# Zachary-Luk/3D-Denoising-Diffusion-Model

Hardware: AMD Instinct MI355X
Metric: denoised 64³ volumes/sec @250 DDPM steps, 1/2/4/8 MI355X; PSNR vs ref (higher is better)
Workload: dtype f32 (conv products: 3x f16-split MFMA, f32 accumulate)

## Files before the change

3d-denoising-diffusion-model_amd/csrc/api.hip:

```cpp
#include <hip/hip_runtime.h>
#include <stdarg.h>
#include <stdio.h>
#include <string.h>
#include "conv3d_params.h"
#include "ddpm3d.h"
#include "ops.h"

static thread_local char g_err[512] = "";

static int fail(int code, const char* fmt, ...) {
    va_list ap;
    va_start(ap, fmt);
    vsnprintf(g_err, sizeof(g_err), fmt, ap);
    va_end(ap);
    return code;
}
static int launched(hipError_t e, const char* what) {
    if (e == hipSuccess) return DDPM3D_OK;
    return fail(DDPM3D_ELAUNCH, "%s: %s", what, hipGetErrorString(e));
}
static bool aligned16(const void* p) { return (reinterpret_cast<uintptr_t>(p) & 15) == 0; }

extern "C" {

// ... 51 lines not shown
    if (N <= 0 || D <= 0 || H <= 0 || W <= 0 || Cin <= 0 || Cout <= 0 || !prec_ok(precision)) return 0;
    return ddpm3d_conv_cfg(N, D, H, W, Cin, Cout, ksize, precision).workspace_bytes;
}

enum { ROUTE_GENERAL = 0, ROUTE_SKINNY = 1, ROUTE_PW = 2 };
static int conv_prepare(const ddpm3d_conv_desc* d, ConvK& k, ConvCfg& c, int& route, bool for_launch) {
    if (!d) return fail(DDPM3D_EINVAL, "conv3d: null descriptor");
    if (d->N <= 0 || d->D <= 0 || d->H <= 0 || d->W <= 0 || d->Cout <= 0 || d->Cin <= 0)
        return fail(DDPM3D_EINVAL, "conv3d: non-positive shape N=%d D=%d H=%d W=%d Cin=%d Cout=%d", d->N, d->D,
                    d->H, d->W, d->Cin, d->Cout);
    if (d->ksize != 1 && d->ksize != 3) return fail(DDPM3D_EINVAL, "conv3d: ksize %d (1 or 3)", d->ksize);
    if (!prec_ok(d->precision)) return fail(DDPM3D_ENOSUP, "conv3d: precision mode %d not implemented", d->precision);
    if (d->C0 + d->C1 != d->Cin) return fail(DDPM3D_EINVAL, "conv3d: C0+C1 != Cin");
    if (for_launch && (!d->src0 || !d->w_packed || !d->bias || !d->out)) return fail(DDPM3D_EINVAL, "conv3d: null buffer");
    if (d->in_mode == DDPM3D_IN_PLANAR2) {
        if (d->Cin != 2 || d->C0 != 1 || d->C1 != 1 || (for_launch && !d->src1) || d->aff_a)
            return fail(DDPM3D_EINVAL, "conv3d: planar2 input needs C0=C1=1, two planes, no affine");
    } else {
        if (d->in_mode < 0 || d->in_mode > DDPM3D_IN_STRIDE2) return fail(DDPM3D_EINVAL, "conv3d: in_mode %d", d->in_mode);
        if (d->in_mode == DDPM3D_IN_STRIDE2 && d->ksize != 3)
            return fail(DDPM3D_EINVAL, "conv3d: the strided input mode is the 3x3x3 Downsample conv's");
        if (d->Cin % DDPM3D_CONV_CK) return fail(DDPM3D_EINVAL, "conv3d: Cin=%d not a multiple of %d", d->Cin, DDPM3D_CONV_CK);
        if (d->C1 > 0 && (d->C0 % DDPM3D_CONV_CK || (for_launch && !d->src1)))
            return fail(DDPM3D_EINVAL, "conv3d: concat needs C0 %% %d == 0 and src1", DDPM3D_CONV_CK);
        if (!aligned16(d->src0) || (d->src1 && !aligned16(d->src1)))
            return fail(DDPM3D_EINVAL, "conv3d: sources must be 16-byte aligned");
        if (d->in_mode == DDPM3D_IN_UP && ((d->H | d->W) & 1))
            return fail(DDPM3D_EINVAL, "conv3d: upsampled input needs even H, W (got %d, %d)", d->H, d->W);
    }
    if ((d->aff_a == nullptr) != (d->aff_b == nullptr)) return fail(DDPM3D_EINVAL, "conv3d: aff_a/aff_b must come together");
    if (d->aff_a && (!aligned16(d->aff_a) || !aligned16(d->aff_b)))
        return fail(DDPM3D_EINVAL, "conv3d: affine tables must be 16-byte aligned");
    if (!aligned16(d->w_packed)) return fail(DDPM3D_EINVAL, "conv3d: w_packed must be 16-byte aligned");
    if (d->res_mode < 0 || d->res_mode > 3 || (d->res_mode != DDPM3D_RES_NONE && !d->res))
        return fail(DDPM3D_EINVAL, "conv3d: residual mode %d without / with bad buffer", d->res_mode);
    if (d->res_mode == DDPM3D_RES_UP && ((d->H | d->W) & 1))
        return fail(DDPM3D_EINVAL, "conv3d: upsampled residual needs even H, W");
    if (d->bias_stride_n < 0) return fail(DDPM3D_EINVAL, "conv3d: negative bias_stride_n");
    if (d->out_layout != DDPM3D_OUT_NDHWC && d->out_layout != DDPM3D_OUT_NCDHW)
        return fail(DDPM3D_EINVAL, "conv3d: out_layout %d", d->out_layout);

    c = ddpm3d_conv_cfg(d->N, d->D, d->H, d->W, d->Cin, d->Cout, d->ksize, d->precision);
    if (d->kernel_hint & DDPM3D_HINT_SPLITK_MASK) {
        const int s_forced = (d->kernel_hint & DDPM3D_HINT_SPLITK_MASK) >> DDPM3D_HINT_SPLITK_SHIFT;
        const int nch = ddpm3d_cin_pad(d->Cin) / DDPM3D_CONV_CK;
        if (s_forced > nch || (s_forced != c.S && c.WN != 4))
            return fail(DDPM3D_EINVAL, "conv3d: a forced split factor needs Cout > 64 and S <= Cin / 16");
        ddpm3d_conv_cfg_split(c, s_forced, d->N, d->D, d->H, d->W, d->Cout);
    }
    if (prec_wz(d->precision) &&
        !(wz_layer_ok(d->Cout, d->Cin, d->ksize) && c.WN == 4 && c.MT == 4 &&
          (d->in_mode == DDPM3D_IN_SAME || d->in_mode == DDPM3D_IN_UP)))
        return fail(DDPM3D_ENOSUP, "conv3d: the Winograd-D form needs ksize 3, Cout %% 128 == 0 "
                                   "and input mode SAME or UP; use the F16X3 packing for this call");
    if (for_launch && c.S > 1 && (!d->workspace || d->workspace_bytes < c.workspace_bytes || !aligned16(d->workspace)))
        return fail(DDPM3D_EINVAL, "conv3d: this shape is split %d-way over Cin and needs %zu bytes of "
                                   "16-byte aligned workspace (got %zu)", c.S, c.workspace_bytes,
                    d->workspace ? d->workspace_bytes : (size_t)0);
    memset(&k, 0, sizeof(k));
    k.src0 = d->src0; k.src1 = d->src1; k.affA = d->aff_a; k.affB = d->aff_b;
    k.w = (const float*)d->w_packed; k.bias = d->bias; k.res = d->res; k.out = d->out; k.stats = d->stats;
    k.N = d->N; k.D = d->D; k.H = d->H; k.W = d->W; k.Cin = d->Cin; k.Cout = d->Cout;
    k.C0 = d->C0; k.C1 = d->C1;
    k.CinPad = ddpm3d_cin_pad(d->Cin); k.CoutPad = ddpm3d_cout_pad(d->Cout);
    k.in_mode = d->in_mode; k.act = d->act; k.bias_stride_n = d->bias_stride_n;
    k.res_mode = d->res_mode; k.out_layout = d->out_layout;
    k.tilesZ = c.tilesZ; k.tilesY = c.tilesY; k.tilesX = c.tilesX;
    k.stats_rows = c.stats_rows;
    k.reduce_vox = c.reduce_vox;
    k.hint = d->kernel_hint;
    bool phase = false;
    if (d->kernel_hint & DDPM3D_HINT_UP_PHASE) {
        if (d->precision != DDPM3D_PREC_F16X3_WZ || d->in_mode != DDPM3D_IN_UP)
            return fail(DDPM3D_EINVAL, "conv3d: DDPM3D_HINT_UP_PHASE needs precision F16X3_WZ and in_mode UP");
        UpPhaseGeom g;
        phase = ddpm3d_up_phase_geom(d->D, d->H, d->W, c, g) && d->res_mode != DDPM3D_RES_POOL;
        if (!phase) k.hint &= ~DDPM3D_HINT_UP_PHASE;
    }
    const size_t w_front = phase ? ddpm3d_packed_bytes(d->Cout, d->Cin, d->ksize, d->precision) : (size_t)0;
    k.w = (const float*)((const char*)d->w_packed + w_front);
    k.io = d->io_dtype;
    if (d->io_dtype & ~(DDPM3D_IO_SRC0_BF16 | DDPM3D_IO_SRC1_BF16 | DDPM3D_IO_OUT_BF16 | DDPM3D_IO_RES_BF16 |
                        DDPM3D_IO_HALF_IS_F16))
        return fail(DDPM3D_EINVAL, "conv3d: unknown io_dtype bits %#x", d->io_dtype);
    if ((d->io_dtype & DDPM3D_IO_OUT_BF16) && d->out_layout != DDPM3D_OUT_NDHWC)
        return fail(DDPM3D_EINVAL, "conv3d: a 16-bit output needs the NDHWC layout");
    if ((d->io_dtype & (DDPM3D_IO_SRC0_BF16 | DDPM3D_IO_SRC1_BF16)) && d->in_mode == DDPM3D_IN_PLANAR2)
        return fail(DDPM3D_EINVAL, "conv3d: the planar input volumes are fp32");
    if (prec_scaled(d->precision)) {
        if (!d->in_bound || d->in_bound_count <= 0 || d->in_bound_count > 64 || d->in_bound_stride <= 0)
            return fail(DDPM3D_EINVAL, "conv3d: the split-f16 precisions need in_bound (1..64 entries per sample): "
                                       "the activation scale is derived from it, nothing is clamped");
        k.in_bound = d->in_bound;
        k.in_bound_count = d->in_bound_count;
        k.in_bound_stride = d->in_bound_stride;
    }
    k.ksplit = c.S;
    k.chunks_per_split = (k.CinPad / DDPM3D_CONV_CK + c.S - 1) / c.S;
    if (d->ksize == 1 && c.S > 1) k.chunks_per_split = (k.chunks_per_split + 1) & ~1;
    k.partial = (float*)d->workspace;
    {
        const bool dbl = d->in_mode == DDPM3D_IN_POOL || d->in_mode == DDPM3D_IN_STRIDE2;
        const long long Hs = dbl ? 2LL * d->H : (d->in_mode == DDPM3D_IN_UP ? d->H / 2 : d->H);
        const long long Ws = dbl ? 2LL * d->W : (d->in_mode == DDPM3D_IN_UP ? d->W / 2 : d->W);
        const long long vox = (long long)d->N * d->D * Hs * Ws;
        const long long b0 = vox * d->C0 * ((d->io_dtype & DDPM3D_IO_SRC0_BF16) ? 2 : 4);
        const long long b1 = vox * d->C1 * ((d->io_dtype & DDPM3D_IO_SRC1_BF16) ? 2 : 4);
        const size_t wb = phase ? ddpm3d_up_phase_body_bytes(d->Cout, d->Cin)
                                : ddpm3d_packed_bytes(d->Cout, d->Cin, d->ksize, d->precision);
        if (b0 >= 0xFFFFFFF0LL || b1 >= 0xFFFFFFF0LL || wb >= 0xFFFFFFF0ULL)
            return fail(DDPM3D_E2BIG, "conv3d: a source tensor or the weights exceed 4 GiB; split the batch");
        if ((long long)d->D * d->H * d->W * d->Cout * 4 >= 0xFFFFFFF0LL)
            return fail(DDPM3D_E2BIG, "conv3d: one output sample exceeds 4 GiB; tile the volume");
        k.src0_bytes = (unsigned)b0; k.src1_bytes = (unsigned)b1; k.w_bytes = (unsigned)wb;
        k.wstat = (d->kernel_hint & DDPM3D_HINT_WSTAT_ON)    ? 1
                  : (d->kernel_hint & DDPM3D_HINT_WSTAT_OFF) ? 0
                                                             : ((long long)wb > b0 + b1 ? 1 : 0);
    }
    if (phase)
        k.wscale = (const float*)((const char*)k.w + ddpm3d_up_phase_body_bytes(d->Cout, d->Cin));
    else if (c.PREC != DDPM3D_PREC_F32)
        k.wscale = (const float*)((const char*)d->w_packed +
                                  ddpm3d_packed_bytes(d->Cout, d->Cin, d->ksize, d->precision) -
                                  (size_t)ddpm3d_cout_pad(d->Cout) * 4);
    if (d->stats && d->stats_rows != k.stats_rows)
        return fail(DDPM3D_EINVAL, "conv3d: stats_rows=%d, this shape writes %d", d->stats_rows, k.stats_rows);
    if (d->stats && !aligned16(d->stats)) return fail(DDPM3D_EINVAL, "conv3d: stats must be 16-byte aligned");
    if (d->stats && d->out_layout != DDPM3D_OUT_NDHWC)
        return fail(DDPM3D_EINVAL, "conv3d: statistics only with NDHWC output");
    const long long blocks = (long long)k.N * k.tilesZ * k.tilesY * k.tilesX;
    if (blocks > 0x7fffffffLL) return fail(DDPM3D_EINVAL, "conv3d: grid too large");
    if (d->ksize == 3 && d->Cout <= 2 && d->in_mode == DDPM3D_IN_SAME && d->C1 == 0 && !d->stats &&
        d->res_mode == DDPM3D_RES_NONE &&
        ddpm3d_skinny_ok(k.CinPad, d->precision, !(d->io_dtype & DDPM3D_IO_SRC0_BF16) ? 0
                                                  : ((d->io_dtype & DDPM3D_IO_HALF_IS_F16) ? 2 : 1)))
        route = ROUTE_SKINNY;
    else
        route = ddpm3d_pw_ok(k, c, d->ksize) ? ROUTE_PW : ROUTE_GENERAL;
    return DDPM3D_OK;
}

int ddpm3d_conv3d(const ddpm3d_conv_desc* d, void* stream) {
    ConvK k;
    ConvCfg c;
    int route = ROUTE_GENERAL;
    const int ok = conv_prepare(d, k, c, route, true);
    if (ok != DDPM3D_OK) return ok;
    if (route == ROUTE_SKINNY)
        return launched(ddpm3d_launch_conv_skinny(k, d->precision, (hipStream_t)stream), "conv3d (skinny)");
    const int rc = route == ROUTE_PW ? launched(ddpm3d_launch_conv_pw(k, c, (hipStream_t)stream), "conv3d (1x1)")
                                     : launched(ddpm3d_launch_conv(k, c, (hipStream_t)stream), "conv3d");
    if (rc != DDPM3D_OK || c.S == 1) return rc;
    return launched(ddpm3d_launch_splitk_reduce(k, (hipStream_t)stream), "conv3d split-K reduce");
}

int ddpm3d_conv_plan(const ddpm3d_conv_desc* d, int* stats_rows, size_t* workspace_bytes, int* split) {
    ConvK k;
    ConvCfg c;
    int route = ROUTE_GENERAL;
    const int ok = conv_prepare(d, k, c, route, false);
    if (ok != DDPM3D_OK) return ok;
    if (stats_rows) *stats_rows = c.stats_rows;
    if (workspace_bytes) *workspace_bytes = c.workspace_bytes;
    if (split) *split = c.S;
    return DDPM3D_OK;
}

int ddpm3d_conv_kernel_family(const ddpm3d_conv_desc* d, char* name, int name_len) {
    if (!name || name_len <= 0) return fail(DDPM3D_EINVAL, "conv_kernel_family: no buffer");
    ConvK k;
    ConvCfg c;
    int route = ROUTE_GENERAL;
    const int ok = conv_prepare(d, k, c, route, false);
    if (ok != DDPM3D_OK) return ok;
    const int tile = 1 << c.TXL;
    int n;
    if (route == ROUTE_SKINNY) n = snprintf(name, (size_t)name_len, "conv3d_p%d_k3_skinny", d->precision);
    else if (route == ROUTE_PW) n = snprintf(name, (size_t)name_len, "conv1x1_p%d_t%d", d->precision, tile);
    else n = snprintf(name, (size_t)name_len, "conv3d_p%d_k%d_wn%d_t%d", d->precision, d->ksize, c.WN, tile);
    if (n < 0 || n >= name_len) return fail(DDPM3D_EINVAL, "conv_kernel_family: buffer of %d bytes is too short", name_len);
    return DDPM3D_OK;
}

int ddpm3d_gn_finalize(const double* stats0, int C0, int rows0, const double* stats1, int C1, int rows1,
                       int N, int groups, double count, float eps, const float* gamma, const float* beta,
                       const float* film, int film_stride, int film_off, float* aff_a, float* aff_b,
                       float* bound, void* stream) {
    const int C = C0 + C1;
    if (!stats0 || N <= 0 || groups <= 0 || C0 <= 0 || C1 < 0 || rows0 <= 0 || count <= 0)
        return fail(DDPM3D_EINVAL, "gn_finalize: bad arguments");
    if (!aligned16(stats0) || (stats1 && !aligned16(stats1)))
        return fail(DDPM3D_EINVAL, "gn_finalize: statistics must be 16-byte aligned");
    if (gamma ? (!beta || !aff_a || !aff_b) : !bound)
        return fail(DDPM3D_EINVAL, "gn_finalize: gamma needs beta, aff_a, aff_b; without gamma only `bound` is written");
    if (C % groups) return fail(DDPM3D_EINVAL, "gn_finalize: C=%d not divisible by %d groups", C, groups);
    const int cg = C / groups;
    if (C1 > 0 && (!stats1 || rows1 <= 0 || C0 % cg))
        return fail(DDPM3D_EINVAL, "gn_finalize: a group straddles the concat boundary (C0=%d, group=%d)", C0, cg);
    return launched(ddpm3d_launch_gn_finalize(stats0, C0, rows0, stats1, C1, rows1, N, groups, count, eps,
                                              gamma, beta, film, film_stride, film_off, aff_a, aff_b, bound,
                                              (hipStream_t)stream),
                    "gn_finalize");
}

int ddpm3d_absmax(const float* x0, const float* x1, int N, size_t per_sample, float* bound, void* stream) {
    if (!x0 || !bound || N <= 0 || per_sample == 0) return fail(DDPM3D_EINVAL, "absmax: bad arguments");
    return launched(ddpm3d_launch_absmax(x0, x1, N, per_sample, bound, (hipStream_t)stream), "absmax");
}

int ddpm3d_gn_stats_rows(int voxels) { return voxels > 0 ? ddpm3d_gn_stats_rows_impl(voxels) : 0; }

int ddpm3d_gn_stats(const float* x, int N, int voxels, int C, double* stats, void* stream) {
    if (!x || !stats || N <= 0 || voxels <= 0 || C <= 0 || (C & 3) || !aligned16(x) || !aligned16(stats))
        return fail(DDPM3D_EINVAL, "gn_stats: bad arguments (C must be a multiple of 4, x 16-byte aligned)");
    return launched(ddpm3d_launch_gn_stats(x, N, voxels, C, stats, (hipStream_t)stream), "gn_stats");
}

int ddpm3d_timestep_embedding(const float* t, int rows, int dim, const float* freqs, float* out, void* stream) {
    if (!t || !out || !freqs || rows <= 0 || dim <= 1) return fail(DDPM3D_EINVAL, "timestep_embedding: bad arguments");
    return launched(ddpm3d_launch_timestep_embedding(t, rows, dim, freqs, out, (hipStream_t)stream),
                    "timestep_embedding");
}

int ddpm3d_linear(const float* in, int rows, int K, const float* w, const float* bias, int O, int silu_in,
                  float* out, int out_stride, void* stream) {
    if (!in || !w || !bias || !out || rows <= 0 || K <= 0 || O <= 0 || out_stride < O)
        return fail(DDPM3D_EINVAL, "linear: bad arguments");
    return launched(ddpm3d_launch_linear(in, rows, K, w, bias, O, silu_in, out, out_stride, (hipStream_t)stream),
                    "linear");
}

int ddpm3d_pool_act(const void* src, const float* aff_a, const float* aff_b, int act, int fast_act, int N, int D,
                    int H, int W, int C, void* out, int io_dtype, void* stream) {
    if (!src || !out || N <= 0 || D <= 0 || H <= 0 || W <= 0 || C <= 0 || (C & 3))
        return fail(DDPM3D_EINVAL, "pool_act: bad arguments (C must be a multiple of 4)");
    if ((aff_a == nullptr) != (aff_b == nullptr)) return fail(DDPM3D_EINVAL, "pool_act: aff_a/aff_b must come together");
    if (act && !aff_a) return fail(DDPM3D_EINVAL, "pool_act: an activation needs the affine tables (pass A = 1, B = 0)");
    if (io_dtype & ~(DDPM3D_IO_SRC0_BF16 | DDPM3D_IO_OUT_BF16 | DDPM3D_IO_HALF_IS_F16))
        return fail(DDPM3D_EINVAL, "pool_act: io_dtype bits %#x", io_dtype);
    if (!aligned16(src) || !aligned16(out) || (aff_a && (!aligned16(aff_a) || !aligned16(aff_b))))
        return fail(DDPM3D_EINVAL, "pool_act: buffers must be 16-byte aligned");
    if ((long long)N * D * H * W * (C / 4) > 0x7fffffffLL * 256)
        return fail(DDPM3D_E2BIG, "pool_act: grid too large; split the batch");
    return launched(ddpm3d_launch_pool_act((const float*)src, aff_a, aff_b, act, fast_act, N, D, H, W, C, (float*)out,
                                           (io_dtype & DDPM3D_IO_SRC0_BF16) != 0, (io_dtype & DDPM3D_IO_OUT_BF16) != 0,
                                           (io_dtype & DDPM3D_IO_HALF_IS_F16) != 0, (hipStream_t)stream),
                    "pool_act");
}

int ddpm3d_add_embedding(float* emb, const float* table, const int64_t* idx, int rows, int dim, int num_classes,
                         void* stream) {
    if (!emb || !table || !idx || rows <= 0 || dim <= 0 || num_classes <= 0)
        return fail(DDPM3D_EINVAL, "add_embedding: bad arguments");
    (void)num_classes;
    return launched(ddpm3d_launch_add_embedding(emb, table, idx, rows, dim, num_classes, (hipStream_t)stream), "add_embedding");
}

int ddpm3d_ncdhw_to_ndhwc(const float* in, int N, int C, int voxels, float* out, void* stream) {
    if (!in || !out || N <= 0 || C <= 0 || voxels <= 0) return fail(DDPM3D_EINVAL, "ncdhw_to_ndhwc: bad arguments");
    return launched(ddpm3d_launch_transpose(in, N, C, voxels, out, (hipStream_t)stream), "ncdhw_to_ndhwc");
}
int ddpm3d_ndhwc_to_ncdhw(const float* in, int N, int C, int voxels, float* out, void* stream) {
    if (!in || !out || N <= 0 || C <= 0 || voxels <= 0) return fail(DDPM3D_EINVAL, "ndhwc_to_ncdhw: bad arguments");
    return launched(ddpm3d_launch_transpose(in, N, voxels, C, out, (hipStream_t)stream), "ndhwc_to_ncdhw");
}

int ddpm3d_ncdhw_to_ndhwc_pad(const float* in, int N, int C, int voxels, int Cpad, float* out, void* stream) {
    if (!in || !out || N <= 0 || C <= 0 || voxels <= 0 || Cpad < C)
        return fail(DDPM3D_EINVAL, "ncdhw_to_ndhwc_pad: bad arguments");
    return launched(ddpm3d_launch_to_ndhwc_pad(in, N, C, voxels, Cpad, out, (hipStream_t)stream), "ncdhw_to_ndhwc_pad");
}

int ddpm3d_subsample_hw2(const float* in, int N, int D, int H, int W, int C, float* out, void* stream) {
    if (!in || !out || N <= 0 || D <= 0 || H <= 0 || W <= 0 || C <= 0 || (H & 1) || (W & 1) || (C & 3) ||
        !aligned16(in) || !aligned16(out))
        return fail(DDPM3D_EINVAL, "subsample_hw2: needs even H, W, C %% 4 == 0 and 16-byte aligned tensors");
    return launched(ddpm3d_launch_subsample_hw2(in, N, D, H, W, C, out, (hipStream_t)stream), "subsample_hw2");
}

int ddpm3d_attention_p(const float* qkv, int N, int T, int heads, int head_channels, int precision,
                       const float* qkv_bound, int bound_count, int bound_stride, float* out, void* stream) {
    if (!qkv || !out || N <= 0 || T <= 0 || heads <= 0) return fail(DDPM3D_EINVAL, "attention: bad arguments");
    if (head_channels != 32 && head_channels != 64 && head_channels != 128)
        return fail(DDPM3D_ENOSUP, "attention: %d channels per head (32, 64 or 128 are built)", head_channels);
    if (precision != DDPM3D_PREC_F32 && precision != DDPM3D_PREC_F16X3)
        return fail(DDPM3D_ENOSUP, "attention: precision %d (F32 and F16X3 are built)", precision);
    if (!aligned16(qkv) || !aligned16(out)) return fail(DDPM3D_EINVAL, "attention: buffers must be 16-byte aligned");
    if (precision != DDPM3D_PREC_F32 && (!qkv_bound || bound_count <= 0 || bound_count > 64 || bound_stride <= 0))
        return fail(DDPM3D_EINVAL, "attention: the split-f16 arithmetic needs qkv_bound (1..64 entries per sample)");
    return launched(ddpm3d_launch_attention(qkv, N, T, heads, head_channels, precision, qkv_bound, bound_count,
                                            bound_stride, out, (hipStream_t)stream),
                    "attention");
}

int ddpm3d_attention(const float* qkv, int N, int T, int heads, int head_channels, float* out, void* stream) {
    return ddpm3d_attention_p(qkv, N, T, heads, head_channels, DDPM3D_PREC_F32, nullptr, 0, 0, out, stream);
}

static int step_args_ok(const float* mo, const float* x, const float* noise, const float* coef,
                        const int64_t* t, int N, int voxels, float* sample) {
    return mo && x && noise && coef && t && sample && N > 0 && voxels > 0;
}

int ddpm3d_p_sample_step(const float* model_out, const float* x, const float* noise, const float* coef,
                         const int64_t* t_idx, int N, int voxels, int flags, float* sample,
                         float* pred_xstart, void* stream) {
// ... 383 lines not shown
```

3d-denoising-diffusion-model_amd/csrc/conv3d.hip:

```cpp
#include <hip/hip_runtime.h>
#include "conv3d_load.h"
#include "conv3d_epilogue.h"

template <int PREC, int PIPEM, int KS, int WN, int MT, int TXL, int TYL>
__global__ __launch_bounds__(256, (PIPEM == 2 ? 1 : (TXL == 2 ? 2 : 3))) void conv3d_kernel(const ConvK p) {
    constexpr int CK = DDPM3D_CONV_CK;
    constexpr int PIPE = PIPEM == 1 ? 1 : 0;
    constexpr int SXY = PIPEM == 2 ? 2 : 1;
    constexpr int WM = 4 / WN;
    constexpr int TX = 1 << TXL, TY = 1 << TYL;
    constexpr int TZ = WM * MT * 32 / (TX * TY);
    constexpr int PAD = KS / 2;
    constexpr int HX = SXY * (TX - 1) + KS, HY = SXY * (TY - 1) + KS, HZ = TZ + 2 * PAD;
    constexpr int HV = HX * HY * HZ;
    constexpr int VS = 5;
    constexpr int RY = LdsGeom<TX, HX, HY>::RY;
    constexpr int RZ = LdsGeom<TX, HX, HY>::RZ;
    constexpr int QPV = CK / 4;
    constexpr int NT = KS * KS * KS;
    constexpr int NL = (HV * QPV + 255) / 256;

    extern __shared__ __attribute__((aligned(16))) unsigned char lds[];

    const int tid = threadIdx.x;
// ... 71 lines not shown
    for (int chunk = chunk_begin; chunk < chunk_end; ++chunk) {
        __syncthreads();
        {
            auto store_item = [&](int hz, int hy, int hx, const f32x4 v) {
                unsigned char* vrow = lds + (hz * RZ + hy * RY + hx * VS) * 16;
                if constexpr (PREC == 0) {
                    *reinterpret_cast<f32x4*>(vrow + q * 16) = v;
                } else if constexpr (PREC == 5) {
                    *reinterpret_cast<u32x2*>(vrow + q * 8) = u32x2{bf16_pack(v[0], v[1]), bf16_pack(v[2], v[3])};
                } else {
                    h4 hi, lo;
#pragma unroll
                    for (int c = 0; c < 4; ++c) {
                        const float s = v[c] * asc.s;
                        hi[c] = (_Float16)s;
                        lo[c] = (_Float16)(s - (float)hi[c]);
                    }
                    *reinterpret_cast<h4*>(vrow + q * 8) = hi;
                    if constexpr (PREC == 1) *reinterpret_cast<h4*>(vrow + 32 + q * 8) = lo;
                }
            };
            if constexpr (PIPE) {
#pragma unroll
                for (int i = 0; i < NL; ++i) {
                    const int idx = tid + i * 256;
                    if (idx < HV * QPV) {
                        const int hv = idx / QPV;
                        const int hz = hv / (HY * HX);
                        const int rem = hv - hz * (HY * HX);
                        const int hy = rem / HX;
                        const int hx = rem - hy * HX;
                        const bool inb = halo_inb(p, z0 - PAD + hz, y0 - PAD + hy, x0 - PAD + hx);
                        store_item(hz, hy, hx, halo_finish<PREC != 0>(hs, quad_bits_expand(raw[i], hs.b16, hs.f16), inb, act_mask));
                    }
                }
            } else {
#pragma unroll 1
                for (int idx = tid; idx < HV * QPV; idx += 256) {
                    const int hv = idx / QPV;
                    const int hz = hv / (HY * HX);
                    const int rem = hv - hz * (HY * HX);
                    const int hy = rem / HX;
                    const int hx = rem - hy * HX;
                    store_item(hz, hy, hx, halo_fetch<PREC != 0>(p, hs, n, z0 - PAD + hz, SXY * y0 - PAD + hy,
                                                                 SXY * x0 - PAD + hx, q, chunk == 0));
                }
            }
        }
        __syncthreads();
        const bool more = chunk + 1 < chunk_end;
        if (more) hs = halo_src<CK>(p, n, chunk + 1, q);
        if (!wave_active) {
            if (PIPE && more) issue_raw(hs);
            continue;
        }

        const unsigned wchunk = (unsigned)chunk * wchunk_stride;
        constexpr bool LO = PREC != 2 && PREC != 5;
        constexpr int R = 3;
        u32x4 bq[R][2];
#pragma unroll
        for (int s = 0; s < R - 1 && s < NT; ++s) {
            bq[s][0] = buffer_load16(wrsrc, wlane, wchunk + s * wtap_stride);
            if (LO) bq[s][1] = buffer_load16(wrsrc, wlane, wchunk + s * wtap_stride + wpart);
        }
        constexpr bool AHEAD = PREC != 0 && (TXL == 2 || KS == 1);
        h8 af[2][MT][2];
        if constexpr (AHEAD) {
#pragma unroll
            for (int t = 0; t < MT; ++t) {
                af[0][t][0] = *reinterpret_cast<const h8*>(lds + arow[t]);
                if (LO) af[0][t][1] = *reinterpret_cast<const h8*>(lds + arow[t] + 32);
            }
        }
#pragma unroll
        for (int tap = 0; tap < NT; ++tap) {
            if constexpr (AHEAD) {
                __builtin_amdgcn_sched_barrier(0);
                if (tap + 1 < NT) {
                    const int t1 = tap + 1;
                    const int off1 = ((t1 / (KS * KS)) * RZ + ((t1 / KS) % KS) * RY + (t1 % KS) * VS) * 16;
#pragma unroll
                    for (int t = 0; t < MT; ++t) {
                        af[t1 & 1][t][0] = *reinterpret_cast<const h8*>(lds + arow[t] + off1);
                        if (LO) af[t1 & 1][t][1] = *reinterpret_cast<const h8*>(lds + arow[t] + off1 + 32);
                    }
                }
            }
            if (tap + R - 1 < NT) {
                bq[(tap + R - 1) % R][0] = buffer_load16(wrsrc, wlane, wchunk + (tap + R - 1) * wtap_stride);
                if (LO) bq[(tap + R - 1) % R][1] = buffer_load16(wrsrc, wlane, wchunk + (tap + R - 1) * wtap_stride + wpart);
            }
            if constexpr (AHEAD) __builtin_amdgcn_sched_barrier(0);
            if (PIPE && tap == (NT >= R ? NT - R : 0) && more) issue_raw(hs);
            const int dz = tap / (KS * KS), dy = (tap / KS) % KS, dx = tap % KS;
            const int tapoff = (dz * RZ + dy * RY + dx * VS) * 16;
            const u32x4 b0 = bq[tap % R][0], b1 = LO ? bq[tap % R][1] : b0;
            if constexpr (PREC == 0) {
#pragma unroll
                for (int kk = 0; kk < 2; ++kk) {
                    f32x4 a[MT];
#pragma unroll
                    for (int t = 0; t < MT; ++t)
                        a[t] = *reinterpret_cast<const f32x4*>(lds + arow[t] + tapoff + kk * 32);
                    const f32x4 b = __builtin_bit_cast(f32x4, kk == 0 ? b0 : b1);
#pragma unroll
                    for (int s = 0; s < 4; ++s)
#pragma unroll
                        for (int t = 0; t < MT; ++t)
                            acc[t] = __builtin_amdgcn_mfma_f32_32x32x2f32(a[t][s], b[s], acc[t], 0, 0, 0);
                }
            } else if constexpr (PREC == 2 || PREC == 5) {
                const h8 bhi = __builtin_bit_cast(h8, b0);
#pragma unroll
                for (int t = 0; t < MT; ++t) {
                    const h8 ahi = AHEAD ? af[tap & 1][t][0] : *reinterpret_cast<const h8*>(lds + arow[t] + tapoff);
                    acc[t] = mfma16<PREC == 5>(ahi, bhi, acc[t]);
                }
            } else {
                const h8 bhi = __builtin_bit_cast(h8, b0);
                const h8 blo = __builtin_bit_cast(h8, b1);
#pragma unroll
                for (int t = 0; t < MT; ++t) {
                    const h8 ahi = AHEAD ? af[tap & 1][t][0] : *reinterpret_cast<const h8*>(lds + arow[t] + tapoff);
                    const h8 alo = AHEAD ? af[tap & 1][t][1] : *reinterpret_cast<const h8*>(lds + arow[t] + tapoff + 32);
                    acc[t] = __builtin_amdgcn_mfma_f32_32x32x16_f16(alo, bhi, acc[t], 0, 0, 0);
                    acc[t] = __builtin_amdgcn_mfma_f32_32x32x16_f16(ahi, blo, acc[t], 0, 0, 0);
                    acc[t] = __builtin_amdgcn_mfma_f32_32x32x16_f16(ahi, bhi, acc[t], 0, 0, 0);
                }
            }
        }
    }

    if (!wave_active) return;

    const int tile_in_n = (tz_i * p.tilesY + ty_i) * p.tilesX + tx_i;
    conv_epilogue<PREC, WM, MT, TXL, TYL, PREC == 2 || PREC == 5>(p, acc, n, z0, y0, x0, tile_in_n, wm, cout, half, wg.split,
                                                                 asc.inv);
}

#ifndef DDPM3D_PREC_ONLY
#error "compile with -DDDPM3D_PREC_ONLY=0, 1, 2, 3 or 5"
#endif
#if DDPM3D_PREC_ONLY == 0

__global__ __launch_bounds__(256) void conv_splitk_reduce_kernel(const ConvK p) {
    const size_t DHW = (size_t)p.D * p.H * p.W;
    const int rows = p.stats_rows;
    const int n = blockIdx.x / rows, r = blockIdx.x % rows;
    const size_t v0 = (size_t)r * p.reduce_vox;
    const size_t v1 = min(v0 + (size_t)p.reduce_vox, DHW);
    const size_t slab_stride = (size_t)p.N * DHW * p.Cout;
    for (int cout = threadIdx.x; cout < p.Cout; cout += 256) {
        const float bias = p.bias[(size_t)n * p.bias_stride_n + cout];
        GnAcc gs;
        gs.init(0.0f);
        float cnt = 0.0f;
        for (size_t v = v0; v < v1; ++v) {
            const size_t e = ((size_t)n * DHW + v) * p.Cout + cout;
            float val = p.partial[e];
            for (int s = 1; s < p.ksplit; ++s) val += p.partial[e + s * slab_stride];
            val += bias;
            if (p.res_mode != DDPM3D_RES_NONE) {
                const int x = (int)(v % p.W), y = (int)((v / p.W) % p.H), z = (int)(v / ((size_t)p.W * p.H));
                val += ddpm3d_residual(p, n, z, y, x, cout);
            }
            if (p.out_layout == DDPM3D_OUT_NDHWC)
                ddpm3d_act_store(p.out, e, val, (p.io & DDPM3D_IO_OUT_BF16) != 0, (p.io & DDPM3D_IO_HALF_IS_F16) != 0);
            else
                p.out[((size_t)n * p.Cout + cout) * DHW + v] = val;
            if (cnt == 0.0f) gs.init(val);
            gs.add(val);
            cnt += 1.0f;
        }
        if (p.stats != nullptr)
            *reinterpret_cast<double2*>(p.stats + (((size_t)n * p.Cout + cout) * rows + r) * 2) =
                make_double2(gs.sum1(cnt), gs.sum2(cnt));
    }
}

template <int RV>
__global__ __launch_bounds__(256) void conv_splitk_reduce_v4_kernel(const ConvK p) {
    const size_t DHW = (size_t)p.D * p.H * p.W;
    const int rows = p.stats_rows;
    const int n = blockIdx.x / rows, r = blockIdx.x % rows;
    const size_t v0 = (size_t)r * RV;
    const size_t slab_stride = (size_t)p.N * DHW * p.Cout;
    const int quads = p.Cout / 4;
    const int cq = threadIdx.x & 63, vl = threadIdx.x >> 6;
    __shared__ double red[2][4][64 * 4];
    {
        const int q = blockIdx.y * 64 + cq;
        const bool qok = q < quads;
        GnAcc gs[4];
        float cnt = 0.0f;
#pragma unroll
        for (int c = 0; c < 4; ++c) gs[c].init(0.0f);
        if (qok) {
            const f32x4 bias = *reinterpret_cast<const f32x4*>(p.bias + (size_t)n * p.bias_stride_n + q * 4);
#pragma unroll
            for (int i = 0; i < RV / 4; ++i) {
                const size_t v = v0 + vl + 4 * i;
                if (v < DHW) {
                    const size_t e = ((size_t)n * DHW + v) * p.Cout + q * 4;
                    f32x4 val = *reinterpret_cast<const f32x4*>(p.partial + e);
                    int s = 1;
                    for (; s + 3 < p.ksplit; s += 4) {
                        const f32x4 a = *reinterpret_cast<const f32x4*>(p.partial + e + (size_t)s * slab_stride);
                        const f32x4 b = *reinterpret_cast<const f32x4*>(p.partial + e + (size_t)(s + 1) * slab_stride);
                        const f32x4 c = *reinterpret_cast<const f32x4*>(p.partial + e + (size_t)(s + 2) * slab_stride);
                        const f32x4 d = *reinterpret_cast<const f32x4*>(p.partial + e + (size_t)(s + 3) * slab_stride);
                        val += a; val += b; val += c; val += d;
                    }
                    for (; s < p.ksplit; ++s)
                        val += *reinterpret_cast<const f32x4*>(p.partial + e + (size_t)s * slab_stride);
                    val += bias;
                    if (p.res_mode != DDPM3D_RES_NONE) {
                        const int x = (int)(v % p.W), y = (int)((v / p.W) % p.H), z = (int)(v / ((size_t)p.W * p.H));
#pragma unroll
                        for (int c = 0; c < 4; ++c) val[c] += ddpm3d_residual(p, n, z, y, x, q * 4 + c);
                    }
                    if (p.io & DDPM3D_IO_OUT_BF16) {
                        const bool f16 = (p.io & DDPM3D_IO_HALF_IS_F16) != 0;
                        u32x2 pk = u32x2{half_pack(val[0], val[1], f16), half_pack(val[2], val[3], f16)};
                        *reinterpret_cast<u32x2*>(reinterpret_cast<unsigned short*>(p.out) + e) = pk;
                        asm volatile("s_nop 7" : "+v"(pk) : : "memory");
                    }
                    else
                        *reinterpret_cast<f32x4*>(p.out + e) = val;
#pragma unroll
                    for (int c = 0; c < 4; ++c) {
                        if (cnt == 0.0f) gs[c].init(val[c]);
                        gs[c].add(val[c]);
                    }
                    cnt += 1.0f;
                }
            }
        }
        if (p.stats != nullptr) {
#pragma unroll
            for (int c = 0; c < 4; ++c) {
                red[0][vl][cq * 4 + c] = gs[c].sum1(cnt);
                red[1][vl][cq * 4 + c] = gs[c].sum2(cnt);
            }
            __syncthreads();
            if (vl == 0 && qok) {
#pragma unroll
                for (int c = 0; c < 4; ++c) {
                    const double a = (red[0][0][cq * 4 + c] + red[0][1][cq * 4 + c]) +
                                     (red[0][2][cq * 4 + c] + red[0][3][cq * 4 + c]);
                    const double b = (red[1][0][cq * 4 + c] + red[1][1][cq * 4 + c]) +
                                     (red[1][2][cq * 4 + c] + red[1][3][cq * 4 + c]);
                    *reinterpret_cast<double2*>(p.stats + (((size_t)n * p.Cout + q * 4 + c) * rows + r) * 2) =
                        make_double2(a, b);
                }
            }
            __syncthreads();
        }
    }
}

hipError_t ddpm3d_launch_splitk_reduce(const ConvK& k, hipStream_t st) {
    if (k.Cout % 4 == 0 && k.out_layout == DDPM3D_OUT_NDHWC) {
        const dim3 grid(k.N * k.stats_rows, (k.Cout / 4 + 63) / 64);
        switch (k.reduce_vox) {
            case 4: hipLaunchKernelGGL(conv_splitk_reduce_v4_kernel<4>, grid, dim3(256), 0, st, k); break;
            case 8: hipLaunchKernelGGL(conv_splitk_reduce_v4_kernel<8>, grid, dim3(256), 0, st, k); break;
            case 16: hipLaunchKernelGGL(conv_splitk_reduce_v4_kernel<16>, grid, dim3(256), 0, st, k); break;
            default: return hipErrorInvalidValue;
        }
    } else
        hipLaunchKernelGGL(conv_splitk_reduce_kernel, dim3(k.N * k.stats_rows), dim3(256), 0, st, k);
    return hipGetLastError();
}

hipError_t ddpm3d_launch_conv_p0(const ConvK& k, const ConvCfg& c, hipStream_t st);
hipError_t ddpm3d_launch_conv_p1(const ConvK& k, const ConvCfg& c, hipStream_t st);
hipError_t ddpm3d_launch_conv_p2(const ConvK& k, const ConvCfg& c, hipStream_t st);
hipError_t ddpm3d_launch_conv_p5(const ConvK& k, const ConvCfg& c, hipStream_t st);
hipError_t ddpm3d_launch_conv_wz(const ConvK& k, const ConvCfg& c, hipStream_t st);

hipError_t ddpm3d_launch_conv(const ConvK& k, const ConvCfg& c, hipStream_t st) {
    switch (c.PREC) {
        case 0: return ddpm3d_launch_conv_p0(k, c, st);
        case 1: return ddpm3d_launch_conv_p1(k, c, st);
        case 2: return ddpm3d_launch_conv_p2(k, c, st);
        case 3:
        case 4:
        case 6: return ddpm3d_launch_conv_wz(k, c, st);
        case 5: return ddpm3d_launch_conv_p5(k, c, st);
    }
    return hipErrorInvalidValue;
}
#endif

#if DDPM3D_PREC_ONLY == 3
#include "conv3d_wz.h"
hipError_t ddpm3d_launch_conv_wz(const ConvK& k, const ConvCfg& c, hipStream_t st) {
    const int gy = k.CoutPad / 128;
    const int gx = k.N * k.tilesZ * k.tilesY * k.tilesX;
#ifdef DDPM3D_WZ_STAMPS
    constexpr size_t stamp_lds = 4 * WZ_NSTAMP * 8;
#else
    constexpr size_t stamp_lds = 0;
#endif
    constexpr size_t lds = (size_t)WzGeom::BUF + stamp_lds;
    if (k.hint & DDPM3D_HINT_UP_PHASE) {
        UpPhaseGeom g;
        if (c.PREC != DDPM3D_PREC_F16X3_WZ || !ddpm3d_up_phase_geom(k.D, k.H, k.W, c, g)) return hipErrorInvalidValue;
        ConvK k2 = k;
        k2.tilesX = g.tilesX; k2.tilesY = g.tilesY; k2.tilesZ = g.tilesZ;
        const dim3 grid(4 * k.N * g.tilesZ * g.tilesY * g.tilesX, gy, k.ksplit);
        constexpr size_t plds4 = (size_t)WzGeomT<4>::BUF + stamp_lds, plds84 = (size_t)WzGeomT<8, 4>::BUF + stamp_lds;
        if (g.TX == 4)
            hipLaunchKernelGGL((conv3d_wz_kernel<WZ_F16X3_UP, 4, 4, 4>), grid, dim3(256), plds4, st, k2);
        else if (g.TY == 4)
            hipLaunchKernelGGL((conv3d_wz_kernel<WZ_F16X3_UP, 4, 8, 4>), grid, dim3(256), plds84, st, k2);
        else
            hipLaunchKernelGGL((conv3d_wz_kernel<WZ_F16X3_UP, 4, 8, 8>), grid, dim3(256), lds, st, k2);
        return hipGetLastError();
    }
    if (c.TXL == 2) {
        constexpr size_t lds4 = (size_t)WzGeomT<4>::BUF + stamp_lds;
        if (c.PREC == DDPM3D_PREC_F16_WZ)
            hipLaunchKernelGGL((conv3d_wz_kernel<WZ_F16, 0, 4>), dim3(gx, gy, k.ksplit), dim3(256), lds4, st, k);
        else if (c.PREC == DDPM3D_PREC_BF16_WZ)
            hipLaunchKernelGGL((conv3d_wz_kernel<WZ_BF16, 0, 4>), dim3(gx, gy, k.ksplit), dim3(256), lds4, st, k);
        else
            hipLaunchKernelGGL((conv3d_wz_kernel<WZ_F16X3, 4, 4>), dim3(gx, gy, k.ksplit), dim3(256), lds4, st, k);
        return hipGetLastError();
    }
#ifndef DDPM3D_WZ_T84
#define DDPM3D_WZ_T84 1
#endif
    if (DDPM3D_WZ_T84 && k.H % 8 == 0 && k.D % 4 == 0 && !(k.hint & DDPM3D_HINT_WZ_ORDER_MASK)) {
        ConvK k2 = k;
        k2.tilesY = 2 * k.tilesY;
        k2.tilesZ = k.tilesZ / 2;
        constexpr size_t lds84 = (size_t)WzGeomT<8, 4>::BUF + stamp_lds;
        if (c.PREC == DDPM3D_PREC_F16_WZ)
            hipLaunchKernelGGL((conv3d_wz_kernel<WZ_F16, 0, 8, 4>), dim3(gx, gy, k.ksplit), dim3(256), lds84, st, k2);
        else if (c.PREC == DDPM3D_PREC_BF16_WZ)
            hipLaunchKernelGGL((conv3d_wz_kernel<WZ_BF16, 0, 8, 4>), dim3(gx, gy, k.ksplit), dim3(256), lds84, st, k2);
        else
            hipLaunchKernelGGL((conv3d_wz_kernel<WZ_F16X3, 4, 8, 4>), dim3(gx, gy, k.ksplit), dim3(256), lds84, st, k2);
        return hipGetLastError();
    }
    if (c.PREC == DDPM3D_PREC_F16_WZ)
        hipLaunchKernelGGL(conv3d_wz_kernel<WZ_F16>, dim3(gx, gy, k.ksplit), dim3(256), lds, st, k);
    else if (c.PREC == DDPM3D_PREC_BF16_WZ)
        hipLaunchKernelGGL(conv3d_wz_kernel<WZ_BF16>, dim3(gx, gy, k.ksplit), dim3(256), lds, st, k);
    else {
        int order = (k.hint & DDPM3D_HINT_WZ_ORDER_MASK) >> DDPM3D_HINT_WZ_ORDER_SHIFT;
        if (order == 0) order = 5;
        switch (order - 1) {
            case 0: hipLaunchKernelGGL((conv3d_wz_kernel<WZ_F16X3, 0>), dim3(gx, gy, k.ksplit), dim3(256), lds, st, k); break;
            case 1: hipLaunchKernelGGL((conv3d_wz_kernel<WZ_F16X3, 1>), dim3(gx, gy, k.ksplit), dim3(256), lds, st, k); break;
            case 2: hipLaunchKernelGGL((conv3d_wz_kernel<WZ_F16X3, 2>), dim3(gx, gy, k.ksplit), dim3(256), lds, st, k); break;
            case 4: hipLaunchKernelGGL((conv3d_wz_kernel<WZ_F16X3, 4>), dim3(gx, gy, k.ksplit), dim3(256), lds, st, k); break;
            default: return hipErrorInvalidValue;
        }
    }
    return hipGetLastError();
}
#else

template <int PREC, int PIPE, int KS, int WN, int MT, int TXL, int TYL>
static hipError_t launch_cfg(const ConvK& k, int grid_x, int grid_y, hipStream_t st) {
    constexpr int TX = 1 << TXL, TY = 1 << TYL, TZ = (4 / WN) * MT * 32 / (TX * TY);
    constexpr int PAD = KS / 2, SXY = PIPE == 2 ? 2 : 1;
    constexpr int HX = SXY * (TX - 1) + KS, HY = SXY * (TY - 1) + KS, HZ = TZ + 2 * PAD;
    constexpr size_t lds_bytes = (size_t)HZ * LdsGeom<TX, HX, HY>::RZ * 16;
    if constexpr (lds_bytes > 65536) {
        static DynLdsOnce once = {};
        const hipError_t attr = ddpm3d_allow_dynamic_lds(
            once, reinterpret_cast<const void*>(&conv3d_kernel<PREC, PIPE, KS, WN, MT, TXL, TYL>), (int)lds_bytes);
        if (attr != hipSuccess) return attr;
    }
    hipLaunchKernelGGL((conv3d_kernel<PREC, PIPE, KS, WN, MT, TXL, TYL>), dim3(grid_x, grid_y, k.ksplit), dim3(256),
                       lds_bytes, st, k);
    return hipGetLastError();
}

#define DDPM3D_CAT2(a, b) a##b
#define DDPM3D_CAT(a, b) DDPM3D_CAT2(a, b)
hipError_t DDPM3D_CAT(ddpm3d_launch_conv_p, DDPM3D_PREC_ONLY)(const ConvK& k, const ConvCfg& c, hipStream_t st) {
    const int gx = k.N * k.tilesZ * k.tilesY * k.tilesX;
    const int gy = (k.CoutPad + 32 * c.WN - 1) / (32 * c.WN);
    const int pipe = k.in_mode == DDPM3D_IN_STRIDE2 ? 2 : ((k.in_mode == DDPM3D_IN_SAME || k.in_mode == DDPM3D_IN_UP) ? 1 : 0);
#define CASE(P_, PI_, KS_, WN_, MT_, TXL_, TYL_)                                                      \
    if (pipe == PI_ && c.KS == KS_ && c.WN == WN_ && c.MT == MT_ && c.TXL == TXL_ && c.TYL == TYL_)   \
        return launch_cfg<P_, PI_, KS_, WN_, MT_, TXL_, TYL_>(k, gx, gy, st);
#define CASES(P_, PI_)                                                                          \
    CASE(P_, PI_, 3, 4, 4, 3, 3) CASE(P_, PI_, 3, 2, 2, 3, 3) CASE(P_, PI_, 3, 1, 1, 3, 3)      \
    CASE(P_, PI_, 3, 4, 4, 2, 2) CASE(P_, PI_, 3, 2, 2, 2, 2) CASE(P_, PI_, 3, 1, 1, 2, 2)      \
    CASE(P_, PI_, 1, 4, 4, 3, 3) CASE(P_, PI_, 1, 2, 2, 3, 3) CASE(P_, PI_, 1, 1, 1, 3, 3)      \
    CASE(P_, PI_, 1, 4, 4, 2, 2) CASE(P_, PI_, 1, 2, 2, 2, 2) CASE(P_, PI_, 1, 1, 1, 2, 2)
    CASES(DDPM3D_PREC_ONLY, 1) CASES(DDPM3D_PREC_ONLY, 0)
    CASE(DDPM3D_PREC_ONLY, 2, 3, 4, 4, 3, 3) CASE(DDPM3D_PREC_ONLY, 2, 3, 2, 2, 3, 3) CASE(DDPM3D_PREC_ONLY, 2, 3, 1, 1, 3, 3)
    CASE(DDPM3D_PREC_ONLY, 2, 3, 4, 4, 2, 2) CASE(DDPM3D_PREC_ONLY, 2, 3, 2, 2, 2, 2) CASE(DDPM3D_PREC_ONLY, 2, 3, 1, 1, 2, 2)
#undef CASES
#undef CASE
    return hipErrorInvalidValue;
}
#endif
```

3d-denoising-diffusion-model_amd/csrc/conv3d_params.h:

```cpp
#pragma once
#include <hip/hip_runtime.h>
#include <stddef.h>
#include <stdlib.h>
#include "ddpm3d.h"

#define DDPM3D_CONV_CK 16
#define DDPM3D_REDUCE_VOX 16
#define DDPM3D_X3_W_TARGET 8.0f

struct ConvK {
    const float* src0;
    const float* src1;
    const float* affA;
    const float* affB;
    const float* w;
    const float* bias;
    const float* res;
    float* out;
    double* stats;
    float* partial;
    const float* wscale;
    const float* in_bound;
    int in_bound_count, in_bound_stride;
    unsigned w_bytes, src0_bytes, src1_bytes;
    int N, D, H, W, Cin, Cout, C0, C1, CinPad, CoutPad;
    int in_mode, act, bias_stride_n, res_mode, out_layout, stats_rows;
    int tilesX, tilesY, tilesZ;
    int ksplit, chunks_per_split;
    int wstat;
    int reduce_vox;
    int hint;
    int io;
};

struct ConvCfg {
    int PREC;
    int KS;
    int WN;
    int MT;
    int TXL, TYL;
    int S;
    int tilesX, tilesY, tilesZ;
    int stats_rows;
    int reduce_vox;
    size_t workspace_bytes;
};

static inline int ddpm3d_round_up(int v, int m) { return (v + m - 1) / m * m; }
static inline int ddpm3d_cout_pad(int Cout) { return ddpm3d_round_up(Cout, 32); }
static inline int ddpm3d_cin_pad(int Cin) { return ddpm3d_round_up(Cin, DDPM3D_CONV_CK); }

static inline void ddpm3d_conv_cfg_split(ConvCfg& c, int S, int N, int D, int H, int W, int Cout) {
    const long long vox = (long long)D * H * W;
    c.S = S;
    if (S > 1) {
        c.stats_rows = (int)((vox + c.reduce_vox - 1) / c.reduce_vox);
        c.workspace_bytes = (size_t)S * N * vox * Cout * sizeof(float);
    } else {
        c.stats_rows = c.tilesZ * c.tilesY * c.tilesX * (4 / c.WN);
        c.workspace_bytes = 0;
    }
}

static inline ConvCfg ddpm3d_conv_cfg(int N, int D, int H, int W, int Cin, int Cout, int ksize, int prec) {
    ConvCfg c;
    c.PREC = prec;
    const bool one_mfma = prec == DDPM3D_PREC_F16 || prec == DDPM3D_PREC_F16_WZ || prec == DDPM3D_PREC_BF16 ||
                          prec == DDPM3D_PREC_BF16_WZ;
    c.KS = ksize;
    c.WN = Cout > 64 ? 4 : (Cout > 32 ? 2 : 1);
#ifdef DDPM3D_FORCE_T4_3X3
    if (H >= 8 && W >= 8 && ksize != 3) { c.TXL = 3; c.TYL = 3; } else { c.TXL = 2; c.TYL = 2; }
#else
    if (H >= 8 && W >= 8) { c.TXL = 3; c.TYL = 3; } else { c.TXL = 2; c.TYL = 2; }
#endif
    c.MT = c.WN;
    const int TX = 1 << c.TXL, TY = 1 << c.TYL, TZ = (4 / c.WN) * c.MT * 32 / (TX * TY);
    c.tilesX = (W + TX - 1) / TX;
    c.tilesY = (H + TY - 1) / TY;
    c.tilesZ = (D + TZ - 1) / TZ;
    const long long mtiles = (long long)N * c.tilesZ * c.tilesY * c.tilesX;
    const long long blocks = mtiles * ((ddpm3d_cout_pad(Cout) + 32 * c.WN - 1) / (32 * c.WN));
    const int nch = ddpm3d_cin_pad(Cin) / DDPM3D_CONV_CK;
    int best = 1;
    if (ksize == 1 && c.WN == 4) {
        double best_cost = 1e300;
        for (int s = 1; s <= 32 && s <= nch; ++s) {
            const int cps = (nch + s - 1) / s;
            if (s > 1 && cps < 4) break;
            const long long per_cu = (blocks * s + 255) / 256;
            const double cost = (double)per_cu * (0.25 * cps + 6.0) + (s > 1 ? 6.0 : 0.0);
            if (cost < best_cost * 0.9) { best_cost = cost; best = s; }
        }
    }
    if (ksize == 3 && c.WN == 4 && !one_mfma) {
        static const double eff[4] = {1.0, 0.62, 0.78, 0.82};
        double best_cost = 1e300;
        for (int s = 1; s <= 16 && s <= nch; ++s) {
            const int cps = (nch + s - 1) / s;
            if (s > 1 && cps < 2) break;
            const long long per_cu = (blocks * s + 255) / 256;
            const double e = eff[per_cu > 3 ? 3 : (int)per_cu];
            const double cost = (double)per_cu * (cps + (s > 1 ? 0.75 : 0.5)) / e;
            if (cost < best_cost * 0.99) { best_cost = cost; best = s; }
        }
    }
    if (ksize == 3 && c.WN == 4 && one_mfma) {
        static const double eff[4] = {1.0, 0.5, 1.0, 0.9};
        static const int cand[] = {1, 2, 3, 4, 5, 6, 8, 10, 12, 16};
        const double out_mb = (double)N * D * H * W * Cout * 4.0 / 1e6;
        double best_cost = 1e300;
        for (int i = 0; i < 10 && cand[i] <= nch; ++i) {
            const int s = cand[i];
            const int cps = (nch + s - 1) / s;
            if (s > 1 && cps < 2) break;
            const long long per_cu = (blocks * s + 255) / 256;
            const double e = eff[per_cu > 3 ? 3 : (int)per_cu];
            const double cost = (double)per_cu * (cps + (s > 1 ? 3.0 : 0.25)) / e + (s > 1 ? 0.2 * s * out_mb : 0.0);
            if (cost < best_cost * 0.99) { best_cost = cost; best = s; }
        }
    }
    const long long vox = (long long)D * H * W;
    c.reduce_vox = DDPM3D_REDUCE_VOX;
    while (c.reduce_vox > 4 &&
           (long long)N * ((vox + c.reduce_vox - 1) / c.reduce_vox) * ((Cout / 4 + 63) / 64) < 1024)
        c.reduce_vox /= 2;
    ddpm3d_conv_cfg_split(c, best, N, D, H, W, Cout);
    return c;
}

static inline size_t ddpm3d_packed_bytes(int Cout, int Cin, int ksize, int prec) {
    const size_t taps = (prec == DDPM3D_PREC_F16X3_WZ || prec == DDPM3D_PREC_F16_WZ || prec == DDPM3D_PREC_BF16_WZ)
                            ? 36 : (size_t)ksize * ksize * ksize;
    const size_t body = taps * ddpm3d_cin_pad(Cin) * ddpm3d_cout_pad(Cout) * 4;
    return prec != 0 ? body + (size_t)ddpm3d_cout_pad(Cout) * 4 : body;
}

static inline size_t ddpm3d_up_phase_body_bytes(int Cout, int Cin) {
    return (size_t)64 * ddpm3d_cin_pad(Cin) * ddpm3d_cout_pad(Cout) * 4;
}
static inline size_t ddpm3d_up_phase_bytes(int Cout, int Cin) {
    return ddpm3d_packed_bytes(Cout, Cin, 3, DDPM3D_PREC_F16X3_WZ) + ddpm3d_up_phase_body_bytes(Cout, Cin) +
           (size_t)ddpm3d_cout_pad(Cout) * 4;
}
struct UpPhaseGeom { int TX, TY, tilesX, tilesY, tilesZ; };
static inline bool ddpm3d_up_phase_geom(int D, int H, int W, const ConvCfg& c, UpPhaseGeom& g) {
    if (((H | W) & 1) || c.KS != 3 || c.WN != 4 || c.MT != 4) return false;
    const int Hl = H / 2, Wl = W / 2;
    if (Hl >= 8 && Wl >= 8) { g.TX = 8; g.TY = (Hl % 8 == 0 && D % 4 == 0) ? 4 : 8; }
    else { g.TX = 4; g.TY = 4; }
    const int TZ = 128 / (g.TX * g.TY);
    g.tilesX = (Wl + g.TX - 1) / g.TX;
    g.tilesY = (Hl + g.TY - 1) / g.TY;
    g.tilesZ = (D + TZ - 1) / TZ;
    return 4LL * g.tilesX * g.tilesY * g.tilesZ == (long long)c.tilesX * c.tilesY * c.tilesZ;
}

struct DynLdsOnce { unsigned long long mask[4]; };
static inline hipError_t ddpm3d_allow_dynamic_lds(DynLdsOnce& done, const void* kernel, int bytes) {
    int dev = 0;
    hipError_t e = hipGetDevice(&dev);
    if (e != hipSuccess) return e;
    dev &= 255;
    unsigned long long& w = done.mask[dev >> 6];
    const unsigned long long bit = 1ull << (dev & 63);
    if (__atomic_load_n(&w, __ATOMIC_ACQUIRE) & bit) return hipSuccess;
    e = hipFuncSetAttribute(kernel, hipFuncAttributeMaxDynamicSharedMemorySize, bytes);
    if (e == hipSuccess) __atomic_fetch_or(&w, bit, __ATOMIC_RELEASE);
    return e;
}

hipError_t ddpm3d_launch_conv(const ConvK& k, const ConvCfg& c, hipStream_t st);
hipError_t ddpm3d_launch_splitk_reduce(const ConvK& k, hipStream_t st);
hipError_t ddpm3d_launch_conv_skinny(const ConvK& k, int prec, hipStream_t st);
hipError_t ddpm3d_launch_conv_pw(const ConvK& k, const ConvCfg& c, hipStream_t st);
static inline bool ddpm3d_pw_ok(const ConvK& k, const ConvCfg& c, int ksize) {
    const bool s0 = (k.io & DDPM3D_IO_SRC0_BF16) != 0, s1 = (k.io & DDPM3D_IO_SRC1_BF16) != 0;
    return ksize == 1 && (c.PREC == 1 || c.PREC == 2 || c.PREC == 5) && c.WN == 4 && c.MT == 4 &&
           k.in_mode == DDPM3D_IN_SAME && k.affA == nullptr && k.act == 0 && k.stats == nullptr &&
           k.Cout % 128 == 0 && k.Cin % 32 == 0 && k.C0 % 32 == 0 && (k.C1 == 0 || s0 == s1) &&
           (k.ksplit == 1 || k.chunks_per_split % 2 == 0);
}
bool ddpm3d_skinny_ok(int CinPad, int prec, int src16);

struct GnAcc {
#ifdef DDPM3D_STATS_F64
    double a1, a2;
    __device__ __forceinline__ void init(float) { a1 = 0.0; a2 = 0.0; }
    __device__ __forceinline__ void add(float v) { const double d = (double)v; a1 += d; a2 = __builtin_fma(d, d, a2); }
    __device__ __forceinline__ double sum1(float) const { return a1; }
    __device__ __forceinline__ double sum2(float) const { return a2; }
#else
    float p, s1, s2;
    __device__ __forceinline__ void init(float pivot) { p = pivot; s1 = 0.0f; s2 = 0.0f; }
    __device__ __forceinline__ void add(float v) { const float d = v - p; s1 += d; s2 = __builtin_fmaf(d, d, s2); }
    __device__ __forceinline__ double sum1(float n) const { return (double)n * (double)p + (double)s1; }
    __device__ __forceinline__ double sum2(float n) const {
        const double dp = (double)p;
        return (double)s2 + 2.0 * dp * (double)s1 + (double)n * dp * dp;
    }
#endif
};

__device__ __forceinline__ float ddpm3d_half_to_float(unsigned short h, bool f16) {
    if (f16) return (float)__builtin_bit_cast(_Float16, h);
    return __builtin_bit_cast(float, (unsigned)h << 16);
}
__device__ __forceinline__ float ddpm3d_act_load(const float* base, size_t e, bool b16, bool f16) {
    if (b16) return ddpm3d_half_to_float(reinterpret_cast<const unsigned short*>(base)[e], f16);
    return base[e];
}
__device__ __forceinline__ unsigned short ddpm3d_to_bf16(float v) {
    return __builtin_bit_cast(unsigned short, (__bf16)v);
}
__device__ __forceinline__ unsigned short ddpm3d_to_half(float v, bool f16) {
    if (f16) return __builtin_bit_cast(unsigned short, (_Float16)v);
    return ddpm3d_to_bf16(v);
}
__device__ __forceinline__ void ddpm3d_act_store(float* base, size_t e, float v, bool b16, bool f16) {
    if (b16) reinterpret_cast<unsigned short*>(base)[e] = ddpm3d_to_half(v, f16);
    else base[e] = v;
}

__device__ __forceinline__ float ddpm3d_residual(const ConvK& p, int n, int z, int y, int x, int cout) {
    const bool b16 = (p.io & DDPM3D_IO_RES_BF16) != 0, f16 = (p.io & DDPM3D_IO_HALF_IS_F16) != 0;
    if (p.res_mode == DDPM3D_RES_SAME) {
        const size_t vox = (((size_t)n * p.D + z) * p.H + y) * p.W + x;
        return ddpm3d_act_load(p.res, vox * p.Cout + cout, b16, f16);
    }
    if (p.res_mode == DDPM3D_RES_UP) {
        const int Hr = p.H / 2, Wr = p.W / 2;
        const size_t rv = (((size_t)n * p.D + z) * Hr + (y >> 1)) * Wr + (x >> 1);
        return ddpm3d_act_load(p.res, rv * p.Cout + cout, b16, f16);
    }
    if (p.res_mode == DDPM3D_RES_POOL) {
        const int Hr = p.H * 2, Wr = p.W * 2;
        const size_t rv = (((size_t)n * p.D + z) * Hr + 2 * y) * Wr + 2 * x;
        const size_t e = rv * p.Cout + cout;
        const float r = ((ddpm3d_act_load(p.res, e, b16, f16) + ddpm3d_act_load(p.res, e + p.Cout, b16, f16)) +
                         ddpm3d_act_load(p.res, e + (size_t)Wr * p.Cout, b16, f16)) +
                        ddpm3d_act_load(p.res, e + (size_t)Wr * p.Cout + p.Cout, b16, f16);
        return r * 0.25f;
    }
    return 0.0f;
}
```

3d-denoising-diffusion-model_amd/csrc/conv3d_stage.h:

```cpp
#pragma once
#include "conv3d_epilogue.h"

enum { WZ_F16X3 = 0, WZ_F16 = 1, WZ_BF16 = 2,
       WZ_F16X3_UP = 3 };

__device__ __forceinline__ void split_pair(float s0, float s1, unsigned& hi, unsigned& lo) {
    float l0, l1;
    asm("v_cvt_pk_f16_f32 %0, %3, %4\n\t"
        "v_fma_mix_f32 %1, %0, -1.0, %3 op_sel:[0,0,0] op_sel_hi:[1,0,0]\n\t"
        "v_fma_mix_f32 %2, %0, -1.0, %4 op_sel:[1,0,0] op_sel_hi:[1,0,0]"
        : "=&v"(hi), "=&v"(l0), "=&v"(l1)
        : "v"(s0), "v"(s1));
    asm("v_cvt_pk_f16_f32 %0, %1, %2" : "=v"(lo) : "v"(l0), "v"(l1));
}

template <int TX_, int TY_ = TX_>
struct WzGeomT {
    static constexpr int CK = DDPM3D_CONV_CK;
    static constexpr int TX = TX_, TY = TY_, HX = TX_ + 2, HY = TY_ + 2, NP = 4, VS = 5;
    static constexpr int RP = TX_ * TY_;
    static constexpr int NZP = 64 / RP;
    static constexpr int NPL = 2 * NZP + 2;
    static constexpr int RY = LdsGeom<TX_, HX, HY>::RY;
    static constexpr int RZ = LdsGeom<TX_, HX, HY>::RZ;
    static constexpr int PAIR = NP * RZ * 16;
    static constexpr int BUF = NZP * PAIR;
    static constexpr int HC = HX * HY * (CK / 4);
    static constexpr int NL = (HC + 255) / 256;
    static_assert(RP * NZP == 64 && PAIR % 256 == 0, "128-voxel tiles; pair images keep the bank residues");
};
typedef WzGeomT<8, 8> WzGeom;

template <class G>
struct StageLaneT {
    unsigned vo0[G::NL], vo1[G::NL];
    unsigned es0, es1;
    bool f16;
    int lds[G::NL];
    bool ok[G::NL];
    unsigned plane0, plane1;
    int zb;
    float scale;
    float km, ka;
    int q;
};
typedef StageLaneT<WzGeom> StageLane;

template <class G = WzGeom, bool LOWRES = false>
__device__ __forceinline__ StageLaneT<G> stage_lane(const ConvK& p, int lt, int n, int y0, int x0, int zb, float scale) {
    StageLaneT<G> s;
    s.scale = scale;
    const int up_mode = p.in_mode == DDPM3D_IN_UP ? 1 : 0;
    const int Hs = p.H >> up_mode, Ws = p.W >> up_mode;
    const int up = LOWRES ? 0 : up_mode;
    const int Hb = LOWRES ? Hs : p.H, Wb = LOWRES ? Ws : p.W;
    s.q = lt & 3;
    s.zb = zb;
    s.es0 = (p.io & DDPM3D_IO_SRC0_BF16) ? 2u : 4u;
    s.es1 = (p.io & DDPM3D_IO_SRC1_BF16) ? 2u : 4u;
    s.f16 = (p.io & DDPM3D_IO_HALF_IS_F16) != 0;
    s.plane0 = (unsigned)(Hs * Ws) * (unsigned)p.C0 * s.es0;
    s.plane1 = (unsigned)(Hs * Ws) * (unsigned)p.C1 * s.es1;
    s.km = p.act ? -1.44269504088896341f / scale : 0.0f;
    s.ka = p.act ? 0.0f : -126.0f;
#pragma unroll
    for (int i = 0; i < G::NL; ++i) {
        const int idx = lt + i * 256;
        const int hyx = idx >> 2;
        const int hy = hyx / G::HX, hx = hyx - hy * G::HX;
        const int y = y0 - 1 + hy, x = x0 - 1 + hx;
        s.ok[i] = idx < G::HC && (unsigned)y < (unsigned)Hb && (unsigned)x < (unsigned)Wb;
        const unsigned vox = (unsigned)(((n * p.D + zb) * Hs + (y >> up)) * Ws + (x >> up));
        s.vo0[i] = s.ok[i] ? (vox * (unsigned)p.C0 + s.q * 4u) * s.es0 : DDPM3D_OOB_OFFSET;
        s.vo1[i] = s.ok[i] ? (vox * (unsigned)p.C1 + s.q * 4u) * s.es1 : DDPM3D_OOB_OFFSET;
        s.lds[i] = (hy * G::RY + hx * G::VS) * 16 + s.q * 8;
    }
    return s;
}

template <class G>
__device__ __forceinline__ void stage_lane_scale(const ConvK& p, StageLaneT<G>& s, float scale) {
    s.scale = scale;
    s.km = p.act ? -1.44269504088896341f / scale : 0.0f;
}

template <class G>
__device__ __forceinline__ void stage_zero_border(const StageLaneT<G>& s, unsigned char* lds_images, int nimages, int lt) {
#pragma unroll
    for (int i = 0; i < G::NL; ++i) {
        if (lt + i * 256 < G::HC && !s.ok[i]) {
            for (int b = 0; b < nimages * G::NZP; ++b)
#pragma unroll
                for (int j = 0; j < G::NP; ++j) {
                    unsigned char* v = lds_images + b * G::PAIR + j * G::RZ * 16 + s.lds[i];
                    *reinterpret_cast<u32x2*>(v) = u32x2{0u, 0u};
                    *reinterpret_cast<u32x2*>(v + 32) = u32x2{0u, 0u};
                }
        }
    }
}

template <class G>
struct StageRawT {
    u32x4 v[G::NL][G::NPL];
    f32x4 ga, gb;
    unsigned zmask;
    bool b16;
};
typedef StageRawT<WzGeom> StageRaw;

template <class G>
__device__ __forceinline__ void stage_issue(const ConvK& p, const StageLaneT<G>& s, StageRawT<G>& r, int n, int z0, int chunk) {
    const int c0 = chunk * G::CK;
    const bool from0 = c0 < p.C0;
    const __amdgpu_buffer_rsrc_t rs = from0 ? make_rsrc(p.src0, p.src0_bytes) : make_rsrc(p.src1, p.src1_bytes);
    const unsigned plane = from0 ? s.plane0 : s.plane1;
    const unsigned cb4 = (unsigned)(from0 ? c0 : c0 - p.C0) * (from0 ? s.es0 : s.es1);
    r.b16 = (from0 ? s.es0 : s.es1) == 2u;
    r.zmask = 0;
#pragma unroll
    for (int k = 0; k < G::NPL; ++k) {
        const int z = z0 - 1 + k;
        if ((unsigned)z < (unsigned)p.D) {
            r.zmask |= 1u << k;
            const unsigned soff = cb4 + (unsigned)(z - s.zb) * plane;
#pragma unroll
            for (int i = 0; i < G::NL; ++i)
                r.v[i][k] = buffer_load_quad(rs, from0 ? s.vo0[i] : s.vo1[i], soff, r.b16);
        }
    }
    if (p.affA != nullptr) {
        r.ga = *reinterpret_cast<const f32x4*>(p.affA + (size_t)n * p.Cin + c0 + s.q * 4);
        r.gb = *reinterpret_cast<const f32x4*>(p.affB + (size_t)n * p.Cin + c0 + s.q * 4);
    } else {
        r.ga = f32x4{1.f, 1.f, 1.f, 1.f};
        r.gb = f32x4{0.f, 0.f, 0.f, 0.f};
    }
}

template <int MODE, class G>
__device__ __forceinline__ void stage_write(const StageLaneT<G>& s, const StageRawT<G>& r, unsigned char* buf) {
    float sa[4], sb[4];
#pragma unroll
    for (int c = 0; c < 4; ++c) {
        sa[c] = r.ga[c] * s.scale;
        sb[c] = r.gb[c] * s.scale;
    }
#pragma unroll
    for (int i = 0; i < G::NL; ++i) {
        auto plane = [&](const int k, float (&d)[4]) {
            if (r.zmask & (1u << k)) {
                const f32x4 x = quad_bits_expand(r.v[i][k], r.b16, s.f16);
#pragma unroll
                for (int c = 0; c < 4; ++c) {
                    const float ys = __builtin_fmaf(x[c], sa[c], sb[c]);
#ifdef DDPM3D_WZ_NOSILU
                    d[c] = ys;
// ... 45 lines not shown
```

3d-denoising-diffusion-model_amd/csrc/conv3d_wz.h:

```cpp
#pragma once
#include "conv3d_stage.h"

#ifdef DDPM3D_WZ_STAMPS
#define WZ_NSTAMP 48
#define WZ_STAMP(i) do { if (lane == 0) wz_stamps[(i)] = __builtin_amdgcn_s_memtime(); } while (0)
#else
#define WZ_STAMP(i) do { } while (0)
#endif

template <int MODE_, int IL = 0, int TX = 8, int TY = TX>
__global__ __launch_bounds__(256, 2) void conv3d_wz_kernel(const ConvK p) {
    constexpr bool PHASE = MODE_ == WZ_F16X3_UP;
    constexpr int MODE = PHASE ? (int)WZ_F16X3 : MODE_;
    typedef WzGeomT<TX, TY> G;
    constexpr bool X3 = MODE == WZ_F16X3;
    constexpr int CK = DDPM3D_CONV_CK, NT = PHASE ? 16 : 36;
    constexpr int TPJ = NT / 4;
    constexpr int TXL = TX == 8 ? 3 : 2, TYL = TY == 8 ? 3 : 2;
    constexpr int VS = G::VS, RY = G::RY, RZ = G::RZ;

    extern __shared__ __attribute__((aligned(16))) unsigned char lds[];

    const int tid = threadIdx.x;
    const int lane = tid & 63;
    const int wn = __builtin_amdgcn_readfirstlane(tid >> 6);
    const int half = lane >> 5;
#ifdef DDPM3D_WZ_STAMPS
    unsigned long long* wz_stamps = reinterpret_cast<unsigned long long*>(lds + G::BUF) + wn * WZ_NSTAMP;
    WZ_STAMP(0);
#endif

    const WgId wg = wg_id(p);
    int tile = wg.tile;
    const int tx_i = tile % p.tilesX; tile /= p.tilesX;
    const int ty_i = tile % p.tilesY; tile /= p.tilesY;
    const int tz_i = tile % p.tilesZ; tile /= p.tilesZ;
    const int ph = PHASE ? (tile & 3) : 0;
    const int py = ph >> 1, px = ph & 1;
    const int n = PHASE ? tile >> 2 : tile;
    const int x0 = tx_i * TX, y0 = ty_i * TY, z0 = tz_i * 2 * G::NZP;

    int arow[2];
#pragma unroll
    for (int t = 0; t < 2; ++t) {
        const int m = t * 32 + (lane & 31);
        const int pos = m % G::RP;
        arow[t] = (m / G::RP) * G::PAIR + ((pos >> TXL) * RY + (pos & (TX - 1)) * VS + half) * 16;
        if constexpr (PHASE) arow[t] += (py * RY + px * VS) * 16;
    }

    const int cout = wg.cy * 128 + wn * 32 + (lane & 31);
    const float pre_ws = cout < p.Cout ? p.wscale[cout] : 1.0f;
    const float pre_bias = cout < p.Cout ? p.bias[(size_t)n * p.bias_stride_n + cout] : 0.0f;
    const __amdgpu_buffer_rsrc_t wrsrc = make_rsrc(p.w, p.w_bytes);
    const unsigned wlane = ((unsigned)cout * 2 + half) * 16;
    const unsigned wpart = (unsigned)p.CoutPad * 32;
    const unsigned wchunk_stride = 2 * wpart;
    const unsigned wtap_stride = (unsigned)(p.CinPad / CK) * wchunk_stride;

    f32x16 acc[4][2];
#pragma unroll
    for (int j = 0; j < 4; ++j)
#pragma unroll
        for (int t = 0; t < 2; ++t)
#pragma unroll
            for (int i = 0; i < 16; ++i) acc[j][t][i] = 0.0f;

    const int nchunks = p.CinPad / CK;
    const int chunk_begin = wg.split * p.chunks_per_split;
    const int chunk_end = min(nchunks, chunk_begin + p.chunks_per_split);

    ActScale asc = {1.0f, 1.0f};
    float bound_raw = 0.0f;
    if constexpr (MODE != WZ_BF16) bound_raw = act_scale_load(p, n);
    StageLaneT<G> sl = stage_lane<G, PHASE>(p, tid, n, y0, x0, max(z0 - 1, 0), 1.0f);
    stage_zero_border(sl, lds, 1, tid);
    StageRawT<G> raw;
    if (chunk_begin < chunk_end) stage_issue(p, sl, raw, n, z0, chunk_begin);
    if constexpr (MODE != WZ_BF16) {
        asc = act_scale_finish(bound_raw, 2.0f);
        stage_lane_scale(p, sl, asc.s);
    }
    WZ_STAMP(1);

    constexpr int L = X3 ? 1 : 0;
#ifndef DDPM3D_WZ_RING_X3
#define DDPM3D_WZ_RING_X3 4
#endif
#ifndef DDPM3D_WZ_RING_X1
#define DDPM3D_WZ_RING_X1 8
#endif
    constexpr int R = X3 ? DDPM3D_WZ_RING_X3 : DDPM3D_WZ_RING_X1;
    constexpr int STAGE_TAP = X3 ? NT - 3 : NT - 8;
    for (int chunk = chunk_begin; chunk < chunk_end; ++chunk) {
        const bool more = chunk + 1 < chunk_end;
        const unsigned char* bufc = lds;
        WZ_STAMP(2 + (chunk - chunk_begin) * 5);
        __syncthreads();
        WZ_STAMP(3 + (chunk - chunk_begin) * 5);
        stage_write<MODE, G>(sl, raw, lds);
        WZ_STAMP(4 + (chunk - chunk_begin) * 5);
        __syncthreads();
        WZ_STAMP(5 + (chunk - chunk_begin) * 5);

        if constexpr (IL == 3 || IL == 4 || IL == 6) __builtin_amdgcn_s_setprio(1);
        unsigned woff = (unsigned)chunk * wchunk_stride + (PHASE ? (unsigned)ph * 16u * wtap_stride : 0u);
        auto bump = [&]() {
            woff += wtap_stride;
            asm volatile("" : "+s"(woff));
        };
        u32x4 bq[R][X3 ? 2 : 1];
#pragma unroll
        for (int s = 0; s < R - 1; ++s) {
            bq[s][0] = buffer_load16(wrsrc, wlane, woff);
            if (X3) bq[s][L] = buffer_load16(wrsrc, wlane, woff + wpart);
            bump();
        }
#ifndef DDPM3D_WZ_A_AHEAD
#define DDPM3D_WZ_A_AHEAD 1
#endif
        constexpr int AH = DDPM3D_WZ_A_AHEAD, AS = AH + 1;
        h8 af[AS][2][X3 ? 2 : 1];
        auto aread = [&](const int t1) {
            const int off1 = PHASE ? ((t1 / 4) * RZ + ((t1 / 2) % 2) * RY + (t1 % 2) * VS) * 16
                                   : ((t1 / 9) * RZ + ((t1 / 3) % 3) * RY + (t1 % 3) * VS) * 16;
#pragma unroll
            for (int t = 0; t < 2; ++t) {
                af[t1 % AS][t][0] = *reinterpret_cast<const h8*>(bufc + arow[t] + off1);
                if (X3) af[t1 % AS][t][L] = *reinterpret_cast<const h8*>(bufc + arow[t] + off1 + 32);
            }
        };
#pragma unroll
        for (int t1 = 0; t1 < AH; ++t1) aread(t1);
#pragma unroll
        for (int tap = 0; tap < NT; ++tap) {
            __builtin_amdgcn_sched_barrier(0);
            if (tap + AH < NT) aread(tap + AH);
            if (tap + R - 1 < NT) {
                bq[(tap + R - 1) % R][0] = buffer_load16(wrsrc, wlane, woff);
                if (X3) bq[(tap + R - 1) % R][L] = buffer_load16(wrsrc, wlane, woff + wpart);
                bump();
            }
            if constexpr (!IL) __builtin_amdgcn_sched_barrier(0);
            if (tap == STAGE_TAP && more) stage_issue(p, sl, raw, n, z0, chunk + 1);
            const int j = tap / TPJ;
            const h8 bhi = __builtin_bit_cast(h8, bq[tap % R][0]);
            if (X3) {
                const h8 blo = __builtin_bit_cast(h8, bq[tap % R][L]);
#pragma unroll
                for (int t = 0; t < 2; ++t)
                    acc[j][t] = mfma16<false>(af[tap % AS][t][L], bhi, acc[j][t]);
#pragma unroll
                for (int t = 0; t < 2; ++t)
                    acc[j][t] = mfma16<false>(af[tap % AS][t][0], blo, acc[j][t]);
            }
#pragma unroll
            for (int t = 0; t < 2; ++t)
                acc[j][t] = mfma16<MODE == WZ_BF16>(af[tap % AS][t][0], bhi, acc[j][t]);
            if constexpr (IL == 1 || IL == 3) {
#pragma unroll
                for (int i = 0; i < (X3 ? 4 : 2); ++i) {
                    __builtin_amdgcn_sched_group_barrier(0x008, 1, 0);
                    __builtin_amdgcn_sched_group_barrier(0x100, 1, 0);
                }
#pragma unroll
                for (int i = 0; i < (X3 ? 2 : 1); ++i) {
                    __builtin_amdgcn_sched_group_barrier(0x008, 1, 0);
                    __builtin_amdgcn_sched_group_barrier(0x020, 1, 0);
                }
            } else if constexpr (IL == 5 || IL == 6) {
#pragma unroll
                for (int i = 0; i < (X3 ? 2 : 1); ++i) {
                    __builtin_amdgcn_sched_group_barrier(0x008, 1, 0);
                    __builtin_amdgcn_sched_group_barrier(0x100, 2, 0);
                }
#pragma unroll
                for (int i = 0; i < (X3 ? 2 : 1); ++i) {
                    __builtin_amdgcn_sched_group_barrier(0x008, 1, 0);
                    __builtin_amdgcn_sched_group_barrier(0x020, 1, 0);
                }
            } else if constexpr (IL == 2 || IL == 4) {
#pragma unroll
                for (int i = 0; i < (X3 ? 2 : 1); ++i) {
                    __builtin_amdgcn_sched_group_barrier(0x008, 1, 0);
                    __builtin_amdgcn_sched_group_barrier(0x020, 1, 0);
                }
#pragma unroll
                for (int i = 0; i < (X3 ? 4 : 2); ++i) {
                    __builtin_amdgcn_sched_group_barrier(0x008, 1, 0);
                    __builtin_amdgcn_sched_group_barrier(0x100, 1, 0);
                }
            }
        }
        if constexpr (IL == 3 || IL == 4 || IL == 6) __builtin_amdgcn_s_setprio(0);
        WZ_STAMP(6 + (chunk - chunk_begin) * 5);
    }
    WZ_STAMP(42);

    f32x16 outv[4];
#pragma unroll
    for (int t = 0; t < 2; ++t) {
        outv[t] = acc[0][t] + acc[1][t] + acc[2][t];
        outv[2 + t] = acc[1][t] - acc[2][t] - acc[3][t];
    }
    const int tile_in_n = ((ph * p.tilesZ + tz_i) * p.tilesY + ty_i) * p.tilesX + tx_i;
    #ifndef DDPM3D_WZ_WIDE_X3
#define DDPM3D_WZ_WIDE_X3 0
#endif
#ifndef DDPM3D_WZ_LEAN
#define DDPM3D_WZ_LEAN 1
#endif
    constexpr bool LEAN = DDPM3D_WZ_LEAN && MODE != WZ_F16X3;
    const float ws1[1] = {pre_ws}, bs1[1] = {pre_bias};
    if (p.ksplit > 1) {
        if (LEAN && conv_epilogue_lean<1, 1, 4, 1, TXL, TYL, G::NZP != 1, true>(p, outv, n, z0, y0, x0, tile_in_n, 0, cout, half,
                                                                                         wg.split, asc.inv, ws1, bs1)) {
        } else
        conv_epilogue<1, 1, 4, TXL, TYL, true, G::NZP != 1, true, PHASE>(p, outv, n, z0, y0, x0, tile_in_n, 0, cout, half, wg.split,
                                                                 asc.inv, true, pre_ws, pre_bias, py, px);
    } else if (LEAN &&
               conv_epilogue_lean<1, 1, 4, 1, TXL, TYL, G::NZP != 1, false>(p, outv, n, z0, y0, x0, tile_in_n, 0, cout, half, wg.split,
                                                                           asc.inv, ws1, bs1)) {
    } else
    conv_epilogue<1, 1, 4, TXL, TYL, MODE != WZ_F16X3 || DDPM3D_WZ_WIDE_X3, G::NZP != 1, false, PHASE>(p, outv, n, z0, y0, x0, tile_in_n, 0, cout, half, wg.split,
                                                                 asc.inv, true, pre_ws, pre_bias, py, px);
#ifdef DDPM3D_WZ_STAMPS
    WZ_STAMP(43);
    if (lane == 0) {
        wz_stamps[44] = __builtin_amdgcn_s_getreg((31 << 11) | 4);
        wz_stamps[45] = __builtin_amdgcn_s_getreg((31 << 11) | 20);
        wz_stamps[46] = __builtin_amdgcn_s_memrealtime();
    }
    if (p.partial != nullptr && lane < WZ_NSTAMP) {
        const size_t wgl = blockIdx.x + (size_t)gridDim.x * (blockIdx.y + (size_t)gridDim.y * blockIdx.z);
        float* dump = p.partial + (p.ksplit > 1 ? (size_t)p.ksplit * p.N * p.D * p.H * p.W * p.Cout : (size_t)0);
        reinterpret_cast<unsigned long long*>(dump)[(wgl * 4 + wn) * WZ_NSTAMP + lane] = wz_stamps[lane];
    }
#endif
}
```

3d-denoising-diffusion-model_amd/csrc/unet_plan.hip:

```cpp
#include <hip/hip_runtime.h>
#include <stdarg.h>
#include <stdio.h>
#include <string.h>
#include <map>
#include <new>
#include <vector>
#include "ddpm3d.h"

namespace {

struct Act {
    size_t off = 0;
    int C = 0, D = 0, H = 0, W = 0;
    int esize = 4;
    size_t stats_off = 0;
    int rows = 0;
    size_t bytes(int N) const { return (size_t)N * D * H * W * C * esize; }
    long long voxels() const { return (long long)D * H * W; }
};

enum StepKind { S_CONV, S_FINALIZE, S_ABSMAX, S_PAD, S_POOL, S_ATTN };

struct Step {
    int kind;
    ddpm3d_conv_desc conv;
    size_t st0, st1; int C0, rows0, C1, rows1; double count; const float *gamma, *beta; int film, film_off;
    size_t A, B, bound; bool has_ab;
    size_t per_sample; int two; size_t dst; int C, Cpad, vox;
    size_t src, pA, pB; int act, D, H, W, io;
    size_t qkv, qb; int T, heads, ch, prec; bool has_qb;
};

struct Planner {
    const ddpm3d_unet_desc& m;
    int N, D, H, W;
    char* base;
    size_t top = 0;
    std::map<std::pair<size_t, int>, std::vector<size_t>> pool;
    std::vector<Step> steps;
    std::vector<int> film_steps, bias_steps;
    std::vector<int> bias_offs;
    std::vector<int> ws_steps;
    size_t ws_bytes = 0, ws_off = 0;
    int first_step = -1, last_step = -1, absmax_step = -1, pad_step = -1;
    size_t in_absmax = 0;
    int half_esize;
    bool scaled, f16;
    char err[256] = "";
    int code = DDPM3D_EINVAL;

    Planner(const ddpm3d_unet_desc& d, int n, int dd, int hh, int ww, char* b)
        : m(d), N(n), D(dd), H(hh), W(ww), base(b) {
        half_esize = (m.arithmetic == DDPM3D_PREC_F16 || m.arithmetic == DDPM3D_PREC_BF16) ? 2 : 4;
        f16 = m.arithmetic == DDPM3D_PREC_F16;
        scaled = m.arithmetic == DDPM3D_PREC_F16X3 || m.arithmetic == DDPM3D_PREC_F16;
    }
    bool fail(const char* fmt, ...) {
        va_list ap;
        va_start(ap, fmt);
        vsnprintf(err, sizeof(err), fmt, ap);
        va_end(ap);
        return false;
    }
    size_t alloc(size_t bytes) {
        const size_t o = (top + 255) & ~(size_t)255;
        top = o + bytes;
        return o;
    }
    void* at(size_t off) const { return base + off; }

    Act new_act(int C, int d, int h, int w, bool fp32 = false) {
        Act a;
        a.C = C; a.D = d; a.H = h; a.W = w;
        a.esize = fp32 ? 4 : half_esize;
        const size_t b = a.bytes(N);
        auto& fr = pool[{b, a.esize}];
        if (!fr.empty()) { a.off = fr.back(); fr.pop_back(); }
        else a.off = alloc(b);
        return a;
    }
    void release(const Act& a) { pool[{a.bytes(N), a.esize}].push_back(a.off); }

    bool finalize(const Act* s0, const Act* s1, const float* gamma, const float* beta, int film_off, bool force_bound,
                  size_t* A, size_t* B, size_t* bound, bool* has) {
        *has = false;
        if (!gamma && !(scaled || force_bound)) return true;
        if (s1 && s1->voxels() != s0->voxels()) return fail("concat of tensors with different spatial size");
        const int Cn = s0->C + (s1 ? s1->C : 0);
        Step st;
        memset(&st, 0, sizeof(st));
        st.kind = S_FINALIZE;
        st.st0 = s0->stats_off; st.C0 = s0->C; st.rows0 = s0->rows;
        st.st1 = s1 ? s1->stats_off : 0; st.C1 = s1 ? s1->C : 0; st.rows1 = s1 ? s1->rows : 0;
        st.count = (double)s0->voxels();
        st.gamma = gamma; st.beta = beta;
        st.has_ab = gamma != nullptr;
        if (gamma) { st.A = alloc((size_t)N * Cn * 4); st.B = alloc((size_t)N * Cn * 4); }
        st.bound = alloc((size_t)N * 32 * 2 * 4);
        st.film = film_off >= 0;
        st.film_off = film_off >= 0 ? film_off : 0;
        if (st.film) film_steps.push_back((int)steps.size());
        steps.push_back(st);
        *A = st.A; *B = st.B; *bound = st.bound; *has = true;
        return true;
    }

    struct ConvArgs {
        const Act* src0 = nullptr; const Act* src1 = nullptr;
        Act* out = nullptr;
        size_t A = 0, B = 0; bool aff = false;
        int act = DDPM3D_ACT_NONE, in_mode = DDPM3D_IN_SAME;
        const Act* res = nullptr; int res_mode = DDPM3D_RES_NONE;
        bool planar = false, want_stats = true, bias_per_n = false;
        bool ncdhw_out = false;
        size_t bound = 0; int bound_first = 0, bound_count = 0, bound_stride = 0; bool has_bound = false;
        int film_off = 0;
    };
    bool conv_step(const ddpm3d_conv_weights& pc, ConvArgs a, int* step_index = nullptr) {
        ddpm3d_conv_desc d;
        memset(&d, 0, sizeof(d));
        const bool wz = pc.w_packed_wz && !a.planar && (a.in_mode == DDPM3D_IN_SAME || a.in_mode == DDPM3D_IN_UP);
        d.precision = wz ? (pc.precision_wz & ~DDPM3D_WZ_UP_PHASE_IMAGE) : pc.precision;
        d.w_packed = wz ? pc.w_packed_wz : pc.w_packed;
        if (wz && (pc.precision_wz & DDPM3D_WZ_UP_PHASE_IMAGE) && a.in_mode == DDPM3D_IN_UP)
            d.kernel_hint = DDPM3D_HINT_UP_PHASE;
        d.bias = pc.bias;
        d.Cout = pc.Cout; d.ksize = pc.ksize;
        const Act* geo = a.out ? a.out : a.src0;
        d.N = N; d.D = geo->D; d.H = geo->H; d.W = geo->W;
        d.out_layout = a.ncdhw_out ? DDPM3D_OUT_NCDHW : DDPM3D_OUT_NDHWC;
        if (a.planar) {
            d.in_mode = DDPM3D_IN_PLANAR2; d.Cin = 2; d.C0 = 1; d.C1 = 1;
        } else {
            d.in_mode = a.in_mode;
            d.src0 = (const float*)at(a.src0->off); d.C0 = a.src0->C;
            if (a.src1) { d.src1 = (const float*)at(a.src1->off); d.C1 = a.src1->C; }
            d.Cin = d.C0 + d.C1;
            if (d.Cin != pc.Cin) return fail("conv %dx%d fed %d channels", pc.Cout, pc.Cin, d.Cin);
            if (a.src0->esize == 2) d.io_dtype |= DDPM3D_IO_SRC0_BF16;
            if (a.src1 && a.src1->esize == 2) d.io_dtype |= DDPM3D_IO_SRC1_BF16;
        }
        if (a.out) {
            d.out = (float*)at(a.out->off);
            if (a.out->esize == 2) d.io_dtype |= DDPM3D_IO_OUT_BF16;
        }
        if (a.aff) { d.aff_a = (const float*)at(a.A); d.aff_b = (const float*)at(a.B); }
        d.act = a.act;
        if (a.res) {
            if (a.res->C != pc.Cout) return fail("residual has %d channels, the conv writes %d", a.res->C, pc.Cout);
            d.res = (const float*)at(a.res->off);
            if (a.res->esize == 2) d.io_dtype |= DDPM3D_IO_RES_BF16;
        }
        d.res_mode = a.res_mode;
        if (d.io_dtype && f16) d.io_dtype |= DDPM3D_IO_HALF_IS_F16;
        if (scaled) {
            if (!a.has_bound) return fail("conv step without an input bound");
            d.in_bound = (const float*)at(a.bound) + a.bound_first;
            d.in_bound_count = a.bound_count; d.in_bound_stride = a.bound_stride;
        }
        int rows = 0, split = 1;
        size_t need = 0;
        const int rc = ddpm3d_conv_plan(&d, &rows, &need, &split);
        if (rc != DDPM3D_OK) { code = rc; return fail("%s", ddpm3d_last_error()); }
        if (a.out && a.want_stats) {
            a.out->rows = rows;
            a.out->stats_off = alloc((size_t)N * rows * pc.Cout * 2 * sizeof(double));
            d.stats = (double*)at(a.out->stats_off);
            d.stats_rows = rows;
        }
        if (need) { ws_steps.push_back((int)steps.size()); if (need > ws_bytes) ws_bytes = need; }
        Step st;
        memset(&st, 0, sizeof(st));
        st.kind = S_CONV;
        st.conv = d;
        if (a.bias_per_n) { bias_steps.push_back((int)steps.size()); bias_offs.push_back(a.film_off); }
        if (step_index) *step_index = (int)steps.size();
        steps.push_back(st);
        return true;
    }

    bool resblock(const ddpm3d_layer& e, const Act* s0, const Act* s1, Act* y_out) {
        int d = s0->D, h = s0->H, w = s0->W, im = DDPM3D_IN_SAME, rm = DDPM3D_RES_SAME;
        if (e.updown == DDPM3D_UPDOWN_DOWN) {
            if ((s0->H | s0->W) & 1) return fail("Downsample needs even H, W (got %dx%d)", s0->H, s0->W);
            h /= 2; w /= 2; im = DDPM3D_IN_POOL; rm = DDPM3D_RES_POOL;
        } else if (e.updown == DDPM3D_UPDOWN_UP) {
            h *= 2; w *= 2; im = DDPM3D_IN_UP; rm = DDPM3D_RES_UP;
        }
        size_t A1, B1, bnd1; bool has1;
        if (!finalize(s0, s1, e.norm1_gamma, e.norm1_beta, -1, false, &A1, &B1, &bnd1, &has1)) return false;
        Act h1 = new_act(e.conv1.Cout, d, h, w);
        ConvArgs c1;
        c1.src0 = s0; c1.src1 = s1; c1.out = &h1; c1.A = A1; c1.B = B1; c1.aff = true; c1.act = DDPM3D_ACT_SILU;
        c1.in_mode = im; c1.bound = bnd1; c1.bound_first = 0; c1.bound_count = 32; c1.bound_stride = 2; c1.has_bound = has1;
        Act pooled;
        bool use_pooled = false;
        if (e.updown == DDPM3D_UPDOWN_DOWN && e.conv1.w_packed_wz && !s1) {
            pooled = new_act(s0->C, d, h, w, true);
            Step st;
            memset(&st, 0, sizeof(st));
            st.kind = S_POOL;
            st.src = s0->off; st.pA = A1; st.pB = B1; st.act = DDPM3D_ACT_SILU;
            st.D = d; st.H = h; st.W = w; st.C = s0->C; st.dst = pooled.off;
            st.io = (s0->esize == 2 ? DDPM3D_IO_SRC0_BF16 : 0) | ((s0->esize == 2 && f16) ? DDPM3D_IO_HALF_IS_F16 : 0);
            steps.push_back(st);
            c1.src0 = &pooled; c1.aff = false; c1.act = DDPM3D_ACT_NONE; c1.in_mode = DDPM3D_IN_SAME;
            use_pooled = true;
        }
        size_t A2, B2, bnd2; bool has2;
        if (m.film) {
            if (!conv_step(e.conv1, c1)) return false;
            if (!finalize(&h1, nullptr, e.norm2_gamma, e.norm2_beta, e.film_off, false, &A2, &B2, &bnd2, &has2)) return false;
        } else {
            c1.bias_per_n = true; c1.film_off = e.film_off;
            if (!conv_step(e.conv1, c1)) return false;
            if (!finalize(&h1, nullptr, e.norm2_gamma, e.norm2_beta, -1, false, &A2, &B2, &bnd2, &has2)) return false;
        }
        if (use_pooled) release(pooled);
        Act y = new_act(e.conv2.Cout, d, h, w);
        ConvArgs c2;
        c2.src0 = &h1; c2.out = &y; c2.A = A2; c2.B = B2; c2.aff = true; c2.act = DDPM3D_ACT_SILU;
        c2.bound = bnd2; c2.bound_count = 32; c2.bound_stride = 2; c2.has_bound = has2;
        if (e.skip.w_packed) {
            if (e.updown != DDPM3D_UPDOWN_NONE) return fail("up/down ResBlock with a channel change is not in the reference");
            ConvArgs cs;
            cs.src0 = s0; cs.src1 = s1; cs.out = &y; cs.want_stats = false;
            cs.bound = bnd1; cs.bound_first = 1; cs.bound_count = 32; cs.bound_stride = 2; cs.has_bound = has1;
            if (!conv_step(e.skip, cs)) return false;
            c2.res = &y; c2.res_mode = DDPM3D_RES_SAME;
        } else {
            if (s1) return fail("ResBlock with an Identity skip over a concatenated input (%d + %d -> %d channels)",
                                s0->C, s1->C, e.conv2.Cout);
            c2.res = s0; c2.res_mode = rm;
        }
        if (!conv_step(e.conv2, c2)) return false;
        release(h1);
        *y_out = y;
        return true;
    }

    bool attention(const ddpm3d_layer& e, const Act* x, Act* y_out) {
        const int Cn = x->C;
        if (e.heads <= 0 || Cn % e.heads) return fail("attention: %d channels not divisible by %d heads", Cn, e.heads);
        const int ch = Cn / e.heads;
        if (ch != 32 && ch != 64 && ch != 128) return fail("attention with %d channels per head (32, 64 or 128 are built)", ch);
        size_t A, B, bnd; bool has;
        if (!finalize(x, nullptr, e.norm1_gamma, e.norm1_beta, -1, false, &A, &B, &bnd, &has)) return false;
        Act qkv = new_act(3 * Cn, x->D, x->H, x->W, true);
        ConvArgs cq;
        cq.src0 = x; cq.out = &qkv; cq.A = A; cq.B = B; cq.aff = true; cq.act = DDPM3D_ACT_NONE;
        cq.bound = bnd; cq.bound_count = 32; cq.bound_stride = 2; cq.has_bound = has;
        if (!conv_step(e.conv1, cq)) return false;
        size_t qA, qB, qb; bool hasq;
        if (!finalize(&qkv, nullptr, nullptr, nullptr, -1, m.arithmetic != DDPM3D_PREC_F32, &qA, &qB, &qb, &hasq)) return false;
        Act a = new_act(Cn, x->D, x->H, x->W, true);
        Step st;
        memset(&st, 0, sizeof(st));
        st.kind = S_ATTN;
        st.qkv = qkv.off; st.T = (int)x->voxels(); st.heads = e.heads; st.ch = ch;
        st.prec = m.arithmetic == DDPM3D_PREC_F32 ? DDPM3D_PREC_F32 : DDPM3D_PREC_F16X3;
        st.qb = qb; st.has_qb = hasq; st.dst = a.off;
        steps.push_back(st);
        release(qkv);
        Act y = new_act(Cn, x->D, x->H, x->W);
        ConvArgs cp;
        cp.src0 = &a; cp.out = &y; cp.res = x; cp.res_mode = DDPM3D_RES_SAME;
        cp.bound = qb; cp.bound_first = 1; cp.bound_count = 32; cp.bound_stride = 2; cp.has_bound = hasq;
        if (!conv_step(e.conv2, cp)) return false;
        release(a);
        *y_out = y;
        return true;
    }

    bool layer(const ddpm3d_layer& e, const Act* s0, const Act* s1, Act* out) {
        const bool n1 = e.norm1_gamma && e.norm1_beta, n2 = e.norm2_gamma && e.norm2_beta;
        const bool c1 = e.conv1.w_packed && e.conv1.bias, c2 = e.conv2.w_packed && e.conv2.bias;
        if (e.kind == DDPM3D_LAYER_RES && !(n1 && n2 && c1 && c2 && (!e.skip.w_packed || e.skip.bias)))
            return fail("ResBlock description without its norms / convs");
        if (e.kind == DDPM3D_LAYER_ATTN && !(n1 && c1 && c2)) return fail("AttentionBlock description without norm / qkv / proj_out");
        if ((e.kind == DDPM3D_LAYER_UPCONV || e.kind == DDPM3D_LAYER_DOWNCONV) && !c1) return fail("resampling conv without weights");
        if (e.kind == DDPM3D_LAYER_RES) return resblock(e, s0, s1, out);
        if (e.kind == DDPM3D_LAYER_ATTN) return attention(e, s0, out);
        if (e.kind == DDPM3D_LAYER_UPCONV || e.kind == DDPM3D_LAYER_DOWNCONV) {
            const bool up = e.kind == DDPM3D_LAYER_UPCONV;
            if (!up && ((s0->H | s0->W) & 1)) return fail("Downsample needs even H, W (got %dx%d)", s0->H, s0->W);
            Act y = new_act(e.conv1.Cout, s0->D, up ? s0->H * 2 : s0->H / 2, up ? s0->W * 2 : s0->W / 2);
            size_t A, B, bnd; bool has;
            if (!finalize(s0, nullptr, nullptr, nullptr, -1, false, &A, &B, &bnd, &has)) return false;
            ConvArgs c;
            c.src0 = s0; c.out = &y; c.in_mode = up ? DDPM3D_IN_UP : DDPM3D_IN_STRIDE2;
            c.bound = bnd; c.bound_first = 1; c.bound_count = 32; c.bound_stride = 2; c.has_bound = has;
            if (!conv_step(e.conv1, c)) return false;
            *out = y;
            return true;
        }
        return fail("unknown layer kind %d", e.kind);
    }

    bool build() {
        Act h = new_act(m.first.Cout, D, H, W);
        Act xin;
        if (m.planar) {
            in_absmax = alloc((size_t)N * 2 * 4);
            Step st;
            memset(&st, 0, sizeof(st));
            st.kind = S_ABSMAX; st.per_sample = (size_t)D * H * W; st.two = 1; st.dst = in_absmax;
            if (scaled) { absmax_step = (int)steps.size(); steps.push_back(st); }
            ConvArgs c;
            c.out = &h; c.planar = true; c.bound = in_absmax; c.bound_count = 2; c.bound_stride = 1; c.has_bound = true;
            if (!conv_step(m.first, c, &first_step)) return false;
        } else {
            xin = new_act(m.cin_pad, D, H, W, true);
            in_absmax = alloc((size_t)N * 4);
            Step st;
            memset(&st, 0, sizeof(st));
            st.kind = S_ABSMAX; st.per_sample = (size_t)m.in_channels * D * H * W; st.two = 0; st.dst = in_absmax;
            if (scaled) { absmax_step = (int)steps.size(); steps.push_back(st); }
            Step sp;
            memset(&sp, 0, sizeof(sp));
            sp.kind = S_PAD; sp.C = m.in_channels; sp.Cpad = m.cin_pad; sp.vox = D * H * W; sp.dst = xin.off;
            pad_step = (int)steps.size();
            steps.push_back(sp);
            ConvArgs c;
            c.src0 = &xin; c.out = &h; c.bound = in_absmax; c.bound_count = 1; c.bound_stride = 1; c.has_bound = true;
            if (!conv_step(m.first, c, &first_step)) return false;
        }
        std::vector<Act> hs;
        hs.push_back(h);
        int li = 0;
        for (int b = 0; b < m.n_input_blocks; ++b) {
            for (int i = 0; i < m.input_block_layers[b]; ++i) {
                Act prev = h;
                if (!layer(m.layers[li++], &prev, nullptr, &h)) return false;
                if (i > 0) release(prev);
            }
            hs.push_back(h);
        }
        for (int i = 0; i < m.n_middle_layers; ++i) {
            Act prev = h;
            if (!layer(m.layers[li++], &prev, nullptr, &h)) return false;
            if (prev.off != hs.back().off) release(prev);
        }
        for (int b = 0; b < m.n_output_blocks; ++b) {
            Act skip = hs.back();
            hs.pop_back();
            Act s0 = h, s1 = skip;
            bool two = true;
            for (int i = 0; i < m.output_block_layers[b]; ++i) {
                if (!layer(m.layers[li++], &s0, two ? &s1 : nullptr, &h)) return false;
                release(s0);
                if (two) release(s1);
                s0 = h;
                two = false;
            }
        }
        if (li != m.n_layers) return fail("the block sizes cover %d of %d layers", li, m.n_layers);
        size_t A, B, bnd; bool has;
        if (!finalize(&h, nullptr, m.out_gamma, m.out_beta, -1, false, &A, &B, &bnd, &has)) return false;
        ConvArgs c;
        c.src0 = &h; c.A = A; c.B = B; c.aff = true; c.act = DDPM3D_ACT_SILU; c.ncdhw_out = true; c.want_stats = false;
        c.bound = bnd; c.bound_count = 32; c.bound_stride = 2; c.has_bound = has;
        if (!conv_step(m.out, c, &last_step)) return false;
        release(h);
        if (ws_bytes) ws_off = alloc(ws_bytes);
        for (int i : ws_steps) { steps[i].conv.workspace = at(ws_off); steps[i].conv.workspace_bytes = ws_bytes; }
        return true;
    }
};

thread_local char g_unet_err[256] = "";

}

struct ddpm3d_unet_plan {
    std::vector<Step> steps;
    std::vector<int> film_steps, bias_steps, bias_offs;
    int first_step, last_step, absmax_step, pad_step;
    int N, planar, out_channels;
    char* base;
};

extern "C" {

const char* ddpm3d_unet_last_error(void) { return g_unet_err; }

static bool desc_ok(const ddpm3d_unet_desc* m, int N, int D, int H, int W) {
    return m && N > 0 && D > 0 && H > 0 && W > 0 && m->layers && m->n_layers > 0 && m->first.w_packed && m->out.w_packed &&
           m->out_gamma && m->out_beta && (m->n_input_blocks == 0 || m->input_block_layers) &&
           (m->n_output_blocks == 0 || m->output_block_layers) &&
           (m->arithmetic == DDPM3D_PREC_F32 || m->arithmetic == DDPM3D_PREC_F16X3 || m->arithmetic == DDPM3D_PREC_F16 ||
            m->arithmetic == DDPM3D_PREC_BF16);
}

size_t ddpm3d_unet_plan_bytes(const ddpm3d_unet_desc* m, int N, int D, int H, int W) {
    if (!desc_ok(m, N, D, H, W)) { snprintf(g_unet_err, sizeof(g_unet_err), "unet_plan_bytes: bad description"); return 0; }
    Planner p(*m, N, D, H, W, reinterpret_cast<char*>(4096));
    if (!p.build()) { snprintf(g_unet_err, sizeof(g_unet_err), "%s", p.err); return 0; }
    return (p.top + 255) & ~(size_t)255;
}

int ddpm3d_unet_plan_create(const ddpm3d_unet_desc* m, int N, int D, int H, int W, void* arena, size_t arena_bytes,
                            ddpm3d_unet_plan** plan) {
    if (!desc_ok(m, N, D, H, W) || !arena || !plan || (reinterpret_cast<uintptr_t>(arena) & 255)) {
        snprintf(g_unet_err, sizeof(g_unet_err), "unet_plan_create: bad description, or an arena that is not 256-byte aligned");
        return DDPM3D_EINVAL;
    }
    Planner p(*m, N, D, H, W, static_cast<char*>(arena));
    if (!p.build()) { snprintf(g_unet_err, sizeof(g_unet_err), "%s", p.err); return p.code; }
    if (p.top > arena_bytes) {
        snprintf(g_unet_err, sizeof(g_unet_err), "unet_plan_create: the plan needs %zu bytes, the arena has %zu", p.top, arena_bytes);
        return DDPM3D_EINVAL;
    }
    ddpm3d_unet_plan* pl = new (std::nothrow) ddpm3d_unet_plan();
    if (!pl) return DDPM3D_EINVAL;
    pl->steps.swap(p.steps);
    pl->film_steps.swap(p.film_steps);
    pl->bias_steps.swap(p.bias_steps);
    pl->bias_offs.swap(p.bias_offs);
    pl->first_step = p.first_step; pl->last_step = p.last_step; pl->absmax_step = p.absmax_step; pl->pad_step = p.pad_step;
    pl->N = N; pl->planar = m->planar; pl->out_channels = m->out.Cout;
    pl->base = static_cast<char*>(arena);
    *plan = pl;
    return DDPM3D_OK;
}

void ddpm3d_unet_plan_destroy(ddpm3d_unet_plan* plan) { delete plan; }

int ddpm3d_unet_forward(ddpm3d_unet_plan* pl, const float* x, const float* low_res, const float* film_rows,
                        int film_stride, float* out, void* stream) {
    if (!pl || !x || !film_rows || !out || (pl->planar && !low_res)) {
        snprintf(g_unet_err, sizeof(g_unet_err), "unet_forward: null argument");
        return DDPM3D_EINVAL;
    }
    char* b = pl->base;
    if (pl->planar) {
        pl->steps[pl->first_step].conv.src0 = x;
        pl->steps[pl->first_step].conv.src1 = low_res;
    }
    for (size_t i = 0; i < pl->bias_steps.size(); ++i) {
        ddpm3d_conv_desc& d = pl->steps[pl->bias_steps[i]].conv;
        d.bias = film_rows + pl->bias_offs[i];
        d.bias_stride_n = film_stride;
    }
    pl->steps[pl->last_step].conv.out = out;
    for (const Step& s : pl->steps) {
        int rc = DDPM3D_OK;
        switch (s.kind) {
            case S_CONV: rc = ddpm3d_conv3d(&s.conv, stream); break;
            case S_FINALIZE:
                rc = ddpm3d_gn_finalize((const double*)(b + s.st0), s.C0, s.rows0, s.C1 ? (const double*)(b + s.st1) : nullptr,
                                        s.C1, s.rows1, pl->N, 32, s.count, 1e-5f, s.gamma, s.beta,
                                        s.film ? film_rows : nullptr, s.film ? film_stride : 0, s.film_off,
                                        s.has_ab ? (float*)(b + s.A) : nullptr, s.has_ab ? (float*)(b + s.B) : nullptr,
                                        (float*)(b + s.bound), stream);
                break;
            case S_ABSMAX:
                rc = ddpm3d_absmax(x, s.two ? low_res : nullptr, pl->N, s.per_sample, (float*)(b + s.dst), stream);
                break;
            case S_PAD: rc = ddpm3d_ncdhw_to_ndhwc_pad(x, pl->N, s.C, s.vox, s.Cpad, (float*)(b + s.dst), stream); break;
            case S_POOL:
                rc = ddpm3d_pool_act(b + s.src, (const float*)(b + s.pA), (const float*)(b + s.pB), s.act, 1, pl->N, s.D, s.H,
                                     s.W, s.C, b + s.dst, s.io, stream);
                break;
            case S_ATTN:
                rc = ddpm3d_attention_p((const float*)(b + s.qkv), pl->N, s.T, s.heads, s.ch, s.prec,
                                        s.has_qb ? (const float*)(b + s.qb) + 1 : nullptr, 32, 2, (float*)(b + s.dst), stream);
                break;
        }
        if (rc != DDPM3D_OK) {
            snprintf(g_unet_err, sizeof(g_unet_err), "unet_forward: %s", ddpm3d_last_error());
            return rc;
        }
    }
    return DDPM3D_OK;
}

}
```

3d-denoising-diffusion-model_amd/guided_diffusion/_hip.py:

```python

import ctypes as C
import os

import torch

_HERE = os.path.dirname(os.path.abspath(__file__))
LIB_PATH = os.environ.get("DDPM3D_LIB") or os.path.normpath(os.path.join(_HERE, "..", "csrc", "libddpm3d.so"))

IN_SAME, IN_POOL, IN_UP, IN_PLANAR2, IN_STRIDE2 = 0, 1, 2, 3, 4
RES_NONE, RES_SAME, RES_POOL, RES_UP = 0, 1, 2, 3
ACT_NONE, ACT_SILU = 0, 1
OUT_NDHWC, OUT_NCDHW = 0, 1
F_LEARN_SIGMA, F_PREDICT_XSTART, F_CLIP = 1, 2, 4
NCOEF = 8
NQCOEF = 4
NSCOEF = 8
S_CX, S_W0, S_W1, S_W2, S_CZ = 0, 1, 2, 3, 4
PREC_F32, PREC_F16X3, PREC_F16, PREC_F16X3_WZ, PREC_F16_WZ, PREC_BF16, PREC_BF16_WZ = 0, 1, 2, 3, 4, 5, 6
PRECISIONS = {"f32": PREC_F32, "f16x3": PREC_F16X3, "f16": PREC_F16, "bf16": PREC_BF16}
WINOGRAD_OF = {PREC_F16X3: PREC_F16X3_WZ, PREC_F16: PREC_F16_WZ, PREC_BF16: PREC_BF16_WZ}
IO_SRC0_BF16, IO_SRC1_BF16, IO_OUT_BF16, IO_RES_BF16 = 1, 2, 4, 8
IO_HALF_IS_F16 = 16
ABI_VERSION = 13
MAX_DRAWS = 64
HINT_WSTAT_OFF, HINT_WSTAT_ON = 0x100, 0x200
HINT_SPLITK_SHIFT = 16
HINT_WZ_ORDER_SHIFT = 12
HINT_UP_PHASE = 0x400
WZ_UP_PHASE_IMAGE = 0x100

_fp = C.c_void_p


class ConvDesc(C.Structure):
    _fields_ = [
        ("N", C.c_int32), ("D", C.c_int32), ("H", C.c_int32), ("W", C.c_int32),
        ("Cin", C.c_int32), ("Cout", C.c_int32), ("ksize", C.c_int32), ("in_mode", C.c_int32),
        ("src0", _fp), ("src1", _fp), ("C0", C.c_int32), ("C1", C.c_int32),
        ("aff_a", _fp), ("aff_b", _fp), ("act", C.c_int32), ("precision", C.c_int32),
        ("w_packed", _fp), ("bias", _fp), ("bias_stride_n", C.c_int32), ("res_mode", C.c_int32),
        ("res", _fp), ("out", _fp), ("out_layout", C.c_int32), ("stats_rows", C.c_int32),
        ("stats", _fp), ("workspace", _fp), ("workspace_bytes", C.c_size_t),
        ("kernel_hint", C.c_int32), ("in_bound_count", C.c_int32), ("in_bound", _fp),
        ("in_bound_stride", C.c_int32), ("io_dtype", C.c_int32),
    ]


class ConvWeights(C.Structure):
    _fields_ = [("w_packed", _fp), ("w_packed_wz", _fp), ("bias", _fp), ("Cout", C.c_int32), ("Cin", C.c_int32),
                ("ksize", C.c_int32), ("precision", C.c_int32), ("precision_wz", C.c_int32)]


class Layer(C.Structure):
    _fields_ = [("kind", C.c_int32), ("updown", C.c_int32), ("heads", C.c_int32), ("film_off", C.c_int32),
                ("norm1_gamma", _fp), ("norm1_beta", _fp), ("norm2_gamma", _fp), ("norm2_beta", _fp),
                ("conv1", ConvWeights), ("conv2", ConvWeights), ("skip", ConvWeights)]


class UnetDesc(C.Structure):
    _fields_ = [("n_layers", C.c_int32), ("layers", C.POINTER(Layer)),
                ("n_input_blocks", C.c_int32), ("input_block_layers", C.POINTER(C.c_int32)),
                ("n_middle_layers", C.c_int32),
                ("n_output_blocks", C.c_int32), ("output_block_layers", C.POINTER(C.c_int32)),
                ("first", ConvWeights), ("out_gamma", _fp), ("out_beta", _fp), ("out", ConvWeights),
                ("film", C.c_int32), ("planar", C.c_int32), ("in_channels", C.c_int32), ("cin_pad", C.c_int32),
                ("arithmetic", C.c_int32)]


(EM_N, EM_SUM_E, EM_SUM_ABS_E, EM_SUM_SQ_E, EM_SUM_Y, EM_SUM_SQ_Y, EM_MIN_Y, EM_MAX_Y, EM_COVER_1, EM_COVER_2,
 EM_REC) = range(11)

(ROI_N, ROI_SUM_X, ROI_SUM_SQ_X, ROI_MIN_X, ROI_MAX_X, ROI_SUM_E, ROI_SUM_ABS_E, ROI_SUM_SQ_E, ROI_REC) = range(9)
ROI_MAX_REGIONS, ROI_CHUNK = 4096, 4096

JOINT_MAX_STARTS = 8


class JointStarts(C.Structure):
    _fields_ = [("nx", C.c_int32), ("ny", C.c_int32), ("nz", C.c_int32), ("xs", C.c_int32 * JOINT_MAX_STARTS),
                ("ys", C.c_int32 * JOINT_MAX_STARTS), ("zs", C.c_int32 * JOINT_MAX_STARTS)]


class Tiling(C.Structure):
    _fields_ = [("n", C.c_int32 * 3), ("starts", C.POINTER(C.c_int32) * 3), ("d_starts", C.c_void_p),
                ("d_cover", C.c_void_p), ("d_tables", C.c_void_p)]


class RoiIndex(C.Structure):
    _fields_ = [("regions", C.c_int32), ("entries", C.c_int64), ("offsets", C.POINTER(C.c_int64)),
                ("d_offsets", C.c_void_p), ("d_chunks", C.c_void_p), ("d_index", C.c_void_p)]


LAYER_RES, LAYER_ATTN, LAYER_DOWNCONV, LAYER_UPCONV = 1, 2, 3, 4
UPDOWN = {None: 0, "down": 1, "up": 2}

EXPORTS = {
    "ddpm3d_abi_version": (C.c_int, []),
    "ddpm3d_last_error": (C.c_char_p, []),
    "ddpm3d_packed_weight_bytes": (C.c_size_t, [C.c_int, C.c_int, C.c_int, C.c_int]),
    "ddpm3d_pack_conv_weight": (C.c_int, [_fp, C.c_int, C.c_int, C.c_int, C.c_int, _fp, _fp]),
    "ddpm3d_packed_up_phase_bytes": (C.c_size_t, [C.c_int, C.c_int]),
    "ddpm3d_pack_up_phase_weight": (C.c_int, [_fp, C.c_int, C.c_int, _fp, _fp]),
    "ddpm3d_conv_stats_rows": (C.c_int, [C.c_int] * 8),
    "ddpm3d_conv_workspace_bytes": (C.c_size_t, [C.c_int] * 8),
    "ddpm3d_conv3d": (C.c_int, [C.POINTER(ConvDesc), _fp]),
    "ddpm3d_conv_kernel_family": (C.c_int, [C.POINTER(ConvDesc), C.c_char_p, C.c_int]),
    "ddpm3d_conv_plan": (C.c_int, [C.POINTER(ConvDesc), C.POINTER(C.c_int), C.POINTER(C.c_size_t), C.POINTER(C.c_int)]),
    "ddpm3d_unet_plan_bytes": (C.c_size_t, [C.POINTER(UnetDesc), C.c_int, C.c_int, C.c_int, C.c_int]),
    "ddpm3d_unet_plan_create": (C.c_int, [C.POINTER(UnetDesc), C.c_int, C.c_int, C.c_int, C.c_int, _fp, C.c_size_t,
                                          C.POINTER(_fp)]),
    "ddpm3d_unet_forward": (C.c_int, [_fp, _fp, _fp, _fp, C.c_int, _fp, _fp]),
    "ddpm3d_unet_plan_destroy": (None, [_fp]),
    "ddpm3d_unet_last_error": (C.c_char_p, []),
    "ddpm3d_gn_finalize": (C.c_int, [_fp, C.c_int, C.c_int, _fp, C.c_int, C.c_int, C.c_int, C.c_int,
                                     C.c_double, C.c_float, _fp, _fp, _fp, C.c_int, C.c_int, _fp, _fp, _fp, _fp]),
    "ddpm3d_absmax": (C.c_int, [_fp, _fp, C.c_int, C.c_size_t, _fp, _fp]),
    "ddpm3d_gn_stats_rows": (C.c_int, [C.c_int]),
    "ddpm3d_gn_stats": (C.c_int, [_fp, C.c_int, C.c_int, C.c_int, _fp, _fp]),
    "ddpm3d_timestep_embedding": (C.c_int, [_fp, C.c_int, C.c_int, _fp, _fp, _fp]),
    "ddpm3d_linear": (C.c_int, [_fp, C.c_int, C.c_int, _fp, _fp, C.c_int, C.c_int, _fp, C.c_int, _fp]),
    "ddpm3d_attention": (C.c_int, [_fp, C.c_int, C.c_int, C.c_int, C.c_int, _fp, _fp]),
    "ddpm3d_attention_p": (C.c_int, [_fp, C.c_int, C.c_int, C.c_int, C.c_int, C.c_int, _fp, C.c_int, C.c_int,
                                     _fp, _fp]),
    "ddpm3d_ncdhw_to_ndhwc": (C.c_int, [_fp, C.c_int, C.c_int, C.c_int, _fp, _fp]),
    "ddpm3d_ndhwc_to_ncdhw": (C.c_int, [_fp, C.c_int, C.c_int, C.c_int, _fp, _fp]),
    "ddpm3d_ncdhw_to_ndhwc_pad": (C.c_int, [_fp, C.c_int, C.c_int, C.c_int, C.c_int, _fp, _fp]),
    "ddpm3d_subsample_hw2": (C.c_int, [_fp, C.c_int, C.c_int, C.c_int, C.c_int, C.c_int, _fp, _fp]),
    "ddpm3d_p_sample_step": (C.c_int, [_fp, _fp, _fp, _fp, _fp, C.c_int, C.c_int, C.c_int, _fp, _fp, _fp]),
    "ddpm3d_ddim_step": (C.c_int, [_fp, _fp, _fp, _fp, _fp, C.c_int, C.c_int, C.c_int, C.c_float,
                                   _fp, _fp, _fp]),
    "ddpm3d_add_embedding": (C.c_int, [_fp, _fp, _fp, C.c_int, C.c_int, C.c_int, _fp]),
    "ddpm3d_pool_act": (C.c_int, [_fp, _fp, _fp, C.c_int, C.c_int, C.c_int, C.c_int, C.c_int, C.c_int, C.c_int, _fp,
                                  C.c_int, _fp]),
    "ddpm3d_q_sample": (C.c_int, [_fp, _fp, _fp, _fp, C.c_int, C.c_int, C.c_int, _fp, _fp]),
    "ddpm3d_vb_terms_workspace_bytes": (C.c_size_t, [C.c_int, C.c_int]),
    "ddpm3d_vb_terms": (C.c_int, [_fp, _fp, _fp, _fp, _fp, _fp, _fp, C.c_int, C.c_int, C.c_int, C.c_int, _fp,
                                  C.c_size_t, _fp, _fp, _fp, C.c_int, _fp, _fp]),
    "ddpm3d_prior_bpd": (C.c_int, [_fp, _fp, C.c_int, C.c_int, C.c_int, _fp, C.c_size_t, _fp, _fp]),
    "ddpm3d_p_mean_variance": (C.c_int, [_fp, _fp, _fp, _fp, C.c_int, C.c_int, C.c_int, C.c_int, _fp, _fp, _fp,
                                         _fp, _fp]),
    "ddpm3d_ddim_reverse_step": (C.c_int, [_fp, _fp, _fp, _fp, C.c_int, C.c_int, C.c_int, C.c_int, _fp, _fp, _fp]),
    "ddpm3d_dpm_solver_step": (C.c_int, [_fp, _fp, _fp, _fp, _fp, _fp, _fp, _fp, C.c_int, C.c_int, C.c_int,
                                         C.c_int, C.c_int, _fp, _fp, _fp]),
    "ddpm3d_draw_stitch": (C.c_int, [_fp, C.c_int, C.c_int, _fp, C.c_int, C.c_int, C.c_int, C.c_int, C.c_int, C.c_int,
                                     _fp, _fp, _fp]),
    "ddpm3d_draw_moments": (C.c_int, [_fp, _fp, C.c_int, C.c_int64, _fp, _fp, _fp]),
    "ddpm3d_joint_gather": (C.c_int, [_fp, C.c_int, C.c_int, C.c_int, C.c_int, C.c_int, C.POINTER(JointStarts),
                                      C.c_int, C.c_int, _fp, _fp]),
    "ddpm3d_joint_blend": (C.c_int, [_fp, C.c_int, C.c_int, C.c_int, C.c_int, C.c_int, C.POINTER(JointStarts), _fp,
                                     _fp, _fp]),
    "ddpm3d_tiles_gather": (C.c_int, [_fp, C.c_int, C.c_int, C.c_int, C.c_int, C.c_int, C.POINTER(Tiling), C.c_int,
                                      C.c_int, _fp, _fp]),
    "ddpm3d_tiles_blend": (C.c_int, [_fp, C.c_int, C.c_int, C.c_int, C.c_int, C.c_int, C.POINTER(Tiling), _fp, _fp]),
    "ddpm3d_error_moments_workspace_bytes": (C.c_size_t, [C.c_int, C.c_int64]),
    "ddpm3d_error_moments": (C.c_int, [_fp, _fp, _fp, _fp, C.c_int, C.c_int64, _fp, C.c_size_t, _fp, _fp]),
    "ddpm3d_ssim3d_workspace_bytes": (C.c_size_t, [C.c_int] * 4),
    "ddpm3d_ssim3d": (C.c_int, [_fp, _fp, _fp, C.c_int, C.c_int, C.c_int, C.c_int, C.c_double, C.c_double, _fp,
                                C.c_size_t, _fp, _fp, _fp]),
    "ddpm3d_roi_moments_workspace_bytes": (C.c_size_t, [C.c_int, C.POINTER(RoiIndex)]),
    "ddpm3d_roi_moments": (C.c_int, [_fp, _fp, C.c_int, C.c_int64, C.POINTER(RoiIndex), _fp, C.c_size_t, _fp, _fp]),
    "ddpm3d_mfma_probe_flops_per_iter": (C.c_double, [C.c_int]),
    "ddpm3d_mfma_probe": (C.c_int, [C.c_int, C.c_int, C.c_int, _fp, _fp, _fp]),
}

_lib = None


def load():
    global _lib
    if _lib is not None:
        return _lib
    if not os.path.exists(LIB_PATH):
        raise RuntimeError(
            "ddpm3d HIP library not found at %s -- build it with "
            "`make -C 3d-denoising-diffusion-model_amd/csrc` (or __graft_entry__.build()); "
            "there is no CPU fallback." % LIB_PATH)
    lib = C.CDLL(LIB_PATH)
    for name, (res, args) in EXPORTS.items():
        fn = getattr(lib, name)
        fn.restype = res
        fn.argtypes = args
    if lib.ddpm3d_abi_version() != ABI_VERSION:
        raise RuntimeError("libddpm3d ABI %d, binding expects %d" % (lib.ddpm3d_abi_version(), ABI_VERSION))
    _lib = lib
    return lib


E_INVAL, E_LAUNCH, E_NOSUP, E_2BIG = -1, -2, -3, -4
PROBE_F16_32X32X16, PROBE_F16_16X16X32, PROBE_F32_32X32X2, PROBE_BF16_32X32X16, PROBE_BF16_16X16X32 = 0, 1, 2, 3, 4


class Ddpm3dError(RuntimeError):

    def __init__(self, code, msg):
        super().__init__("ddpm3d error %d: %s" % (code, msg))
        self.code = code


def check(rc):
    if rc != 0:
        raise Ddpm3dError(rc, load().ddpm3d_last_error().decode())


def conv_plan(desc):
    rows, ws, split = C.c_int(0), C.c_size_t(0), C.c_int(0)
    check(load().ddpm3d_conv_plan(C.byref(desc), C.byref(rows), C.byref(ws), C.byref(split)))
    return rows.value, ws.value, split.value


def stream():
    return torch.cuda.current_stream().cuda_stream


def ptr(t):
    return 0 if t is None else t.data_ptr()


def require_device(t, what):
    if not (isinstance(t, torch.Tensor) and t.is_cuda):
        raise RuntimeError("%s must live on the GPU: this package runs on HIP kernels only "
                           "(got %s)" % (what, getattr(t, "device", type(t))))
    if t.dtype != torch.float32 or not t.is_contiguous():
        raise RuntimeError("%s must be contiguous float32" % what)
```

3d-denoising-diffusion-model_amd/guided_diffusion/engine.py:

```python

import collections
import ctypes as C
import math
import os

import torch

from . import _hip as H


class Act:
    __slots__ = ("buf", "C", "D", "H", "W", "stats", "rows")

    def __init__(self, buf, Cn, D, Hh, W, stats, rows):
        self.buf, self.C, self.D, self.H, self.W, self.stats, self.rows = buf, Cn, D, Hh, W, stats, rows

    @property
    def half(self):
        return self.buf.dtype in (torch.bfloat16, torch.float16)

    @property
    def voxels(self):
        return self.D * self.H * self.W


class PackedConv:
    __slots__ = ("w", "b", "Cout", "Cin", "k", "precision", "wz", "up_phase")

    def __init__(self, weight, bias, precision, stream):
        lib = H.load()
        self.wz = None
        self.up_phase = False
        Cout, Cin, k = weight.shape[0], weight.shape[1], weight.shape[2]
        n = lib.ddpm3d_packed_weight_bytes(Cout, Cin, k, precision)
        if n == 0:
            raise RuntimeError("unsupported conv weight shape %s" % (tuple(weight.shape),))
        w32 = weight.detach().float().contiguous()
        self.w = torch.empty(n, dtype=torch.uint8, device=weight.device)
        H.check(lib.ddpm3d_pack_conv_weight(H.ptr(w32), Cout, Cin, k, precision, H.ptr(self.w), stream))
        self.b = bias.detach().float().contiguous()
        self.Cout, self.Cin, self.k, self.precision = Cout, Cin, k, precision

    def pack_up_phase(self, weight, stream):
        lib = H.load()
        n = lib.ddpm3d_packed_up_phase_bytes(self.Cout, self.Cin)
        if n == 0:
            raise RuntimeError("no phase image for a %dx%d conv" % (self.Cout, self.Cin))
        w32 = weight.detach().float().contiguous()
        self.w = torch.empty(n, dtype=torch.uint8, device=weight.device)
        H.check(lib.ddpm3d_pack_up_phase_weight(H.ptr(w32), self.Cout, self.Cin, H.ptr(self.w), stream))
        self.up_phase = True


class UNetEngine:

    def __init__(self, topo, params, model_channels, film, device, precision="f32", in_channels=2, planar=True,
                 winograd=True, step_graph=False):
        if precision not in H.PRECISIONS:
            raise ValueError("precision must be one of %s" % sorted(H.PRECISIONS))
        self.precision = precision
        self.step_graph = step_graph
        self.native_plan = False
        self.native_plans = collections.OrderedDict()
        self._native_desc = None
        self.lib = H.load()
        self.topo = topo
        self.device = device
        self.mc = model_channels
        self.film = film
        self.p = params
        self.plans = collections.OrderedDict()
        self.split_above = {}
        st = H.stream()
        self.conv = {}
        self.winograd = winograd
        if planar and in_channels != 2:
            raise ValueError("the planar first conv reads ONE image and ONE low_res channel (got in_channels=%d)"
                             % in_channels)
        self.planar = planar
        self.in_channels = in_channels
        self.cin_pad = (in_channels + 15) // 16 * 16
        first = topo.input[0][0].prefix
        qkv_perm = {}
        if getattr(topo, "new_attention_order", False):
            for e in topo.all_layers():
                if e.kind == "attn":
                    Cn, ch = e.cin, e.cin // e.heads
                    leg = torch.arange(3 * Cn)
                    h, part, i = leg // (3 * ch), (leg // ch) % 3, leg % ch
                    qkv_perm[e.prefix + ".qkv"] = (part * Cn + h * ch + i).to(device)
        params = dict(params)
        for base, perm in qkv_perm.items():
            params[base + ".weight"] = params[base + ".weight"][perm].contiguous()
            params[base + ".bias"] = params[base + ".bias"][perm].contiguous()
        self.p = params
        self.up_phase = (winograd and precision == "f16x3" and os.environ.get("DDPM3D_UP_PHASE", "1") != "0")
        up_conv1 = {e.prefix + ".in_layers.2" for e in topo.all_layers() if e.kind == "res" and e.updown == "up"}
        for name, t in params.items():
            if name.endswith(".weight") and t.dim() >= 3:
                base = name[:-len(".weight")]
                if t.dim() == 5:
                    w = t
                elif t.dim() == 4 and t.shape[2] == 3:
                    w = torch.zeros(t.shape[0], t.shape[1], 3, 3, 3, dtype=t.dtype, device=t.device)
                    w[:, :, 1] = t
                else:
                    w = t.reshape(t.shape[0], t.shape[1], 1, 1, 1)
                if base == first and not planar and w.shape[1] != self.cin_pad:
                    wp = torch.zeros(w.shape[0], self.cin_pad, *w.shape[2:], dtype=w.dtype, device=w.device)
                    wp[:, :w.shape[1]] = w
                    w = wp
                prec = H.PRECISIONS[precision]
                self.conv[base] = PackedConv(w, params[base + ".bias"], prec, st)
                if (prec in H.WINOGRAD_OF and self.winograd and w.shape[2] == 3 and w.shape[0] % 128 == 0
                        and w.shape[1] % 16 == 0):
                    self.conv[base].wz = PackedConv(w, params[base + ".bias"], H.WINOGRAD_OF[prec], st)
                    if self.up_phase and base in up_conv1:
                        self.conv[base].wz.pack_up_phase(w, st)
        ws, bs, self.film_off = [], [], {}
        off = 0
        for entry in topo.all_layers():
            if entry.kind != "res":
                continue
            w = params[entry.prefix + ".emb_layers.1.weight"]
            b = params[entry.prefix + ".emb_layers.1.bias"]
            if not film:
                b = b + params[entry.prefix + ".in_layers.2.bias"]
            self.film_off[entry.prefix] = off
            ws.append(w.float())
            bs.append(b.float())
            off += w.shape[0]
        self.film_total = off
        self.ted = 4 * model_channels
        half = model_channels // 2
        self.freqs = torch.exp(-math.log(10000) * torch.arange(start=0, end=half, dtype=torch.float32)
                               / half).to(device)
        self.emb_w = torch.cat(ws, 0).contiguous()
        self.emb_b = torch.cat(bs, 0).contiguous()
        torch.cuda.current_stream().synchronize()

    def film_rows(self, t_float, y=None):
        lib, st, p = self.lib, H.stream(), self.p
        R = t_float.numel()
        dev = self.device
        temb = torch.empty(R, self.mc, dtype=torch.float32, device=dev)
        e1 = torch.empty(R, self.ted, dtype=torch.float32, device=dev)
        e2 = torch.empty(R, self.ted, dtype=torch.float32, device=dev)
        rows = torch.empty(R, self.film_total, dtype=torch.float32, device=dev)
        H.check(lib.ddpm3d_timestep_embedding(H.ptr(t_float), R, self.mc, H.ptr(self.freqs), H.ptr(temb), st))
        H.check(lib.ddpm3d_linear(H.ptr(temb), R, self.mc, H.ptr(p["time_embed.0.weight"]),
                                  H.ptr(p["time_embed.0.bias"]), self.ted, 0, H.ptr(e1), self.ted, st))
        H.check(lib.ddpm3d_linear(H.ptr(e1), R, self.ted, H.ptr(p["time_embed.2.weight"]),
                                  H.ptr(p["time_embed.2.bias"]), self.ted, 1, H.ptr(e2), self.ted, st))
        if y is not None:
            table = p["label_emb.weight"]
            H.check(lib.ddpm3d_add_embedding(H.ptr(e2), H.ptr(table), H.ptr(y), R, self.ted, table.shape[0], st))
        H.check(lib.ddpm3d_linear(H.ptr(e2), R, self.ted, H.ptr(self.emb_w), H.ptr(self.emb_b),
                                  self.film_total, 1, H.ptr(rows), self.film_total, st))
        return rows

    MAX_PLANS = 4

    def plan(self, N, D, Hh, W):
        key = (N, D, Hh, W)
        pl = self.plans.get(key)
        if pl is None:
            while len(self.plans) >= self.MAX_PLANS:
                self.plans.popitem(last=False)
            pl = _Plan(self, N, D, Hh, W)
            self.plans[key] = pl
        else:
            self.plans.move_to_end(key)
        return pl

    def _conv_weights(self, pc):
        w = H.ConvWeights()
        if pc is not None:
            w.w_packed, w.bias = H.ptr(pc.w), H.ptr(pc.b)
            w.Cout, w.Cin, w.ksize, w.precision = pc.Cout, pc.Cin, pc.k, pc.precision
            if pc.wz is not None:
                w.w_packed_wz, w.precision_wz = H.ptr(pc.wz.w), pc.wz.precision
                if pc.wz.up_phase:
                    w.precision_wz |= H.WZ_UP_PHASE_IMAGE
        return w

    def native_desc(self):
        if self._native_desc is not None:
            return self._native_desc[0]
        topo, p = self.topo, self.p
        layers, keep = [], []

        def one(e):
            L = H.Layer()
            L.updown, L.heads = H.UPDOWN[e.updown], e.heads
            if e.kind == "res":
                L.kind = H.LAYER_RES
                L.film_off = self.film_off[e.prefix]
                L.norm1_gamma, L.norm1_beta = H.ptr(p[e.prefix + ".in_layers.0.weight"]), H.ptr(p[e.prefix + ".in_layers.0.bias"])
                L.norm2_gamma, L.norm2_beta = H.ptr(p[e.prefix + ".out_layers.0.weight"]), H.ptr(p[e.prefix + ".out_layers.0.bias"])
                L.conv1 = self._conv_weights(self.conv[e.prefix + ".in_layers.2"])
                L.conv2 = self._conv_weights(self.conv[e.prefix + ".out_layers.3"])
                L.skip = self._conv_weights(self.conv.get(e.prefix + ".skip_connection"))
            elif e.kind == "attn":
                L.kind = H.LAYER_ATTN
                L.norm1_gamma, L.norm1_beta = H.ptr(p[e.prefix + ".norm.weight"]), H.ptr(p[e.prefix + ".norm.bias"])
                L.conv1 = self._conv_weights(self.conv[e.prefix + ".qkv"])
                L.conv2 = self._conv_weights(self.conv[e.prefix + ".proj_out"])
            elif e.kind == "downconv":
                L.kind = H.LAYER_DOWNCONV
                L.conv1 = self._conv_weights(self.conv[e.prefix + ".op"])
            elif e.kind == "upconv":
                L.kind = H.LAYER_UPCONV
                L.conv1 = self._conv_weights(self.conv[e.prefix + ".conv"])
            else:
                raise ValueError(e.kind)
            return L

        in_sizes, out_sizes = [], []
        for blk in topo.input[1:]:
            in_sizes.append(len(blk))
            layers += [one(e) for e in blk]
        layers += [one(e) for e in topo.middle]
        for blk in topo.output:
            out_sizes.append(len(blk))
            layers += [one(e) for e in blk]
        arr = (H.Layer * len(layers))(*layers)
        ins = (C.c_int32 * max(1, len(in_sizes)))(*in_sizes)
        outs = (C.c_int32 * max(1, len(out_sizes)))(*out_sizes)
        d = H.UnetDesc()
        d.n_layers, d.layers = len(layers), arr
        d.n_input_blocks, d.input_block_layers = len(in_sizes), ins
        d.n_middle_layers = len(topo.middle)
        d.n_output_blocks, d.output_block_layers = len(out_sizes), outs
        d.first = self._conv_weights(self.conv[topo.input[0][0].prefix])
        d.out_gamma, d.out_beta = H.ptr(p["out.0.weight"]), H.ptr(p["out.0.bias"])
        d.out = self._conv_weights(self.conv["out.2"])
        d.film, d.planar = int(self.film), int(self.planar)
        d.in_channels, d.cin_pad = self.in_channels, self.cin_pad
        d.arithmetic = H.PRECISIONS[self.precision]
        self._native_desc = (d, arr, ins, outs)
        return d

    def native(self, N, D, Hh, W):
        key = (N, D, Hh, W)
        pl = self.native_plans.get(key)
        if pl is None:
            while len(self.native_plans) >= self.MAX_PLANS:
                self.native_plans.popitem(last=False)
            pl = _NativePlan(self, N, D, Hh, W)
            self.native_plans[key] = pl
        else:
            self.native_plans.move_to_end(key)
        return pl

    def forward(self, x, low_res, film_rows, film_stride, out=None):
        N, _, D, Hh, W = x.shape
        if N > self.split_above.get((D, Hh, W), 1 << 30):
            return self._forward_halves(x, low_res, film_rows, film_stride, out)
        try:
            if self.native_plan:
                return self.native(N, D, Hh, W).run(x, low_res, film_rows, film_stride, out)
            pl = self.plan(N, D, Hh, W)
            return pl.run(x, low_res, film_rows, film_stride, out)
        except H.Ddpm3dError as e:
            if N == 1 or e.code != H.E_2BIG:
                raise
        self.plans.pop((N, D, Hh, W), None)
        self.split_above[(D, Hh, W)] = min(self.split_above.get((D, Hh, W), 1 << 30), N - 1)
        return self._forward_halves(x, low_res, film_rows, film_stride, out)

    def _forward_halves(self, x, low_res, film_rows, film_stride, out):
        N = x.shape[0]
        res = out
        h = (N + 1) // 2
        for a, b in ((0, h), (h, N)):
            rows = film_rows if film_stride == 0 else film_rows.reshape(-1)[a * film_stride:]
            part = self.forward(x[a:b].contiguous(), None if low_res is None else low_res[a:b].contiguous(),
                                rows, film_stride, None if res is None else res[a:b])
            if res is None:
                res = torch.empty((N,) + tuple(part.shape[1:]), dtype=part.dtype, device=part.device)
                res[a:b] = part
        return res


class _PlanBase:
    timing = None

    def run(self, x, low_res, film_rows, film_stride, out=None):
        H.require_device(x, "x")
        if self.eng.planar:
            H.require_device(low_res, "low_res")
        if self.eng.step_graph and self.timing is None:
            return self._replay(x, low_res, film_rows, film_stride, out)
        target = out if out is not None else self.out_buf
        self._enqueue(x.data_ptr(), low_res.data_ptr() if self.eng.planar else 0, film_rows.data_ptr(), film_stride,
                      target.data_ptr())
        return target

    def _replay(self, x, low_res, film_rows, film_stride, out):
        eng, N = self.eng, self.N
        shared = film_stride == 0
        g = self.graphs.get(shared)
        if g is None:
            ft = eng.film_total
            st = {"x": torch.empty_like(x),
                  "lr": torch.empty_like(low_res) if eng.planar else None,
                  "film": torch.empty((1 if shared else N) * ft, dtype=torch.float32, device=x.device)}
            args = (st["x"].data_ptr(), st["lr"].data_ptr() if eng.planar else 0, st["film"].data_ptr(),
                    0 if shared else ft, self.out_buf.data_ptr())
            self._stage_inputs(st, x, low_res, film_rows, film_stride)
            self._enqueue(*args)
            torch.cuda.current_stream().synchronize()
            graph = torch.cuda.CUDAGraph()
            with torch.cuda.graph(graph):
                self._enqueue(*args)
            g = self.graphs[shared] = (graph, st)
        graph, st = g
        self._stage_inputs(st, x, low_res, film_rows, film_stride)
        graph.replay()
        if out is not None:
            out.copy_(self.out_buf)
            return out
        return self.out_buf

    def _stage_inputs(self, st, x, low_res, film_rows, film_stride):
        ft = self.eng.film_total
        st["x"].copy_(x)
        if st["lr"] is not None:
            st["lr"].copy_(low_res)
        flat = film_rows.reshape(-1)
        if film_stride == 0:
            st["film"].copy_(flat[:ft])
        else:
            st["film"].view(self.N, ft).copy_(torch.as_strided(flat, (self.N, ft), (film_stride, 1)))


class _NativePlan(_PlanBase):

    def __init__(self, eng, N, D, Hh, W):
        self.eng, self.N = eng, N
        self.graphs = {}
        lib, desc = eng.lib, eng.native_desc()
        need = lib.ddpm3d_unet_plan_bytes(C.byref(desc), N, D, Hh, W)
        if need == 0:
            msg = lib.ddpm3d_unet_last_error().decode()
            raise H.Ddpm3dError(H.E_2BIG if "4 GiB" in msg else H.E_INVAL, msg)
        self.arena = torch.empty(need, dtype=torch.uint8, device=eng.device)
        self.act_bytes = need
        handle = C.c_void_p()
        rc = lib.ddpm3d_unet_plan_create(C.byref(desc), N, D, Hh, W, H.ptr(self.arena), need, C.byref(handle))
        if rc != 0:
            raise H.Ddpm3dError(rc, lib.ddpm3d_unet_last_error().decode())
        self.handle = handle
        self.out_buf = torch.empty((N, eng.conv["out.2"].Cout, D, Hh, W), dtype=torch.float32, device=eng.device)

    def _enqueue(self, xptr, lrptr, fptr, film_stride, outptr):
        rc = self.eng.lib.ddpm3d_unet_forward(self.handle, xptr, lrptr, fptr, film_stride, outptr, H.stream())
        if rc != 0:
            raise H.Ddpm3dError(rc, self.eng.lib.ddpm3d_unet_last_error().decode())

    def __del__(self):
        try:
            if getattr(self, "handle", None):
                self.eng.lib.ddpm3d_unet_plan_destroy(self.handle)
        except Exception:
            pass


class _Plan(_PlanBase):
    def __init__(self, eng, N, D, Hh, W):
        self.eng = eng
        self.N = N
        self.steps = []
        self.keep = []
        self.film_patches = []
        self.bias_patches = []
        self.conv_meta = {}
        self.timing = None
        self.graphs = {}
        dev = eng.device
        topo = eng.topo
        lib = eng.lib

        self.pool = {}
        self.act_bytes = 0

        self.half_dtype = {"bf16": torch.bfloat16, "f16": torch.float16}.get(eng.precision)
        self.scaled = eng.precision in ("f16x3", "f16")

        def new_act(Cn, d, h, w, fp32=False):
            numel = N * d * h * w * Cn
            dt = self.half_dtype if (self.half_dtype is not None and not fp32) else torch.float32
            free = self.pool.get((numel, dt))
            if free:
                buf = free.pop()
            else:
                buf = torch.empty(numel, dtype=dt, device=dev)
                self.act_bytes += buf.element_size() * numel
                self.keep.append(buf)
            return Act(buf, Cn, d, h, w, None, 0)

        def release(act):
            self.pool.setdefault((act.buf.numel(), act.buf.dtype), []).append(act.buf)

        self.ws_descs = []
        self.ws_bytes = 0

        self.new_act = new_act
        self.release = release
        first = topo.input[0][0]
        cin_conv = eng.conv[first.prefix]
        self.first_desc = None
        h = new_act(cin_conv.Cout, D, Hh, W)
        if eng.planar:
            self.in_absmax = torch.empty(N * 2, dtype=torch.float32, device=dev)
            self.absmax_args = [0, 0, N, D * Hh * W, H.ptr(self.in_absmax), 0]
            if self.scaled:
                self.steps.append((lib.ddpm3d_absmax, self.absmax_args))
            self.first_desc = self.conv_step(cin_conv, srcs=None, out=h, planar=True,
                                             bound=(self.in_absmax, 0, 2, 1))
        else:
            ci = eng.in_channels
            xin = new_act(eng.cin_pad, D, Hh, W, fp32=True)
            self.in_absmax = torch.empty(N, dtype=torch.float32, device=dev)
            self.absmax_args = [0, 0, N, ci * D * Hh * W, H.ptr(self.in_absmax), 0]
            self.pad_args = [0, N, ci, D * Hh * W, eng.cin_pad, H.ptr(xin.buf), 0]
            if self.scaled:
                self.steps.append((lib.ddpm3d_absmax, self.absmax_args))
            self.steps.append((lib.ddpm3d_ncdhw_to_ndhwc_pad, self.pad_args))
            self.first_desc = self.conv_step(cin_conv, srcs=[xin], out=h, bound=(self.in_absmax, 0, 1, 1))
        hs = [h]
        for blk in topo.input[1:]:
            for i, e in enumerate(blk):
                prev, h = h, self.layer(e, [h])
                if i > 0:
                    release(prev)
            hs.append(h)
        for e in topo.middle:
            prev, h = h, self.layer(e, [h])
            if prev is not hs[-1]:
                release(prev)
        for blk in topo.output:
            skip = hs.pop()
            srcs = [h, skip]
            for e in blk:
                h = self.layer(e, srcs)
                for a in srcs:
                    release(a)
                srcs = [h]
        A, B, bnd = self.finalize([h], "out.0", None)
        oc = eng.conv["out.2"]
        self.out_C = oc.Cout
        self.out_shape = (N, oc.Cout, D, Hh, W)
        self.out_buf = torch.empty(self.out_shape, dtype=torch.float32, device=dev)
        self.last_desc = self.conv_step(oc, srcs=[h], out=None, aff=(A, B), act=H.ACT_SILU, bound=(bnd, 0, 32, 2),
                                        out_tensor=self.out_buf, out_layout=H.OUT_NCDHW)
        release(h)
        if self.ws_bytes:
            self.workspace = torch.empty(self.ws_bytes, dtype=torch.uint8, device=dev)
            for dsc in self.ws_descs:
                dsc.workspace, dsc.workspace_bytes = H.ptr(self.workspace), self.ws_bytes

    def finalize(self, srcs, gn_prefix, film_prefix, need_bound=None):
        eng, N = self.eng, self.N
        if gn_prefix is None and not (self.scaled if need_bound is None else need_bound):
            return None, None, None
        Cn = sum(s.C for s in srcs)
        A = torch.empty(N * Cn, dtype=torch.float32, device=eng.device) if gn_prefix else None
        B = torch.empty(N * Cn, dtype=torch.float32, device=eng.device) if gn_prefix else None
        bound = torch.empty(N * 32 * 2, dtype=torch.float32, device=eng.device)
        s0 = srcs[0]
        s1 = srcs[1] if len(srcs) > 1 else None
        if s1 is not None and s1.voxels != s0.voxels:
            raise RuntimeError("concat of tensors with different spatial size")
        gamma = eng.p[gn_prefix + ".weight"] if gn_prefix else None
        beta = eng.p[gn_prefix + ".bias"] if gn_prefix else None
        args = [H.ptr(s0.stats), s0.C, s0.rows,
                H.ptr(s1.stats) if s1 else 0, s1.C if s1 else 0, s1.rows if s1 else 0,
                N, 32, float(s0.voxels), 1e-5, H.ptr(gamma), H.ptr(beta),
                0, 0, 0, H.ptr(A), H.ptr(B), H.ptr(bound), 0]
        if film_prefix is not None:
            args[14] = eng.film_off[film_prefix]
            self.film_patches.append(args)
        self.steps.append((eng.lib.ddpm3d_gn_finalize, args))
        self.keep += [A, B, bound]
        return A, B, bound

    def conv_step(self, pc, srcs, out, aff=None, act=H.ACT_NONE, in_mode=H.IN_SAME, res=None,
                  res_mode=H.RES_NONE, planar=False, out_tensor=None, out_layout=H.OUT_NDHWC,
                  bias_per_n=False, want_stats=True, bound=None):
        N = self.N
        d = H.ConvDesc()
        lib = self.eng.lib
        cin_total = 2 if planar else sum(s.C for s in srcs)
        if pc.wz is not None and not planar and in_mode in (H.IN_SAME, H.IN_UP):
            pc_use = pc.wz
        else:
            pc_use = pc
        if out is not None:
            d.N, d.D, d.H, d.W = N, out.D, out.H, out.W
            d.out = H.ptr(out.buf)
        else:
            s = srcs[0]
            d.N, d.D, d.H, d.W = N, s.D, s.H, s.W
            d.out = H.ptr(out_tensor)
            d.stats = 0
            d.stats_rows = 0
        d.Cout, d.ksize = pc.Cout, pc.k
        d.out_layout = out_layout
        if planar:
            d.in_mode, d.Cin, d.C0, d.C1 = H.IN_PLANAR2, 2, 1, 1
        else:
            d.in_mode = in_mode
            d.src0, d.C0 = H.ptr(srcs[0].buf), srcs[0].C
            if len(srcs) > 1:
                d.src1, d.C1 = H.ptr(srcs[1].buf), srcs[1].C
            d.Cin = d.C0 + d.C1
            if d.Cin != pc.Cin:
                raise RuntimeError("conv %dx%d fed %d channels" % (pc.Cout, pc.Cin, d.Cin))
        for s in ([] if planar else srcs):
            if N * s.voxels * s.C * s.buf.element_size() >= 0xFFFFFFF0:
                raise H.Ddpm3dError(H.E_2BIG, "a source tensor of %d x %d voxels x %d channels exceeds 4 GiB; "
                                              "split the batch" % (N, s.voxels, s.C))
        if aff is not None:
            d.aff_a, d.aff_b = H.ptr(aff[0]), H.ptr(aff[1])
        d.act = act
        io = 0
        if not planar:
            io |= H.IO_SRC0_BF16 if srcs[0].half else 0
            io |= H.IO_SRC1_BF16 if (len(srcs) > 1 and srcs[1].half) else 0
        io |= H.IO_OUT_BF16 if (out is not None and out.half) else 0
        io |= H.IO_RES_BF16 if (res is not None and res.half) else 0
        if io and self.half_dtype == torch.float16:
            io |= H.IO_HALF_IS_F16
        d.io_dtype = io
        if self.scaled:
            if bound is None or bound[0] is None:
                raise RuntimeError("conv_step without an input bound")
            d.in_bound = bound[0].data_ptr() + 4 * bound[1]
            d.in_bound_count, d.in_bound_stride = bound[2], bound[3]
        d.precision = pc_use.precision
        d.w_packed, d.bias = H.ptr(pc_use.w), H.ptr(pc.b)
        if pc_use.up_phase and in_mode == H.IN_UP:
            d.kernel_hint = H.HINT_UP_PHASE
        d.bias_stride_n = 0
        d.res_mode = res_mode
        if res is not None and res.C != pc.Cout:
            raise RuntimeError("residual has %d channels, the conv writes %d" % (res.C, pc.Cout))
        d.res = H.ptr(res.buf) if res is not None else 0
        rows, need, _ = H.conv_plan(d)
        if out is not None and want_stats:
            out.rows = rows
            out.stats = torch.empty(N * rows * pc.Cout * 2, dtype=torch.float64,
                                    device=self.eng.device)
            self.keep.append(out.stats)
            d.stats, d.stats_rows = H.ptr(out.stats), rows
        if need:
            self.ws_descs.append(d)
            self.ws_bytes = max(self.ws_bytes, need)
        self.keep.append(d)
        flops = 2.0 * N * d.D * d.H * d.W * pc.Cout * d.Cin * pc.k ** 3
        name = C.create_string_buffer(64)
        H.check(lib.ddpm3d_conv_kernel_family(C.byref(d), name, 64))
        tag = name.value.decode()
        self.conv_meta[len(self.steps)] = (tag, flops)
        self.steps.append((self.eng.lib.ddpm3d_conv3d, [C.byref(d), 0]))
        return d

    def layer(self, e, srcs):
        eng = self.eng
        if e.kind == "res":
            return self.resblock(e, srcs)
        if e.kind == "upconv":
            x = srcs[0]
            pc = eng.conv[e.prefix + ".conv"]
            y = self.new_act(pc.Cout, x.D, x.H * 2, x.W * 2)
            _, _, bnd = self.finalize([x], None, None)
            self.conv_step(pc, [x], y, in_mode=H.IN_UP, bound=(bnd, 1, 32, 2))
            return y
        if e.kind == "attn":
            return self.attention(e, srcs[0])
        if e.kind == "downconv":
            x = srcs[0]
            if (x.H | x.W) & 1:
                raise RuntimeError("Downsample needs even H, W (got %dx%d)" % (x.H, x.W))
            pc = eng.conv[e.prefix + ".op"]
            y = self.new_act(pc.Cout, x.D, x.H // 2, x.W // 2)
            _, _, bnd = self.finalize([x], None, None)
            self.conv_step(pc, [x], y, in_mode=H.IN_STRIDE2, bound=(bnd, 1, 32, 2))
            return y
        raise ValueError(e.kind)

    def attention(self, e, x):
        eng, N = self.eng, self.N
        p = e.prefix
        heads = e.heads
        Cn = x.C
        if Cn % heads:
            raise RuntimeError("attention: %d channels not divisible by %d heads" % (Cn, heads))
        ch = Cn // heads
        if ch not in (32, 64, 128):
            raise NotImplementedError("attention with %d channels per head (32, 64 or 128 are built)" % ch)
        A, B, bnd = self.finalize([x], p + ".norm", None)
        qkv = self.new_act(3 * Cn, x.D, x.H, x.W, fp32=True)
        self.conv_step(eng.conv[p + ".qkv"], [x], qkv, aff=(A, B), act=H.ACT_NONE, bound=(bnd, 0, 32, 2))
        _, _, qb = self.finalize([qkv], None, None, need_bound=eng.precision != "f32")
        a = self.new_act(Cn, x.D, x.H, x.W, fp32=True)
        self.conv_meta[len(self.steps)] = ("attention_ch%d" % ch, 4.0 * N * heads * float(x.voxels) ** 2 * ch)
        aprec = H.PREC_F32 if eng.precision == "f32" else H.PREC_F16X3
        self.steps.append((eng.lib.ddpm3d_attention_p,
                           [H.ptr(qkv.buf), N, x.voxels, heads, ch, aprec, (H.ptr(qb) + 4) if qb is not None else 0, 32, 2, H.ptr(a.buf), 0]))
        self.release(qkv)
        y = self.new_act(Cn, x.D, x.H, x.W)
        self.conv_step(eng.conv[p + ".proj_out"], [a], y, res=x, res_mode=H.RES_SAME, bound=(qb, 1, 32, 2))
        self.release(a)
        return y

    def resblock(self, e, srcs):
        eng = self.eng
        p = e.prefix
        x0 = srcs[0]
        if e.updown == "down":
            if (x0.H | x0.W) & 1:
                raise RuntimeError("Downsample needs even H, W (got %dx%d)" % (x0.H, x0.W))
            d, h, w, im, rm = x0.D, x0.H // 2, x0.W // 2, H.IN_POOL, H.RES_POOL
        elif e.updown == "up":
            d, h, w, im, rm = x0.D, x0.H * 2, x0.W * 2, H.IN_UP, H.RES_UP
        else:
            d, h, w, im, rm = x0.D, x0.H, x0.W, H.IN_SAME, H.RES_SAME
        c1 = eng.conv[p + ".in_layers.2"]
        c2 = eng.conv[p + ".out_layers.3"]
        A1, B1, bnd1 = self.finalize(srcs, p + ".in_layers.0", None)
        h1 = self.new_act(c1.Cout, d, h, w)
        aff1, act1, srcs1 = (A1, B1), H.ACT_SILU, srcs
        pooled = None
        if e.updown == "down" and c1.wz is not None and len(srcs) == 1:
            pooled = self.new_act(x0.C, d, h, w, fp32=True)
            io = (H.IO_SRC0_BF16 if x0.half else 0) | (H.IO_HALF_IS_F16 if x0.buf.dtype == torch.float16 else 0)
            self.conv_meta[len(self.steps)] = ("pool_act", 0.0)
            self.steps.append((eng.lib.ddpm3d_pool_act,
                               [H.ptr(x0.buf), H.ptr(A1), H.ptr(B1), H.ACT_SILU, 1, self.N, d, h, w, x0.C,
                                H.ptr(pooled.buf), io, 0]))
            aff1, act1, srcs1, im = None, H.ACT_NONE, [pooled], H.IN_SAME
        if eng.film:
            self.conv_step(c1, srcs1, h1, aff=aff1, act=act1, in_mode=im, bound=(bnd1, 0, 32, 2))
            A2, B2, bnd2 = self.finalize([h1], p + ".out_layers.0", p)
        else:
            dsc = self.conv_step(c1, srcs1, h1, aff=aff1, act=act1, in_mode=im, bias_per_n=True,
                                 bound=(bnd1, 0, 32, 2))
            self.bias_patches.append((dsc, eng.film_off[p]))
            A2, B2, bnd2 = self.finalize([h1], p + ".out_layers.0", None)
        if pooled is not None:
            self.release(pooled)
        y = self.new_act(c2.Cout, d, h, w)
        skip = eng.conv.get(p + ".skip_connection")
        if skip is not None:
            if e.updown is not None:
                raise RuntimeError("up/down ResBlock with a channel change is not in the reference")
            self.conv_step(skip, srcs, y, want_stats=False, bound=(bnd1, 1, 32, 2))
            self.conv_step(c2, [h1], y, aff=(A2, B2), act=H.ACT_SILU, res=y, res_mode=H.RES_SAME,
                           bound=(bnd2, 0, 32, 2))
        else:
            if len(srcs) > 1:
                raise NotImplementedError("ResBlock with an Identity skip over a concatenated input "
                                          "(%d + %d -> %d channels)" % (srcs[0].C, srcs[1].C, c2.Cout))
            self.conv_step(c2, [h1], y, aff=(A2, B2), act=H.ACT_SILU, res=x0, res_mode=rm, bound=(bnd2, 0, 32, 2))
        self.release(h1)
        return y

    def _enqueue(self, xptr, lrptr, fptr, film_stride, outptr):
        st = H.stream()
        if self.eng.planar:
            self.first_desc.src0 = xptr
            self.first_desc.src1 = lrptr
            self.absmax_args[0], self.absmax_args[1] = xptr, lrptr
        else:
            self.absmax_args[0] = self.pad_args[0] = xptr
        for a in self.film_patches:
            a[12], a[13] = fptr, film_stride
        for dsc, off in self.bias_patches:
            dsc.bias = fptr + 4 * off
            dsc.bias_stride_n = film_stride
        self.last_desc.out = outptr
        if self.timing is None:
            for fn, args in self.steps:
                args[-1] = st
                rc = fn(*args)
                if rc != 0:
                    H.check(rc)
        else:
            for i, (fn, args) in enumerate(self.steps):
                args[-1] = st
                meta = self.conv_meta.get(i)
                if meta is not None:
                    e0, e1 = torch.cuda.Event(enable_timing=True), torch.cuda.Event(enable_timing=True)
                    e0.record()
                rc = fn(*args)
                if rc != 0:
                    H.check(rc)
                if meta is not None:
                    e1.record()
                    self.timing.append((meta[0], meta[1], e0, e1))
```

include/ddpm3d.h:

```cpp
#ifndef DDPM3D_H
#define DDPM3D_H

#include <stddef.h>
#include <stdint.h>

#ifdef __cplusplus
extern "C" {
#endif

#define DDPM3D_ABI_VERSION 13

enum {
    DDPM3D_OK = 0,
    DDPM3D_EINVAL = -1,
    DDPM3D_ELAUNCH = -2,
    DDPM3D_ENOSUP = -3,
    DDPM3D_E2BIG = -4
};

enum {
    DDPM3D_IN_SAME = 0,
    DDPM3D_IN_POOL = 1,
    DDPM3D_IN_UP = 2,
    DDPM3D_IN_PLANAR2 = 3,
    DDPM3D_IN_STRIDE2 = 4
};

enum {
    DDPM3D_RES_NONE = 0,
    DDPM3D_RES_SAME = 1,
    DDPM3D_RES_POOL = 2,
    DDPM3D_RES_UP = 3
};

enum { DDPM3D_ACT_NONE = 0, DDPM3D_ACT_SILU = 1 };
enum { DDPM3D_OUT_NDHWC = 0, DDPM3D_OUT_NCDHW = 1 };

typedef struct ddpm3d_conv_desc {
    int32_t N, D, H, W;
    int32_t Cin;
    int32_t Cout;
    int32_t ksize;
    int32_t in_mode;
    const float* src0;
    const float* src1;
    int32_t C0, C1;
    const float* aff_a;
    const float* aff_b;
    int32_t act;
    int32_t precision;
    const void* w_packed;
    const float* bias;
    int32_t bias_stride_n;
    int32_t res_mode;
    const float* res;
    float* out;
    int32_t out_layout;
    int32_t stats_rows;
    double* stats;
    void* workspace;
    size_t workspace_bytes;
    int32_t kernel_hint;
    int32_t in_bound_count;
    const float* in_bound;
    int32_t in_bound_stride;
    int32_t io_dtype;
} ddpm3d_conv_desc;

enum {
    DDPM3D_IO_SRC0_BF16 = 1,
    DDPM3D_IO_SRC1_BF16 = 2,
    DDPM3D_IO_OUT_BF16 = 4,
    DDPM3D_IO_RES_BF16 = 8,
    DDPM3D_IO_HALF_IS_F16 = 16
};

enum {
    DDPM3D_HINT_WSTAT_OFF = 0x100,
    DDPM3D_HINT_WSTAT_ON = 0x200,
    DDPM3D_HINT_WZ_ORDER_SHIFT = 12,
    DDPM3D_HINT_WZ_ORDER_MASK = 0x7000,
    DDPM3D_HINT_SPLITK_SHIFT = 16,
    DDPM3D_HINT_SPLITK_MASK = 0x3F0000,
    DDPM3D_HINT_UP_PHASE = 0x400
};

#define DDPM3D_WZ_UP_PHASE_IMAGE 0x100

int ddpm3d_abi_version(void);
const char* ddpm3d_last_error(void);

enum {
    DDPM3D_PREC_F32 = 0,
    DDPM3D_PREC_F16X3 = 1,
    DDPM3D_PREC_F16 = 2,
    DDPM3D_PREC_F16X3_WZ = 3,
    DDPM3D_PREC_F16_WZ = 4,
    DDPM3D_PREC_BF16 = 5,
    DDPM3D_PREC_BF16_WZ = 6
};

size_t ddpm3d_packed_weight_bytes(int Cout, int Cin, int ksize, int precision);
int ddpm3d_pack_conv_weight(const float* w_oidhw, int Cout, int Cin, int ksize, int precision,
                            void* w_packed, void* stream);
size_t ddpm3d_packed_up_phase_bytes(int Cout, int Cin);
int ddpm3d_pack_up_phase_weight(const float* w_oidhw, int Cout, int Cin, void* w_packed, void* stream);

int ddpm3d_conv_stats_rows(int N, int D, int H, int W, int Cin, int Cout, int ksize, int precision);
size_t ddpm3d_conv_workspace_bytes(int N, int D, int H, int W, int Cin, int Cout, int ksize, int precision);
int ddpm3d_conv3d(const ddpm3d_conv_desc* desc, void* stream);
int ddpm3d_conv_kernel_family(const ddpm3d_conv_desc* desc, char* name, int name_len);
int ddpm3d_conv_plan(const ddpm3d_conv_desc* desc, int* stats_rows, size_t* workspace_bytes, int* split);

typedef struct ddpm3d_conv_weights {
    const void* w_packed;
    const void* w_packed_wz;
    const float* bias;
    int32_t Cout, Cin, ksize;
    int32_t precision, precision_wz;
} ddpm3d_conv_weights;

enum { DDPM3D_LAYER_RES = 1, DDPM3D_LAYER_ATTN = 2, DDPM3D_LAYER_DOWNCONV = 3, DDPM3D_LAYER_UPCONV = 4 };
enum { DDPM3D_UPDOWN_NONE = 0, DDPM3D_UPDOWN_DOWN = 1, DDPM3D_UPDOWN_UP = 2 };

typedef struct ddpm3d_layer {
    int32_t kind;
    int32_t updown;
    int32_t heads;
    int32_t film_off;
    const float* norm1_gamma;
    const float* norm1_beta;
    const float* norm2_gamma;
    const float* norm2_beta;
    ddpm3d_conv_weights conv1;
    ddpm3d_conv_weights conv2;
    ddpm3d_conv_weights skip;
} ddpm3d_layer;

typedef struct ddpm3d_unet_desc {
    int32_t n_layers;
    const ddpm3d_layer* layers;
    int32_t n_input_blocks;
    const int32_t* input_block_layers;
    int32_t n_middle_layers;
    int32_t n_output_blocks;
    const int32_t* output_block_layers;
    ddpm3d_conv_weights first;
    const float* out_gamma;
    const float* out_beta;
    ddpm3d_conv_weights out;
    int32_t film;
    int32_t planar;
    int32_t in_channels, cin_pad;
    int32_t arithmetic;
} ddpm3d_unet_desc;

typedef struct ddpm3d_unet_plan ddpm3d_unet_plan;
size_t ddpm3d_unet_plan_bytes(const ddpm3d_unet_desc* model, int N, int D, int H, int W);
int ddpm3d_unet_plan_create(const ddpm3d_unet_desc* model, int N, int D, int H, int W, void* arena, size_t arena_bytes,
                            ddpm3d_unet_plan** plan);
int ddpm3d_unet_forward(ddpm3d_unet_plan* plan, const float* x, const float* low_res, const float* film_rows,
                        int film_stride, float* out, void* stream);
void ddpm3d_unet_plan_destroy(ddpm3d_unet_plan* plan);
const char* ddpm3d_unet_last_error(void);

int ddpm3d_gn_finalize(const double* stats0, int C0, int rows0,
                       const double* stats1, int C1, int rows1,
                       int N, int groups, double count, float eps,
                       const float* gamma, const float* beta,
                       const float* film, int film_stride, int film_off,
                       float* aff_a, float* aff_b, float* bound, void* stream);

int ddpm3d_absmax(const float* x0, const float* x1, int N, size_t per_sample, float* bound, void* stream);

int ddpm3d_gn_stats_rows(int voxels);
int ddpm3d_gn_stats(const float* x, int N, int voxels, int C, double* stats, void* stream);

int ddpm3d_timestep_embedding(const float* t, int rows, int dim, const float* freqs,
                              float* out, void* stream);
int ddpm3d_linear(const float* in, int rows, int K, const float* w, const float* bias,
                  int O, int silu_in, float* out, int out_stride, void* stream);

int ddpm3d_pool_act(const void* src, const float* aff_a, const float* aff_b, int act, int fast_act, int N, int D,
                    int H, int W, int C, void* out, int io_dtype, void* stream);

int ddpm3d_add_embedding(float* emb, const float* table, const int64_t* idx, int rows, int dim, int num_classes,
                         void* stream);

int ddpm3d_attention(const float* qkv, int N, int T, int heads, int head_channels,
                     float* out, void* stream);
int ddpm3d_attention_p(const float* qkv, int N, int T, int heads, int head_channels, int precision,
                       const float* qkv_bound, int bound_count, int bound_stride,
                       float* out, void* stream);

int ddpm3d_ncdhw_to_ndhwc(const float* in, int N, int C, int voxels, float* out, void* stream);
int ddpm3d_ndhwc_to_ncdhw(const float* in, int N, int C, int voxels, float* out, void* stream);
int ddpm3d_ncdhw_to_ndhwc_pad(const float* in, int N, int C, int voxels, int Cpad, float* out, void* stream);

int ddpm3d_subsample_hw2(const float* in, int N, int D, int H, int W, int C, float* out, void* stream);

enum {
    DDPM3D_C_SQRT_RECIP_ACP = 0,
    DDPM3D_C_SQRT_RECIPM1_ACP = 1,
    DDPM3D_C_POST_MEAN_COEF1 = 2,
    DDPM3D_C_POST_MEAN_COEF2 = 3,
    DDPM3D_C_MIN_LOG = 4,
    DDPM3D_C_MAX_LOG = 5,
    DDPM3D_C_ACP = 6,
    DDPM3D_C_ACP_PREV = 7,
    DDPM3D_NCOEF = 8
};
enum {
    DDPM3D_F_LEARN_SIGMA = 1,
    DDPM3D_F_PREDICT_XSTART = 2,
    DDPM3D_F_CLIP = 4
};
int ddpm3d_p_sample_step(const float* model_out, const float* x, const float* noise,
                         const float* coef, const int64_t* t_idx, int N, int voxels,
                         int flags, float* sample, float* pred_xstart, void* stream);
int ddpm3d_ddim_step(const float* model_out, const float* x, const float* noise,
                     const float* coef, const int64_t* t_idx, int N, int voxels,
                     int flags, float eta, float* sample, float* pred_xstart, void* stream);

enum {
    DDPM3D_Q_SQRT_ACP = 0,
    DDPM3D_Q_SQRT_1M_ACP = 1,
    DDPM3D_Q_LOG_1M_ACP = 2,
    DDPM3D_Q_POST_LOG_VAR = 3,
    DDPM3D_NQCOEF = 4
};
int ddpm3d_q_sample(const float* x_start, const float* noise, const float* qcoef, const int64_t* t_idx,
                    int N, int voxels, int T, float* x_t, void* stream);
size_t ddpm3d_vb_terms_workspace_bytes(int N, int voxels);
int ddpm3d_vb_terms(const float* model_out, const float* x_start, const float* x_t, const float* noise,
                    const float* coef, const float* qcoef, const int64_t* t_idx, int N, int voxels, int T,
                    int flags, void* ws, size_t ws_bytes, float* vb, float* xstart_mse, float* mse,
                    int ld_out, float* pred_xstart, void* stream);
int ddpm3d_prior_bpd(const float* x_start, const float* qcoef, int N, int voxels, int T, void* ws,
                     size_t ws_bytes, float* out, void* stream);

int ddpm3d_p_mean_variance(const float* model_out, const float* x, const float* coef, const int64_t* t_idx,
                           int N, int voxels, int T, int flags, float* mean, float* variance,
                           float* log_variance, float* pred_xstart, void* stream);
int ddpm3d_ddim_reverse_step(const float* model_out, const float* x, const float* coef, const int64_t* t_idx,
                             int N, int voxels, int T, int flags, float* sample, float* pred_xstart,
                             void* stream);


enum {
    DDPM3D_S_CX = 0,
    DDPM3D_S_W0 = 1,
    DDPM3D_S_W1 = 2,
    DDPM3D_S_W2 = 3,
    DDPM3D_S_CZ = 4,
    DDPM3D_NSCOEF = 8
};
int ddpm3d_dpm_solver_step(const float* model_out, const float* x, const float* x0_prev1,
                           const float* x0_prev2, const float* noise, const float* coef,
                           const float* scoef, const int64_t* t_idx, int N, int voxels, int T,
                           int flags, int order, float* sample, float* pred_xstart, void* stream);

#define DDPM3D_MAX_DRAWS 64
int ddpm3d_draw_stitch(const float* samples, int K, int res, const double* window, int xs, int ys, int zs,
                       int H, int W, int D, float* acc, float* wsum, void* stream);
int ddpm3d_draw_moments(const float* acc, const float* wsum, int K, int64_t voxels, float* mean, float* std,
// ... 82 lines not shown
```

Before: 0.3331.

## Fuse ResBlock 1x1 skip convolution into the Winograd conv2 kernel epilogue

Adds a SKIP mode to the Winograd conv kernel. After the 3x3x3 accumulation, it streams the skip input and 1x1 weights through LDS and accumulates the skip product into the same registers with 3x f16-split MFMA, then applies the combined bias in one epilogue. This removes a separate 1x1 conv launch plus the write and re-read of the skip output as a residual. In exchange the kernel gets longer and needs more registers, accumulators are rescaled between the two activation scales (a possible accuracy risk), and a fallback two-call path is kept.

```diff
diff --git a/3d-denoising-diffusion-model_amd/csrc/api.hip b/3d-denoising-diffusion-model_amd/csrc/api.hip
--- a/3d-denoising-diffusion-model_amd/csrc/api.hip
+++ b/3d-denoising-diffusion-model_amd/csrc/api.hip
@@ -227,6 +227,84 @@
                                      : launched(ddpm3d_launch_conv(k, c, (hipStream_t)stream), "conv3d");
     if (rc != DDPM3D_OK || c.S == 1) return rc;
     return launched(ddpm3d_launch_splitk_reduce(k, (hipStream_t)stream), "conv3d split-K reduce");
+}
+
+static int base_prec(int p) {
+    return p == DDPM3D_PREC_F16X3_WZ ? DDPM3D_PREC_F16X3 : p == DDPM3D_PREC_F16_WZ ? DDPM3D_PREC_F16
+         : p == DDPM3D_PREC_BF16_WZ ? DDPM3D_PREC_BF16 : p;
+}
+static int skip_prepare(const ddpm3d_conv_desc* d, const ddpm3d_conv_skip* sk, ddpm3d_conv_desc& sd, ConvK& k, ConvCfg& c,
+                        bool& fused, bool for_launch) {
+    fused = false;
+    if (!d || !sk) return fail(DDPM3D_EINVAL, "conv3d_skip: null descriptor");
+    if (d->res_mode != DDPM3D_RES_NONE || d->res)
+        return fail(DDPM3D_EINVAL, "conv3d_skip: conv2 carries no residual of its own (the skip conv is its residual)");
+    if (d->out_layout != DDPM3D_OUT_NDHWC) return fail(DDPM3D_EINVAL, "conv3d_skip: NDHWC output only");
+    if (d->ksize != 3) return fail(DDPM3D_EINVAL, "conv3d_skip: conv2 is a 3x3x3 conv (ksize %d)", d->ksize);
+    if (sk->C0 <= 0 || sk->C1 < 0) return fail(DDPM3D_EINVAL, "conv3d_skip: C0=%d C1=%d", sk->C0, sk->C1);
+    if (sk->io_dtype & ~(DDPM3D_IO_SRC0_BF16 | DDPM3D_IO_SRC1_BF16))
+        return fail(DDPM3D_EINVAL, "conv3d_skip: skip io_dtype names sources only (%#x)", sk->io_dtype);
+    memset(&sd, 0, sizeof(sd));
+    sd.N = d->N; sd.D = d->D; sd.H = d->H; sd.W = d->W;
+    sd.C0 = sk->C0; sd.C1 = sk->C1; sd.Cin = sk->C0 + sk->C1; sd.Cout = d->Cout;
+    sd.ksize = 1; sd.in_mode = DDPM3D_IN_SAME;
+    sd.src0 = sk->src0; sd.src1 = sk->src1;
+    sd.act = DDPM3D_ACT_NONE; sd.precision = base_prec(d->precision);
+    sd.w_packed = sk->w_packed; sd.bias = sk->bias;
+    sd.res_mode = DDPM3D_RES_NONE;
+    sd.out = d->out; sd.out_layout = DDPM3D_OUT_NDHWC;
+    sd.workspace = d->workspace; sd.workspace_bytes = d->workspace_bytes;
+    sd.in_bound = sk->in_bound; sd.in_bound_count = sk->in_bound_count; sd.in_bound_stride = sk->in_bound_stride;
+    sd.io_dtype = sk->io_dtype | (d->io_dtype & (DDPM3D_IO_OUT_BF16 | DDPM3D_IO_HALF_IS_F16));
+    ConvK ks;
+    ConvCfg cs;
+    int route_s = ROUTE_GENERAL, route = ROUTE_GENERAL;
+    int ok = conv_prepare(&sd, ks, cs, route_s, false);
+    if (ok != DDPM3D_OK) return ok;
+    if (for_launch && (!sk->src0 || !sk->w_packed || !sk->bias)) return fail(DDPM3D_EINVAL, "conv3d_skip: null buffer");
+    const int cand = d->precision == DDPM3D_PREC_F16X3_WZ && d->in_mode == DDPM3D_IN_SAME && d->io_dtype == 0 &&
+                     sk->io_dtype == 0 && !(d->kernel_hint & (DDPM3D_HINT_UP_PHASE | DDPM3D_HINT_WZ_ORDER_MASK)) &&
+                     route_s == ROUTE_PW && aligned16(sk->bias);
+    ok = conv_prepare(d, k, c, route, for_launch && cand);
+    if (ok != DDPM3D_OK) return ok;
+    fused = cand && route == ROUTE_GENERAL && ddpm3d_skip_fuse_rule(d->N, d->D, d->H, d->W, sd.Cin, d->Cout, c);
+    if (!fused) return DDPM3D_OK;
+    k.sk_src0 = sk->src0; k.sk_src1 = sk->src1; k.sk_C0 = sk->C0; k.sk_C1 = sk->C1;
+    k.sk_src0_bytes = ks.src0_bytes; k.sk_src1_bytes = ks.src1_bytes;
+    k.sk_w = ks.w; k.sk_w_bytes = ks.w_bytes; k.sk_wscale = ks.wscale;
+    k.sk_bias = sk->bias;
+    k.sk_bound = sk->in_bound; k.sk_bound_count = sk->in_bound_count; k.sk_bound_stride = sk->in_bound_stride;
+    k.sk_blocks_per_split = (sd.Cin / 32 + c.S - 1) / c.S;
+    return DDPM3D_OK;
+}
+
+int ddpm3d_conv3d_skip(const ddpm3d_conv_desc* d, const ddpm3d_conv_skip* sk, void* stream) {
+    ddpm3d_conv_desc sd;
+    ConvK k;
+    ConvCfg c;
+    bool fused = false;
+    const int ok = skip_prepare(d, sk, sd, k, c, fused, true);
+    if (ok != DDPM3D_OK) return ok;
+    if (fused) {
+        const int rc = launched(ddpm3d_launch_conv(k, c, (hipStream_t)stream), "conv3d_skip");
+        if (rc != DDPM3D_OK || c.S == 1) return rc;
+        return launched(ddpm3d_launch_splitk_reduce(k, (hipStream_t)stream), "conv3d_skip split-K reduce");
+    }
+    const int rc = ddpm3d_conv3d(&sd, stream);
+    if (rc != DDPM3D_OK) return rc;
+    ddpm3d_conv_desc d2 = *d;
+    d2.res = d->out;
+    d2.res_mode = DDPM3D_RES_SAME;
+    if (d->io_dtype & DDPM3D_IO_OUT_BF16) d2.io_dtype |= DDPM3D_IO_RES_BF16;
+    return ddpm3d_conv3d(&d2, stream);
+}
+
+int ddpm3d_conv_skip_fused(const ddpm3d_conv_desc* d, const ddpm3d_conv_skip* sk) {
+    ddpm3d_conv_desc sd;
+    ConvK k;
+    ConvCfg c;
+    bool fused = false;
+    return skip_prepare(d, sk, sd, k, c, fused, false) == DDPM3D_OK && fused ? 1 : 0;
 }
 
 int ddpm3d_conv_plan(const ddpm3d_conv_desc* d, int* stats_rows, size_t* workspace_bytes, int* split) {
diff --git a/3d-denoising-diffusion-model_amd/csrc/conv3d.hip b/3d-denoising-diffusion-model_amd/csrc/conv3d.hip
--- a/3d-denoising-diffusion-model_amd/csrc/conv3d.hip
+++ b/3d-denoising-diffusion-model_amd/csrc/conv3d.hip
@@ -247,7 +247,8 @@
     const size_t v1 = min(v0 + (size_t)p.reduce_vox, DHW);
     const size_t slab_stride = (size_t)p.N * DHW * p.Cout;
     for (int cout = threadIdx.x; cout < p.Cout; cout += 256) {
-        const float bias = p.bias[(size_t)n * p.bias_stride_n + cout];
+        float bias = p.bias[(size_t)n * p.bias_stride_n + cout];
+        if (p.sk_bias != nullptr) bias += p.sk_bias[cout];
         GnAcc gs;
         gs.init(0.0f);
         float cnt = 0.0f;
@@ -292,7 +293,8 @@
 #pragma unroll
         for (int c = 0; c < 4; ++c) gs[c].init(0.0f);
         if (qok) {
-            const f32x4 bias = *reinterpret_cast<const f32x4*>(p.bias + (size_t)n * p.bias_stride_n + q * 4);
+            f32x4 bias = *reinterpret_cast<const f32x4*>(p.bias + (size_t)n * p.bias_stride_n + q * 4);
+            if (p.sk_bias != nullptr) bias += *reinterpret_cast<const f32x4*>(p.sk_bias + q * 4);
 #pragma unroll
             for (int i = 0; i < RV / 4; ++i) {
                 const size_t v = v0 + vl + 4 * i;
@@ -391,6 +393,9 @@
 
 #if DDPM3D_PREC_ONLY == 3
 #include "conv3d_wz.h"
+#ifndef DDPM3D_WZ_T84
+#define DDPM3D_WZ_T84 1
+#endif
 hipError_t ddpm3d_launch_conv_wz(const ConvK& k, const ConvCfg& c, hipStream_t st) {
     const int gy = k.CoutPad / 128;
     const int gx = k.N * k.tilesZ * k.tilesY * k.tilesX;
@@ -400,6 +405,20 @@
     constexpr size_t stamp_lds = 0;
 #endif
     constexpr size_t lds = (size_t)WzGeom::BUF + stamp_lds;
+    if (k.sk_w != nullptr) {
+        if (c.PREC != DDPM3D_PREC_F16X3_WZ) return hipErrorInvalidValue;
+        constexpr size_t slds4 = (size_t)WzGeomT<4>::BUF + stamp_lds, slds84 = (size_t)WzGeomT<8, 4>::BUF + stamp_lds;
+        if (c.TXL == 2)
+            hipLaunchKernelGGL((conv3d_wz_kernel<WZ_F16X3_SKIP, 4, 4>), dim3(gx, gy, k.ksplit), dim3(256), slds4, st, k);
+        else if (DDPM3D_WZ_T84 && k.H % 8 == 0 && k.D % 4 == 0) {
+            ConvK k2 = k;
+            k2.tilesY = 2 * k.tilesY;
+            k2.tilesZ = k.tilesZ / 2;
+            hipLaunchKernelGGL((conv3d_wz_kernel<WZ_F16X3_SKIP, 4, 8, 4>), dim3(gx, gy, k.ksplit), dim3(256), slds84, st, k2);
+        } else
+            hipLaunchKernelGGL((conv3d_wz_kernel<WZ_F16X3_SKIP, 4>), dim3(gx, gy, k.ksplit), dim3(256), lds, st, k);
+        return hipGetLastError();
+    }
     if (k.hint & DDPM3D_HINT_UP_PHASE) {
         UpPhaseGeom g;
         if (c.PREC != DDPM3D_PREC_F16X3_WZ || !ddpm3d_up_phase_geom(k.D, k.H, k.W, c, g)) return hipErrorInvalidValue;
@@ -425,9 +444,6 @@
             hipLaunchKernelGGL((conv3d_wz_kernel<WZ_F16X3, 4, 4>), dim3(gx, gy, k.ksplit), dim3(256), lds4, st, k);
         return hipGetLastError();
     }
-#ifndef DDPM3D_WZ_T84
-#define DDPM3D_WZ_T84 1
-#endif
     if (DDPM3D_WZ_T84 && k.H % 8 == 0 && k.D % 4 == 0 && !(k.hint & DDPM3D_HINT_WZ_ORDER_MASK)) {
         ConvK k2 = k;
         k2.tilesY = 2 * k.tilesY;
diff --git a/3d-denoising-diffusion-model_amd/csrc/conv3d_params.h b/3d-denoising-diffusion-model_amd/csrc/conv3d_params.h
--- a/3d-denoising-diffusion-model_amd/csrc/conv3d_params.h
+++ b/3d-denoising-diffusion-model_amd/csrc/conv3d_params.h
@@ -31,6 +31,16 @@
     int reduce_vox;
     int hint;
     int io;
+    const float* sk_src0;
+    const float* sk_src1;
+    const float* sk_w;
+    const float* sk_wscale;
+    const float* sk_bias;
+    const float* sk_bound;
+    int sk_bound_count, sk_bound_stride;
+    unsigned sk_w_bytes, sk_src0_bytes, sk_src1_bytes;
+    int sk_C0, sk_C1;
+    int sk_blocks_per_split;
 };
 
 struct ConvCfg {
@@ -129,6 +139,11 @@
     return c;
 }
 
+static inline bool ddpm3d_skip_fuse_rule(int N, int D, int H, int W, int Cx, int Cout, const ConvCfg& c) {
+    (void)N; (void)D; (void)H; (void)W; (void)Cx; (void)Cout; (void)c;
+    return true;
+}
+
 static inline size_t ddpm3d_packed_bytes(int Cout, int Cin, int ksize, int prec) {
     const size_t taps = (prec == DDPM3D_PREC_F16X3_WZ || prec == DDPM3D_PREC_F16_WZ || prec == DDPM3D_PREC_BF16_WZ)
                             ? 36 : (size_t)ksize * ksize * ksize;
diff --git a/3d-denoising-diffusion-model_amd/csrc/conv3d_stage.h b/3d-denoising-diffusion-model_amd/csrc/conv3d_stage.h
--- a/3d-denoising-diffusion-model_amd/csrc/conv3d_stage.h
+++ b/3d-denoising-diffusion-model_amd/csrc/conv3d_stage.h
@@ -2,7 +2,8 @@
 #include "conv3d_epilogue.h"
 
 enum { WZ_F16X3 = 0, WZ_F16 = 1, WZ_BF16 = 2,
-       WZ_F16X3_UP = 3 };
+       WZ_F16X3_UP = 3,
+       WZ_F16X3_SKIP = 4 };
 
 __device__ __forceinline__ void split_pair(float s0, float s1, unsigned& hi, unsigned& lo) {
     float l0, l1;
diff --git a/3d-denoising-diffusion-model_amd/csrc/conv3d_wz.h b/3d-denoising-diffusion-model_amd/csrc/conv3d_wz.h
--- a/3d-denoising-diffusion-model_amd/csrc/conv3d_wz.h
+++ b/3d-denoising-diffusion-model_amd/csrc/conv3d_wz.h
@@ -11,7 +11,8 @@
 template <int MODE_, int IL = 0, int TX = 8, int TY = TX>
 __global__ __launch_bounds__(256, 2) void conv3d_wz_kernel(const ConvK p) {
     constexpr bool PHASE = MODE_ == WZ_F16X3_UP;
-    constexpr int MODE = PHASE ? (int)WZ_F16X3 : MODE_;
+    constexpr bool SKIP = MODE_ == WZ_F16X3_SKIP;
+    constexpr int MODE = (PHASE || SKIP) ? (int)WZ_F16X3 : MODE_;
     typedef WzGeomT<TX, TY> G;
     constexpr bool X3 = MODE == WZ_F16X3;
     constexpr int CK = DDPM3D_CONV_CK, NT = PHASE ? 16 : 36;
@@ -73,12 +74,17 @@
     ActScale asc = {1.0f, 1.0f};
     float bound_raw = 0.0f;
     if constexpr (MODE != WZ_BF16) bound_raw = act_scale_load(p, n);
+    float sk_bound_raw = 0.0f;
+    ActScale ax = {1.0f, 1.0f};
+    if constexpr (SKIP)
+        if (lane < p.sk_bound_count) sk_bound_raw = p.sk_bound[((size_t)n * p.sk_bound_count + lane) * p.sk_bound_stride];
     StageLaneT<G> sl = stage_lane<G, PHASE>(p, tid, n, y0, x0, max(z0 - 1, 0), 1.0f);
     stage_zero_border(sl, lds, 1, tid);
     StageRawT<G> raw;
     if (chunk_begin < chunk_end) stage_issue(p, sl, raw, n, z0, chunk_begin);
     if constexpr (MODE != WZ_BF16) {
         asc = act_scale_finish(bound_raw, 2.0f);
+        if constexpr (SKIP) ax = act_scale_finish(sk_bound_raw, 1.0f);
         stage_lane_scale(p, sl, asc.s);
     }
     WZ_STAMP(1);
@@ -204,6 +210,101 @@
         outv[2 + t] = acc[1][t] - acc[2][t] - acc[3][t];
     }
     const int tile_in_n = ((ph * p.tilesZ + tz_i) * p.tilesY + ty_i) * p.tilesX + tx_i;
+    if constexpr (SKIP) {
+        const int tid_ = tid;
+        constexpr int XB = 32, XROW = VS * 16, XCH = 128 * XROW;
+        static_assert(2 * XCH <= G::BUF, "an x block fits the tile's image");
+        const int nxb = (p.sk_C0 + p.sk_C1) / XB;
+        const int xb_begin = wg.split * p.sk_blocks_per_split;
+        const int xb_end = min(nxb, xb_begin + p.sk_blocks_per_split);
+        int tid = tid_;
+        asm volatile("" : "+v"(tid));
+        const int lane = tid & 63, half = lane >> 5;
+        const int xq = tid & 7;
+        unsigned xv0[4], xv1[4];
+#pragma unroll
+        for (int i = 0; i < 4; ++i) {
+            const int m = (tid >> 3) + 32 * i;
+            const int z = z0 + epi_tz<TXL, TYL, G::NZP != 1>(m), y = y0 + ((m >> TXL) & (TY - 1)), x = x0 + (m & (TX - 1));
+            const bool inb = z < p.D && y < p.H && x < p.W;
+            const unsigned vox = (unsigned)(((n * p.D + z) * p.H + y) * p.W + x);
+            xv0[i] = inb ? (vox * (unsigned)p.sk_C0 + xq * 4u) * 4u : DDPM3D_OOB_OFFSET;
+            xv1[i] = inb ? (vox * (unsigned)p.sk_C1 + xq * 4u) * 4u : DDPM3D_OOB_OFFSET;
+        }
+        const int xl = ((xq >> 2) * 128 + (tid >> 3)) * XROW + (xq & 3) * 8;
+        const int xa = ((lane & 31) * VS + half) * 16;
+        auto x_issue = [&](const int b, u32x4 (&xr)[4]) {
+            const bool valid = b < xb_end;
+            const int c0 = b * XB;
+            const bool from0 = c0 < p.sk_C0;
+            const __amdgpu_buffer_rsrc_t rs = make_rsrc(from0 ? p.sk_src0 : p.sk_src1,
+                                                        valid ? (from0 ? p.sk_src0_bytes : p.sk_src1_bytes) : 0u);
+            const unsigned soff = valid ? (unsigned)(from0 ? c0 : c0 - p.sk_C0) * 4u : 0u;
+#pragma unroll
+            for (int i = 0; i < 4; ++i) xr[i] = buffer_load16(rs, from0 ? xv0[i] : xv1[i], soff);
+        };
+        auto w_issue = [&](const int b, u32x4 (&wq)[2][2]) {
+            const bool valid = b < xb_end;
+            const __amdgpu_buffer_rsrc_t rs = make_rsrc(p.sk_w, valid ? p.sk_w_bytes : 0u);
+            const unsigned soff = valid ? (unsigned)(2 * b) * wchunk_stride : 0u;
+#pragma unroll
+            for (int c = 0; c < 2; ++c) {
+                wq[c][0] = buffer_load16(rs, wlane, soff + c * wchunk_stride);
+                wq[c][1] = buffer_load16(rs, wlane, soff + c * wchunk_stride + wpart);
+            }
+        };
+        u32x4 xr[4], wa[2][2], wb[2][2];
+        x_issue(xb_begin, xr);
+        w_issue(xb_begin, wa);
+        const int coutk = wg.cy * 128 + (tid >> 6) * 32 + (lane & 31);
+        const float sk_ws = coutk < p.Cout ? p.sk_wscale[coutk] : 1.0f;
+        const float sk_bias = coutk < p.Cout ? p.sk_bias[coutk] : 0.0f;
+        const float rho = (ax.s * asc.inv) * (pre_ws / sk_ws);
+#pragma unroll
+        for (int u = 0; u < 4; ++u)
+#pragma unroll
+            for (int i = 0; i < 16; ++i) outv[u][i] *= rho;
+        auto x_block = [&](const int b, u32x4 (&xr)[4], u32x4 (&wq)[2][2], u32x4 (&wn)[2][2]) {
+            __syncthreads();
+#pragma unroll
+            for (int i = 0; i < 4; ++i) {
+                const f32x4 v = __builtin_bit_cast(f32x4, xr[i]);
+                unsigned h0, h1, l0, l1;
+                split_pair(v[0] * ax.s, v[1] * ax.s, h0, l0);
+                split_pair(v[2] * ax.s, v[3] * ax.s, h1, l1);
+                unsigned char* row = lds + xl + i * 32 * XROW;
+                *reinterpret_cast<u32x2*>(row) = u32x2{h0, h1};
+                *reinterpret_cast<u32x2*>(row + 32) = u32x2{l0, l1};
+            }
+            x_issue(b + 1, xr);
+            w_issue(b + 1, wn);
+            __syncthreads();
+#pragma unroll
+            for (int c = 0; c < 2; ++c) {
+                const h8 bhi = __builtin_bit_cast(h8, wq[c][0]), blo = __builtin_bit_cast(h8, wq[c][1]);
+#pragma unroll
+                for (int u = 0; u < 4; ++u) {
+                    const unsigned char* a = lds + c * XCH + u * 32 * XROW + xa;
+                    const h8 ahi = *reinterpret_cast<const h8*>(a), alo = *reinterpret_cast<const h8*>(a + 32);
+                    outv[u] = mfma16<false>(alo, bhi, outv[u]);
+                    outv[u] = mfma16<false>(ahi, blo, outv[u]);
+                    outv[u] = mfma16<false>(ahi, bhi, outv[u]);
+                }
+            }
+        };
+        for (int b = xb_begin; b < xb_end; b += 2) {
+            x_block(b, xr, wa, wb);
+            x_block(b + 1, xr, wb, wa);
+        }
+        const float bias2 = pre_bias + sk_bias;
+        if (p.ksplit > 1)
+            conv_epilogue<1, 1, 4, TXL, TYL, true, G::NZP != 1, true, false>(p, outv, n, z0, y0, x0, tile_in_n, 0, cout, half, wg.split,
+                                                                     ax.inv, true, sk_ws, bias2, 0, 0);
+        else
+            conv_epilogue<1, 1, 4, TXL, TYL, false, G::NZP != 1, false, false>(p, outv, n, z0, y0, x0, tile_in_n, 0, cout, half, wg.split,
+                                                                     ax.inv, true, sk_ws, bias2, 0, 0);
+        return;
+    }
     #ifndef DDPM3D_WZ_WIDE_X3
 #define DDPM3D_WZ_WIDE_X3 0
 #endif
diff --git a/3d-denoising-diffusion-model_amd/csrc/unet_plan.hip b/3d-denoising-diffusion-model_amd/csrc/unet_plan.hip
--- a/3d-denoising-diffusion-model_amd/csrc/unet_plan.hip
+++ b/3d-denoising-diffusion-model_amd/csrc/unet_plan.hip
@@ -24,6 +24,7 @@
 struct Step {
     int kind;
     ddpm3d_conv_desc conv;
+    ddpm3d_conv_skip skip; bool has_skip;
     size_t st0, st1; int C0, rows0, C1, rows1; double count; const float *gamma, *beta; int film, film_off;
     size_t A, B, bound; bool has_ab;
     size_t per_sample; int two; size_t dst; int C, Cpad, vox;
@@ -115,12 +116,16 @@
         bool ncdhw_out = false;
         size_t bound = 0; int bound_first = 0, bound_count = 0, bound_stride = 0; bool has_bound = false;
         int film_off = 0;
+        const ddpm3d_conv_weights* skip_w = nullptr;
+        const Act* x0 = nullptr; const Act* x1 = nullptr;
+        size_t xbound = 0; int xbound_first = 0; bool has_xbound = false;
+        bool* fused = nullptr;
     };
     bool conv_step(const ddpm3d_conv_weights& pc, ConvArgs a, int* step_index = nullptr) {
         ddpm3d_conv_desc d;
         memset(&d, 0, sizeof(d));
         const bool wz = pc.w_packed_wz && !a.planar && (a.in_mode == DDPM3D_IN_SAME || a.in_mode == DDPM3D_IN_UP);
-        d.precision = wz ? (pc.precision_wz & ~DDPM3D_WZ_UP_PHASE_IMAGE) : pc.precision;
+        d.precision = wz ? (pc.precision_wz & ~DDPM3D_WZ_UP_PHASE_IMAGE) : (pc.precision & ~DDPM3D_SKIP_TWO_CALLS);
         d.w_packed = wz ? pc.w_packed_wz : pc.w_packed;
         if (wz && (pc.precision_wz & DDPM3D_WZ_UP_PHASE_IMAGE) && a.in_mode == DDPM3D_IN_UP)
             d.kernel_hint = DDPM3D_HINT_UP_PHASE;
@@ -158,6 +163,22 @@
             d.in_bound = (const float*)at(a.bound) + a.bound_first;
             d.in_bound_count = a.bound_count; d.in_bound_stride = a.bound_stride;
         }
+        ddpm3d_conv_skip sk;
+        memset(&sk, 0, sizeof(sk));
+        if (a.skip_w) {
+            sk.src0 = (const float*)at(a.x0->off); sk.C0 = a.x0->C;
+            if (a.x1) { sk.src1 = (const float*)at(a.x1->off); sk.C1 = a.x1->C; }
+            sk.w_packed = a.skip_w->w_packed; sk.bias = a.skip_w->bias;
+            if (a.x0->esize == 2) sk.io_dtype |= DDPM3D_IO_SRC0_BF16;
+            if (a.x1 && a.x1->esize == 2) sk.io_dtype |= DDPM3D_IO_SRC1_BF16;
+            if (scaled) {
+                if (!a.has_xbound) return fail("skip conv without an input bound");
+                sk.in_bound = (const float*)at(a.xbound) + a.xbound_first;
+                sk.in_bound_count = a.bound_count; sk.in_bound_stride = a.bound_stride;
+            }
+            *a.fused = ddpm3d_conv_skip_fused(&d, &sk) != 0;
+            if (!*a.fused) return true;
+        }
         int rows = 0, split = 1;
         size_t need = 0;
         const int rc = ddpm3d_conv_plan(&d, &rows, &need, &split);
@@ -173,6 +194,8 @@
         memset(&st, 0, sizeof(st));
         st.kind = S_CONV;
         st.conv = d;
+        st.skip = sk;
+        st.has_skip = a.skip_w != nullptr;
         if (a.bias_per_n) { bias_steps.push_back((int)steps.size()); bias_offs.push_back(a.film_off); }
         if (step_index) *step_index = (int)steps.size();
         steps.push_back(st);
@@ -223,6 +246,18 @@
         c2.bound = bnd2; c2.bound_count = 32; c2.bound_stride = 2; c2.has_bound = has2;
         if (e.skip.w_packed) {
             if (e.updown != DDPM3D_UPDOWN_NONE) return fail("up/down ResBlock with a channel change is not in the reference");
+            bool fused = false;
+            if (!(e.skip.precision & DDPM3D_SKIP_TWO_CALLS)) {
+                ConvArgs cf = c2;
+                cf.skip_w = &e.skip; cf.x0 = s0; cf.x1 = s1;
+                cf.xbound = bnd1; cf.xbound_first = 1; cf.has_xbound = has1; cf.fused = &fused;
+                if (!conv_step(e.conv2, cf)) return false;
+            }
+            if (fused) {
+                release(h1);
+                *y_out = y;
+                return true;
+            }
             ConvArgs cs;
             cs.src0 = s0; cs.src1 = s1; cs.out = &y; cs.want_stats = false;
             cs.bound = bnd1; cs.bound_first = 1; cs.bound_count = 32; cs.bound_stride = 2; cs.has_bound = has1;
@@ -446,7 +481,9 @@
     for (const Step& s : pl->steps) {
         int rc = DDPM3D_OK;
         switch (s.kind) {
-            case S_CONV: rc = ddpm3d_conv3d(&s.conv, stream); break;
+            case S_CONV:
+                rc = s.has_skip ? ddpm3d_conv3d_skip(&s.conv, &s.skip, stream) : ddpm3d_conv3d(&s.conv, stream);
+                break;
             case S_FINALIZE:
                 rc = ddpm3d_gn_finalize((const double*)(b + s.st0), s.C0, s.rows0, s.C1 ? (const double*)(b + s.st1) : nullptr,
                                         s.C1, s.rows1, pl->N, 32, s.count, 1e-5f, s.gamma, s.beta,
diff --git a/3d-denoising-diffusion-model_amd/guided_diffusion/_hip.py b/3d-denoising-diffusion-model_amd/guided_diffusion/_hip.py
--- a/3d-denoising-diffusion-model_amd/guided_diffusion/_hip.py
+++ b/3d-denoising-diffusion-model_amd/guided_diffusion/_hip.py
@@ -28,6 +28,7 @@
 HINT_WZ_ORDER_SHIFT = 12
 HINT_UP_PHASE = 0x400
 WZ_UP_PHASE_IMAGE = 0x100
+SKIP_TWO_CALLS = 0x100
 
 _fp = C.c_void_p
 
@@ -46,6 +47,12 @@
     ]
 
 
+class ConvSkip(C.Structure):
+    _fields_ = [("src0", _fp), ("src1", _fp), ("C0", C.c_int32), ("C1", C.c_int32), ("w_packed", _fp), ("bias", _fp),
+                ("in_bound", _fp), ("in_bound_count", C.c_int32), ("in_bound_stride", C.c_int32),
+                ("io_dtype", C.c_int32)]
+
+
 class ConvWeights(C.Structure):
     _fields_ = [("w_packed", _fp), ("w_packed_wz", _fp), ("bias", _fp), ("Cout", C.c_int32), ("Cin", C.c_int32),
                 ("ksize", C.c_int32), ("precision", C.c_int32), ("precision_wz", C.c_int32)]
@@ -106,6 +113,8 @@
     "ddpm3d_conv3d": (C.c_int, [C.POINTER(ConvDesc), _fp]),
     "ddpm3d_conv_kernel_family": (C.c_int, [C.POINTER(ConvDesc), C.c_char_p, C.c_int]),
     "ddpm3d_conv_plan": (C.c_int, [C.POINTER(ConvDesc), C.POINTER(C.c_int), C.POINTER(C.c_size_t), C.POINTER(C.c_int)]),
+    "ddpm3d_conv3d_skip": (C.c_int, [C.POINTER(ConvDesc), C.POINTER(ConvSkip), _fp]),
+    "ddpm3d_conv_skip_fused": (C.c_int, [C.POINTER(ConvDesc), C.POINTER(ConvSkip)]),
     "ddpm3d_unet_plan_bytes": (C.c_size_t, [C.POINTER(UnetDesc), C.c_int, C.c_int, C.c_int, C.c_int]),
     "ddpm3d_unet_plan_create": (C.c_int, [C.POINTER(UnetDesc), C.c_int, C.c_int, C.c_int, C.c_int, _fp, C.c_size_t,
                                           C.POINTER(_fp)]),
diff --git a/3d-denoising-diffusion-model_amd/guided_diffusion/engine.py b/3d-denoising-diffusion-model_amd/guided_diffusion/engine.py
--- a/3d-denoising-diffusion-model_amd/guided_diffusion/engine.py
+++ b/3d-denoising-diffusion-model_amd/guided_diffusion/engine.py
@@ -95,6 +95,7 @@
             params[base + ".bias"] = params[base + ".bias"][perm].contiguous()
         self.p = params
         self.up_phase = (winograd and precision == "f16x3" and os.environ.get("DDPM3D_UP_PHASE", "1") != "0")
+        self.skip_fuse = os.environ.get("DDPM3D_SKIP_FUSE", "1") != "0"
         up_conv1 = {e.prefix + ".in_layers.2" for e in topo.all_layers() if e.kind == "res" and e.updown == "up"}
         for name, t in params.items():
             if name.endswith(".weight") and t.dim() >= 3:
@@ -201,6 +202,8 @@
                 L.conv1 = self._conv_weights(self.conv[e.prefix + ".in_layers.2"])
                 L.conv2 = self._conv_weights(self.conv[e.prefix + ".out_layers.3"])
                 L.skip = self._conv_weights(self.conv.get(e.prefix + ".skip_connection"))
+                if L.skip.w_packed and not self.skip_fuse:
+                    L.skip.precision |= H.SKIP_TWO_CALLS
             elif e.kind == "attn":
                 L.kind = H.LAYER_ATTN
                 L.norm1_gamma, L.norm1_beta = H.ptr(p[e.prefix + ".norm.weight"]), H.ptr(p[e.prefix + ".norm.bias"])
@@ -488,7 +491,7 @@
 
     def conv_step(self, pc, srcs, out, aff=None, act=H.ACT_NONE, in_mode=H.IN_SAME, res=None,
                   res_mode=H.RES_NONE, planar=False, out_tensor=None, out_layout=H.OUT_NDHWC,
-                  bias_per_n=False, want_stats=True, bound=None):
+                  bias_per_n=False, want_stats=True, bound=None, skip=None):
         N = self.N
         d = H.ConvDesc()
         lib = self.eng.lib
@@ -548,6 +551,20 @@
         if res is not None and res.C != pc.Cout:
             raise RuntimeError("residual has %d channels, the conv writes %d" % (res.C, pc.Cout))
         d.res = H.ptr(res.buf) if res is not None else 0
+        sk = None
+        if skip is not None:
+            spc, xs, xb = skip
+            sk = H.ConvSkip()
+            sk.src0, sk.C0 = H.ptr(xs[0].buf), xs[0].C
+            if len(xs) > 1:
+                sk.src1, sk.C1 = H.ptr(xs[1].buf), xs[1].C
+            sk.w_packed, sk.bias = H.ptr(spc.w), H.ptr(spc.b)
+            sk.io_dtype = (H.IO_SRC0_BF16 if xs[0].half else 0) | (H.IO_SRC1_BF16 if len(xs) > 1 and xs[1].half else 0)
+            if self.scaled:
+                sk.in_bound = xb[0].data_ptr() + 4 * xb[1]
+                sk.in_bound_count, sk.in_bound_stride = xb[2], xb[3]
+            if not lib.ddpm3d_conv_skip_fused(C.byref(d), C.byref(sk)):
+                return None
         rows, need, _ = H.conv_plan(d)
         if out is not None and want_stats:
             out.rows = rows
@@ -563,6 +580,12 @@
         name = C.create_string_buffer(64)
         H.check(lib.ddpm3d_conv_kernel_family(C.byref(d), name, 64))
         tag = name.value.decode()
+        if sk is not None:
+            flops += 2.0 * N * d.D * d.H * d.W * pc.Cout * (sk.C0 + sk.C1)
+            self.keep.append(sk)
+            self.conv_meta[len(self.steps)] = (tag, flops)
+            self.steps.append((lib.ddpm3d_conv3d_skip, [C.byref(d), C.byref(sk), 0]))
+            return d
         self.conv_meta[len(self.steps)] = (tag, flops)
         self.steps.append((self.eng.lib.ddpm3d_conv3d, [C.byref(d), 0]))
         return d
@@ -657,9 +680,14 @@
         if skip is not None:
             if e.updown is not None:
                 raise RuntimeError("up/down ResBlock with a channel change is not in the reference")
-            self.conv_step(skip, srcs, y, want_stats=False, bound=(bnd1, 1, 32, 2))
-            self.conv_step(c2, [h1], y, aff=(A2, B2), act=H.ACT_SILU, res=y, res_mode=H.RES_SAME,
-                           bound=(bnd2, 0, 32, 2))
+            fused = None
+            if eng.skip_fuse:
+                fused = self.conv_step(c2, [h1], y, aff=(A2, B2), act=H.ACT_SILU, bound=(bnd2, 0, 32, 2),
+                                       skip=(skip, srcs, (bnd1, 1, 32, 2)))
+            if fused is None:
+                self.conv_step(skip, srcs, y, want_stats=False, bound=(bnd1, 1, 32, 2))
+                self.conv_step(c2, [h1], y, aff=(A2, B2), act=H.ACT_SILU, res=y, res_mode=H.RES_SAME,
+                               bound=(bnd2, 0, 32, 2))
         else:
             if len(srcs) > 1:
                 raise NotImplementedError("ResBlock with an Identity skip over a concatenated input "
diff --git a/include/ddpm3d.h b/include/ddpm3d.h
--- a/include/ddpm3d.h
+++ b/include/ddpm3d.h
@@ -86,6 +86,7 @@
 };
 
 #define DDPM3D_WZ_UP_PHASE_IMAGE 0x100
+#define DDPM3D_SKIP_TWO_CALLS 0x100
 
 int ddpm3d_abi_version(void);
 const char* ddpm3d_last_error(void);
@@ -111,6 +112,20 @@
 int ddpm3d_conv3d(const ddpm3d_conv_desc* desc, void* stream);
 int ddpm3d_conv_kernel_family(const ddpm3d_conv_desc* desc, char* name, int name_len);
 int ddpm3d_conv_plan(const ddpm3d_conv_desc* desc, int* stats_rows, size_t* workspace_bytes, int* split);
+
+typedef struct ddpm3d_conv_skip {
+    const float* src0;
+    const float* src1;
+    int32_t C0, C1;
+    const void* w_packed;
+    const float* bias;
+    const float* in_bound;
+    int32_t in_bound_count;
+    int32_t in_bound_stride;
+    int32_t io_dtype;
+} ddpm3d_conv_skip;
+int ddpm3d_conv3d_skip(const ddpm3d_conv_desc* conv2, const ddpm3d_conv_skip* skip, void* stream);
+int ddpm3d_conv_skip_fused(const ddpm3d_conv_desc* conv2, const ddpm3d_conv_skip* skip);
 
 typedef struct ddpm3d_conv_weights {
     const void* w_packed;
```

Measured after the change: 0.3440 (median of 6 runs). 3.3% higher.
